# jacarvalho/mpd-public

Measured on AMD Instinct MI355X. Metric: denoising-steps/s, higher is better.
Workload: dtype f32; 1 GPU; cfg2: EnvDense2D-RobotPointMass shape, 100 trajectories (1 context(s)) x H=64 x D=4, T=100 (+5) reverse steps, unguided, U-Net dim_mults (1, 2, 4, 8), one plan = one bench step; parallelism=single, denoising_steps_per_plan=105

## Files before the change

### include/mpdx.h

```cpp
#ifndef MPDX_H
#define MPDX_H

#include <stddef.h>
#include <stdint.h>

#ifdef __cplusplus
extern "C" {
#endif

#define MPDX_E_INVALID   (-1)
#define MPDX_E_NOTFOUND  (-2)
#define MPDX_E_STATE     (-3)
#define MPDX_E_DEVICE    (-4)

#define MPDX_MAX_LEVELS 8

typedef struct mpdx_unet mpdx_unet;

typedef struct mpdx_unet_cfg {
    int32_t state_dim;
    int32_t n_support_points;
    int32_t unet_input_dim;
    int32_t n_levels;
    int32_t dim_mults[MPDX_MAX_LEVELS];
    int32_t time_emb_dim;
    int32_t self_attention;
} mpdx_unet_cfg;

const char* mpdx_last_error(void);
int mpdx_version(void);

int    mpdx_unet_create(const mpdx_unet_cfg* cfg, mpdx_unet** out);
void   mpdx_unet_destroy(mpdx_unet* u);
int    mpdx_unet_set_plan_join(mpdx_unet* u, int on);
int    mpdx_unet_plan_joined(const mpdx_unet* u);
int    mpdx_unet_set_level_split(mpdx_unet* u, int on);
int    mpdx_unet_plan_split(const mpdx_unet* u);
int    mpdx_level_split_block(int B, int block, int32_t* trajectory, int32_t* role);
int    mpdx_unet_set_inner_run(mpdx_unet* u, int on);
int    mpdx_unet_set_inner_run_parts(mpdx_unet* u, int parts);
int    mpdx_unet_set_inner_run_width(mpdx_unet* u, int width);
int    mpdx_inner_run_block(int B, int width, int cus, int block, int32_t* cluster, int32_t* tile, int32_t* counter_lines);
int    mpdx_unet_inner_runs(const mpdx_unet* u);
int    mpdx_unet_inner_run_layers(const mpdx_unet* u);
int    mpdx_unet_status(const mpdx_unet* u);
int    mpdx_unet_set_status(mpdx_unet* u, unsigned word);
int    mpdx_unet_num_params(const mpdx_unet* u);
int    mpdx_unet_param_info(const mpdx_unet* u, int idx, const char** name, int32_t shape[3], int32_t* ndim);
size_t mpdx_unet_packed_floats(const mpdx_unet* u);
size_t mpdx_unet_timetab_floats(const mpdx_unet* u, int T);
size_t mpdx_unet_workspace_floats(const mpdx_unet* u, int B);
int    mpdx_unet_pack_param(mpdx_unet* u, const char* name, const float* src_dev, size_t n_floats,
                            float* packed_dev, void* stream);
int    mpdx_unet_build_timetab(mpdx_unet* u, const float* packed_dev, const float* freqs16_dev, int T,
                               float* timetab_dev, void* stream);

int mpdx_unet_forward(mpdx_unet* u, const float* packed_dev, const float* timetab_dev, int T,
                      const float* x, int t, float* eps, int B, float* ws, void* stream);

typedef struct mpdx_step_coefs {
    float sqrt_recip_alphas_cumprod;
    float sqrt_recipm1_alphas_cumprod;
    float posterior_mean_coef1;
    float posterior_mean_coef2;
    float noise_scale;
    float noise_std_extra;
    int32_t predict_epsilon;
    int32_t clip_denoised;
    float ddim_k1;
    float ddim_k2;
    float guide_scale;
} mpdx_step_coefs;

int mpdx_ddpm_step(mpdx_unet* u, const float* packed_dev, const float* timetab_dev, int T,
                   float* x_io, const float* noise, const float* hard_start, const float* hard_goal,
                   const mpdx_step_coefs* coefs, int t, int mean_only, float* chain_out,
                   uint32_t* absmax_out, int n_per_ctx, int B, float* ws, void* stream);

int mpdx_add_noise(float* x_io, const float* noise, const float* hard_start, const float* hard_goal,
                   float noise_scale, float noise_std_extra, float* chain_out, int B, int H, int D, void* stream);

int mpdx_hard_conds(float* x_io, float* chain_out, int n, const int32_t* horizon_idx, const float* const* values, int B, int H, int D, void* stream);

int mpdx_q_sample(const float* x_start, const float* noise, const long long* t_dev, const float* sqrt_alphas_cumprod_dev,
                  const float* sqrt_one_minus_alphas_cumprod_dev, const float* hard_start, const float* hard_goal, float* out, int B, int H,
                  int D, int T, void* stream);
int mpdx_weighted_loss(const float* pred, const float* targ, const float* weights_hd, const float* hard_start, const float* hard_goal,
                       int l1, float* out1, int B, int H, int D, void* stream);

size_t mpdx_train_flat_floats(mpdx_unet* u);
size_t mpdx_train_dgrad_pack_floats(mpdx_unet* u);
size_t mpdx_train_workspace_floats(mpdx_unet* u, int B);
int    mpdx_train_param_offset(mpdx_unet* u, int idx, size_t* off, size_t* n);
int    mpdx_train_pack(mpdx_unet* u, const float* flat, float* packed, float* packedT, void* stream);
int    mpdx_train_loss_backward(mpdx_unet* u, const float* flat, const float* packed, const float* packedT, float* grads_flat,
                                const float* x_start, const float* noise, const long long* t_dev, const float* sqrt_alphas_cumprod_dev,
                                const float* sqrt_one_minus_alphas_cumprod_dev, const float* freqs16, const float* hard_start,
                                const float* hard_goal, const float* weights_hd, int T, int B, int predict_epsilon, int l1, float loss_scale,
                                float* loss_out, float* ws, void* stream);
int    mpdx_adam_step(float* params, const float* grads, float* exp_avg, float* exp_avg_sq, size_t n, float lr, float beta1, float beta2,
                      float eps, int step, float max_norm, float* scratch, void* stream);
int    mpdx_train_draw(mpdx_unet* u, unsigned long long seed, const int* step_counter_dev);
int    mpdx_ema_update(float* ema, const float* params, size_t n, float beta, void* stream);

int mpdx_randn(float* out, size_t n, uint64_t seed, uint64_t offset, void* stream);

#define MPDX_MAX_FIELDS 4
#define MPDX_FIELD_OBJECTS   0
#define MPDX_FIELD_WORKSPACE 1
#define MPDX_FIELD_SELF      2
#define MPDX_FIELD_GRID      3
#define MPDX_ROBOT_POINTMASS 0
#define MPDX_ROBOT_PANDA     1
#define MPDX_ROBOT_CHAIN     2

typedef struct mpdx_field {
    int32_t kind;
    float   weight;
    int32_t sphere_off, n_spheres;
    int32_t box_off, n_boxes;
    float   ws_min[3], ws_max[3];
    union { int32_t grid_sdf_off;
            int32_t track_len; };
    union { int32_t grid_grad_off;
            int32_t track_off; };
    int32_t n[3];
    float   origin[3];
    float   cell;
    int32_t mode;
} mpdx_field;
#define MPDX_GRID_LINEAR  0
#define MPDX_GRID_NEAREST 1

typedef struct mpdx_guide_params {
    int32_t robot;
    int32_t q_dim;
    int32_t ws_dim;
    int32_t interpolate;
    int32_t n_interp;
    int32_t clip_grad;
    float   max_grad_norm;
    float   mins[16], maxs[16];
    float   cutoff_margin;
    float   link_margin;
    int32_t n_fields;
    mpdx_field fields[MPDX_MAX_FIELDS];
    int32_t use_gp;
    float   gp_weight;
    float   dt;
    float   sigma_gp;
    const float* prims;
    int32_t n_prim_floats;
    int32_t clip_rule;
    float   max_grad_value;
    int32_t gp_half_factor;
    int32_t identity_normalizer;
    const float* grids;
    int32_t n_grid_floats;
    int32_t n_scenes;
    int32_t scene_stride;
    const int32_t* scene_of_ctx;
    int32_t scene_n_per_ctx;
    const float* chain;
    int32_t n_chain_floats;
    int32_t tool_frame;
    float   tool_axis[3];
    float   tool_world[3];
    float   tool_cos_min;
    float   tool_weight;
} mpdx_guide_params;
#define MPDX_ROBOT_CHAIN_MAX_JOINTS    8
#define MPDX_ROBOT_CHAIN_MAX_SPHERES   16
#define MPDX_ROBOT_CHAIN_MAX_PAIRS     24
#define MPDX_ROBOT_CHAIN_HEADER_FLOATS 4
#define MPDX_ROBOT_CHAIN_JOINT_FLOATS  16
#define MPDX_ROBOT_CHAIN_SPHERE_FLOATS 8
#define MPDX_ROBOT_CHAIN_REVOLUTE      0
#define MPDX_ROBOT_CHAIN_PRISMATIC     1
#define MPDX_SCENE_HEADER_WORDS 8
#define MPDX_SCENE_MAX_STAGED_FLOATS 12288

int mpdx_guide_step(const mpdx_guide_params* gp, float* x, float* grad_out, const float* hard_start, const float* hard_goal,
                    const uint32_t* absmax_in, uint32_t* absmax_out, int n_per_ctx, int B, int H, int D, void* stream);
int mpdx_guide_step_scaled(const mpdx_guide_params* gp, float* x, float* grad_out, const float* hard_start, const float* hard_goal,
                           const uint32_t* absmax_in, uint32_t* absmax_out, int n_per_ctx, int B, int H, int D, float guide_scale,
                           void* stream);
int mpdx_guide_time(const mpdx_guide_params* gp, float* x, float* grad_out, const uint32_t* absmax_in, int n_per_ctx, int B, int H, int D,
                    int reps, void* stream, float* ms_avg);
int mpdx_guide_trace(const mpdx_guide_params* gp, float* x, const uint32_t* absmax_in, int B, int H, int D, void* stream,
                     long long* stamps128);
int mpdx_guide_variant(const mpdx_guide_params* gp, int B, int H, int D);
int mpdx_absmax(const float* x, uint32_t* absmax_out, int n_per_ctx, int B, int H, int D, void* stream);

int mpdx_traj_metrics(const mpdx_guide_params* gp, const float* x_unnormalised, float* out4, int n_check, int B, int H, int D,
                      void* stream);
int mpdx_traj_metrics_mask(const mpdx_guide_params* gp, const float* x_unnormalised, float* out4, uint8_t* mask, int n_check, int B,
                           int H, int D, void* stream);

int mpdx_traj_tool_metrics(const mpdx_guide_params* gp, const float* x_unnormalised, float* out2, uint8_t* mask, int n_check, int B, int H, int D,
                           void* stream);

int mpdx_sdf_grid_bake(const mpdx_guide_params* gp, int field, float* sdf_out, float* grad_out, const int n[3], const float origin[3], float cell,
                       void* stream);

size_t mpdx_sdf_grid_edt_ws_bytes(const int n[3]);
int mpdx_sdf_grid_from_occupancy(const uint8_t* occ, float* sdf_out, float* grad_out, int32_t* d2_out, const int n[3], float cell, float inflate, void* ws,
                                 size_t ws_bytes, void* stream);
int mpdx_occupancy_from_points(const float* points, int n_points, uint8_t* occ, const int n[3], const float origin[3], float cell, void* stream);

#define MPDX_MESH_SIGN_WINDING 0
#define MPDX_MESH_SIGN_NONE    1
int mpdx_sdf_grid_from_mesh(const float* vertices, int n_vertices, const int32_t* faces, int n_faces, float* sdf_out, float* grad_out ,
                            float* wind_out , const int n[3], const float origin[3], float cell, float inflate,
                            int sign_mode, void* stream);

#define MPDX_TSDF_MAX_CAMS     8
#define MPDX_TSDF_MAX_SPHERES 64
typedef struct mpdx_depth_camera {
    const float* depth;
    int32_t width, height;
    float fx, fy, cx, cy;
    float cam_from_world[12];
    float world_from_cam[12];
    float min_depth, max_depth;
} mpdx_depth_camera;
int mpdx_tsdf_integrate(const mpdx_depth_camera* cams, int n_cams, const float* spheres , int n_spheres,
                        float* tsdf, float* weight, uint8_t* occ, const int n[3], const float origin[3], float cell, float trunc, float max_weight,
                        void* stream);

typedef struct mpdx_gpmp_opts {
    float   sigma_obs;
    float   lambda_up, lambda_down, lambda_min, lambda_max;
    float   step;
    int32_t adaptive;
} mpdx_gpmp_opts;
int mpdx_gpmp_step(const mpdx_guide_params* gp, const mpdx_gpmp_opts* opts, float* x, float* delta, float* state, int B, int H, int D,
                   int solve, void* stream);

typedef struct mpdx_rrt_opts {
    float    q_lo[8], q_hi[8];
    float    step;
    int32_t  max_nodes, max_iters, max_connect_steps, n_edge_checks;
    uint64_t seed;
} mpdx_rrt_opts;
int mpdx_rrt_connect(const mpdx_guide_params* gp, const mpdx_rrt_opts* opts, const float* start, const float* goal, float* nodes,
                     int32_t* parent, int32_t* count, int32_t* link, int32_t* iters, int n, void* stream);

int mpdx_rrt_paths(const mpdx_guide_params* gp, const float* start, const float* goal, const float* nodes, const int32_t* parent, const int32_t* link,
                   float* trajs_out, int32_t* path_len, int n, int max_nodes, int H, float dt, int n_edge_checks, int rounds, void* stream);

typedef struct mpdx_ik_opts {
    int32_t  frame;
    float    offset[3];
    float    q_lo[8], q_hi[8];
    float    rot_weight;
    float    pos_tol, rot_tol;
    float    lambda_init, lambda_up, lambda_down, lambda_min, lambda_max;
    int32_t  adaptive;
    int32_t  max_iters;
    uint64_t seed;
} mpdx_ik_opts;
int mpdx_ik_solve(const mpdx_guide_params* gp, const mpdx_ik_opts* opts, const float* target, const float* q_init, float* q_out, float* err_out,
                  int32_t* status, int n, int restarts, void* stream);

int mpdx_plan(mpdx_unet* u, const float* packed_dev, const float* timetab_dev, int T, const mpdx_step_coefs* coefs,
              int n_without_noise, float* x, const float* noise, const float* hard_start, const float* hard_goal,
              float* chain, int B, float* ws, const mpdx_guide_params* guide, int n_guide_steps, int t_start_guide,
              uint32_t* guide_flags, int n_per_ctx, uint64_t rng_seed, uint64_t rng_offset, void* stream);

int mpdx_unet_profile(mpdx_unet* u, const float* packed_dev, const float* timetab_dev, int T, const float* x, int t,
                      int B, float* ws, void* stream, int cap, float* ms_out, double* flops_out,
                      const char** names_out, int* n_out);
int mpdx_layer_trace(mpdx_unet* u, const float* packed_dev, const float* timetab_dev, const float* x, int layer, int B, float* ws,
                     void* stream, long long* stamps32);
int mpdx_fused_trace(mpdx_unet* u, const float* packed_dev, const float* timetab_dev, const float* x, int seg, int B,
                     float* ws, void* stream, long long* stamps_out, int cap, int* n_out, int* nops_out);
int mpdx_unet_time_units(mpdx_unet* u, const float* packed_dev, const float* timetab_dev, int T, const float* x, int t, int B,
                         float* ws, void* stream, int unit_first, int unit_last, int reps, float* ms_avg);
int mpdx_unet_time_without(mpdx_unet* u, const float* packed_dev, const float* timetab_dev, int T, const float* x, int t, int B,
                           float* ws, void* stream, unsigned long long skip_mask, int reps, float* ms_avg);
int mpdx_unet_unit_layer(const mpdx_unet* u, int B, int i);
int mpdx_unet_fused_program(const mpdx_unet* u, int seg);
double mpdx_unet_unit_bytes(const mpdx_unet* u, int B, int i);
int mpdx_unet_unit_is_pair(const mpdx_unet* u, int B, int i);
int mpdx_bench_layer(mpdx_unet* u, const float* packed_dev, const float* timetab_dev, const float* x, int layer, int B,
                     float* ws, void* stream, int reps, int dbg, float* ms_per_launch);
int mpdx_unet_layer_tile(const mpdx_unet* u, int i, int B, char* buf, size_t buflen);
int mpdx_attention_block(float* x, const float* to_qkv_w, const float* to_out_w, const float* to_out_b, const float* norm_g, const float* norm_b,
                         int B, int L, int Lv, int C, void* stream);

#ifdef __cplusplus
}
#endif
#endif
```

### mpd_public_amd/_lib.py

```python
from __future__ import annotations

import ctypes as C
from pathlib import Path

import os as _os

_LIB_PATH = Path(_os.environ["MPDX_LIB"]) if _os.environ.get("MPDX_LIB") else Path(__file__).resolve().parent / "libmpdx.so"
_lib = None

MAX_LEVELS = 8


class UnetCfg(C.Structure):
    _fields_ = [("state_dim", C.c_int32), ("n_support_points", C.c_int32), ("unet_input_dim", C.c_int32),
                ("n_levels", C.c_int32), ("dim_mults", C.c_int32 * MAX_LEVELS), ("time_emb_dim", C.c_int32),
                ("self_attention", C.c_int32)]


class StepCoefs(C.Structure):
    _fields_ = [("sqrt_recip_alphas_cumprod", C.c_float), ("sqrt_recipm1_alphas_cumprod", C.c_float),
                ("posterior_mean_coef1", C.c_float), ("posterior_mean_coef2", C.c_float),
                ("noise_scale", C.c_float), ("noise_std_extra", C.c_float),
                ("predict_epsilon", C.c_int32), ("clip_denoised", C.c_int32), ("ddim_k1", C.c_float), ("ddim_k2", C.c_float),
                ("guide_scale", C.c_float)]


MAX_FIELDS = 4
SCENE_HEADER_WORDS = 2 * MAX_FIELDS
SCENE_MAX_STAGED_FLOATS = 12 * 1024
FIELD_OBJECTS, FIELD_WORKSPACE, FIELD_SELF, FIELD_GRID = 0, 1, 2, 3
GRID_LINEAR, GRID_NEAREST = 0, 1
MESH_SIGN_WINDING, MESH_SIGN_NONE = 0, 1
ROBOT_POINTMASS, ROBOT_PANDA, ROBOT_CHAIN = 0, 1, 2
ROBOT_CHAIN_MAX_JOINTS, ROBOT_CHAIN_MAX_SPHERES, ROBOT_CHAIN_MAX_PAIRS = 8, 16, 24
ROBOT_CHAIN_HEADER_FLOATS, ROBOT_CHAIN_JOINT_FLOATS, ROBOT_CHAIN_SPHERE_FLOATS = 4, 16, 8
ROBOT_CHAIN_REVOLUTE, ROBOT_CHAIN_PRISMATIC = 0, 1


class _FieldWord0(C.Union):
    _fields_ = [("grid_sdf_off", C.c_int32), ("track_len", C.c_int32)]


class _FieldWord1(C.Union):
    _fields_ = [("grid_grad_off", C.c_int32), ("track_off", C.c_int32)]


class Field(C.Structure):
    _anonymous_ = ("_word0", "_word1")
    _fields_ = [("kind", C.c_int32), ("weight", C.c_float), ("sphere_off", C.c_int32), ("n_spheres", C.c_int32),
                ("box_off", C.c_int32), ("n_boxes", C.c_int32), ("ws_min", C.c_float * 3), ("ws_max", C.c_float * 3),
                ("_word0", _FieldWord0), ("_word1", _FieldWord1), ("n", C.c_int32 * 3), ("origin", C.c_float * 3),
                ("cell", C.c_float), ("mode", C.c_int32)]


class GuideParams(C.Structure):
    _fields_ = [("robot", C.c_int32), ("q_dim", C.c_int32), ("ws_dim", C.c_int32), ("interpolate", C.c_int32),
                ("n_interp", C.c_int32), ("clip_grad", C.c_int32), ("max_grad_norm", C.c_float),
                ("mins", C.c_float * 16), ("maxs", C.c_float * 16), ("cutoff_margin", C.c_float), ("link_margin", C.c_float),
                ("n_fields", C.c_int32), ("fields", Field * MAX_FIELDS), ("use_gp", C.c_int32), ("gp_weight", C.c_float),
                ("dt", C.c_float), ("sigma_gp", C.c_float), ("prims", C.c_void_p), ("n_prim_floats", C.c_int32),
                ("clip_rule", C.c_int32), ("max_grad_value", C.c_float), ("gp_half_factor", C.c_int32),
                ("identity_normalizer", C.c_int32), ("grids", C.c_void_p), ("n_grid_floats", C.c_int32),
                ("n_scenes", C.c_int32), ("scene_stride", C.c_int32), ("scene_of_ctx", C.c_void_p), ("scene_n_per_ctx", C.c_int32),
                ("chain", C.c_void_p), ("n_chain_floats", C.c_int32),
                ("tool_frame", C.c_int32), ("tool_axis", C.c_float * 3), ("tool_world", C.c_float * 3), ("tool_cos_min", C.c_float),
                ("tool_weight", C.c_float)]


class GpmpOpts(C.Structure):
    _fields_ = [("sigma_obs", C.c_float), ("lambda_up", C.c_float), ("lambda_down", C.c_float), ("lambda_min", C.c_float),
                ("lambda_max", C.c_float), ("step", C.c_float), ("adaptive", C.c_int32)]


class RrtOpts(C.Structure):
    _fields_ = [("q_lo", C.c_float * 8), ("q_hi", C.c_float * 8), ("step", C.c_float), ("max_nodes", C.c_int32), ("max_iters", C.c_int32),
                ("max_connect_steps", C.c_int32), ("n_edge_checks", C.c_int32), ("seed", C.c_uint64)]


class IkOpts(C.Structure):
    _fields_ = [("frame", C.c_int32), ("offset", C.c_float * 3), ("q_lo", C.c_float * 8), ("q_hi", C.c_float * 8), ("rot_weight", C.c_float),
                ("pos_tol", C.c_float), ("rot_tol", C.c_float), ("lambda_init", C.c_float), ("lambda_up", C.c_float), ("lambda_down", C.c_float),
                ("lambda_min", C.c_float), ("lambda_max", C.c_float), ("adaptive", C.c_int32), ("max_iters", C.c_int32), ("seed", C.c_uint64)]


TSDF_MAX_CAMS, TSDF_MAX_SPHERES = 8, 64


class DepthCamera(C.Structure):
    _fields_ = [("depth", C.c_void_p), ("width", C.c_int32), ("height", C.c_int32), ("fx", C.c_float), ("fy", C.c_float), ("cx", C.c_float),
                ("cy", C.c_float), ("cam_from_world", C.c_float * 12), ("world_from_cam", C.c_float * 12), ("min_depth", C.c_float),
                ("max_depth", C.c_float)]


_vp, _sz, _i, _f = C.c_void_p, C.c_size_t, C.c_int, C.c_float
SIGNATURES = {
    "mpdx_last_error": (C.c_char_p, []),
    "mpdx_version": (_i, []),
    "mpdx_unet_create": (_i, [C.POINTER(UnetCfg), C.POINTER(_vp)]),
    "mpdx_unet_destroy": (None, [_vp]),
    "mpdx_unet_set_plan_join": (_i, [_vp, _i]),
    "mpdx_unet_plan_joined": (_i, [_vp]),
    "mpdx_unet_set_level_split": (_i, [_vp, _i]),
    "mpdx_unet_plan_split": (_i, [_vp]),
    "mpdx_level_split_block": (_i, [_i, _i, _vp, _vp]),
    "mpdx_unet_set_inner_run": (_i, [_vp, _i]),
    "mpdx_unet_set_inner_run_parts": (_i, [_vp, _i]),
    "mpdx_unet_set_inner_run_width": (_i, [_vp, _i]),
    "mpdx_inner_run_block": (_i, [_i, _i, _i, _i, _vp, _vp, _vp]),
    "mpdx_unet_inner_runs": (_i, [_vp]),
    "mpdx_unet_inner_run_layers": (_i, [_vp]),
    "mpdx_unet_status": (_i, [_vp]),
    "mpdx_unet_set_status": (_i, [_vp, C.c_uint]),
    "mpdx_unet_num_params": (_i, [_vp]),
    "mpdx_unet_param_info": (_i, [_vp, _i, C.POINTER(C.c_char_p), C.POINTER(C.c_int32 * 3), C.POINTER(C.c_int32)]),
    "mpdx_unet_packed_floats": (_sz, [_vp]),
    "mpdx_unet_timetab_floats": (_sz, [_vp, _i]),
    "mpdx_unet_workspace_floats": (_sz, [_vp, _i]),
    "mpdx_unet_pack_param": (_i, [_vp, C.c_char_p, _vp, _sz, _vp, _vp]),
    "mpdx_unet_build_timetab": (_i, [_vp, _vp, _vp, _i, _vp, _vp]),
    "mpdx_unet_forward": (_i, [_vp, _vp, _vp, _i, _vp, _i, _vp, _i, _vp, _vp]),
    "mpdx_ddpm_step": (_i, [_vp, _vp, _vp, _i, _vp, _vp, _vp, _vp, C.POINTER(StepCoefs), _i, _i, _vp, _vp, _i, _i, _vp, _vp]),
    "mpdx_add_noise": (_i, [_vp, _vp, _vp, _vp, _f, _f, _vp, _i, _i, _i, _vp]),
    "mpdx_hard_conds": (_i, [_vp, _vp, _i, C.POINTER(C.c_int32), C.POINTER(_vp), _i, _i, _i, _vp]),
    "mpdx_q_sample": (_i, [_vp, _vp, _vp, _vp, _vp, _vp, _vp, _vp, _i, _i, _i, _i, _vp]),
    "mpdx_weighted_loss": (_i, [_vp, _vp, _vp, _vp, _vp, _i, _vp, _i, _i, _i, _vp]),
    "mpdx_plan": (_i, [_vp, _vp, _vp, _i, C.POINTER(StepCoefs), _i, _vp, _vp, _vp, _vp, _vp, _i, _vp,
                        C.POINTER(GuideParams), _i, _i, _vp, _i, C.c_uint64, C.c_uint64, _vp]),
    "mpdx_guide_step": (_i, [C.POINTER(GuideParams), _vp, _vp, _vp, _vp, _vp, _vp, _i, _i, _i, _i, _vp]),
    "mpdx_guide_step_scaled": (_i, [C.POINTER(GuideParams), _vp, _vp, _vp, _vp, _vp, _vp, _i, _i, _i, _i, _f, _vp]),
    "mpdx_guide_time": (_i, [C.POINTER(GuideParams), _vp, _vp, _vp, _i, _i, _i, _i, _i, _vp, C.POINTER(C.c_float)]),
    "mpdx_traj_metrics": (_i, [C.POINTER(GuideParams), _vp, _vp, _i, _i, _i, _i, _vp]),
    "mpdx_traj_metrics_mask": (_i, [C.POINTER(GuideParams), _vp, _vp, _vp, _i, _i, _i, _i, _vp]),
    "mpdx_traj_tool_metrics": (_i, [C.POINTER(GuideParams), _vp, _vp, _vp, _i, _i, _i, _i, _vp]),
    "mpdx_guide_trace": (_i, [C.POINTER(GuideParams), _vp, _vp, _i, _i, _i, _vp, C.POINTER(C.c_longlong)]),
    "mpdx_guide_variant": (_i, [C.POINTER(GuideParams), _i, _i, _i]),
    "mpdx_absmax": (_i, [_vp, _vp, _i, _i, _i, _i, _vp]),
    "mpdx_sdf_grid_bake": (_i, [C.POINTER(GuideParams), _i, _vp, _vp, C.POINTER(C.c_int * 3), C.POINTER(C.c_float * 3), _f, _vp]),
    "mpdx_sdf_grid_edt_ws_bytes": (_sz, [C.POINTER(C.c_int * 3)]),
    "mpdx_sdf_grid_from_occupancy": (_i, [_vp, _vp, _vp, _vp, C.POINTER(C.c_int * 3), _f, _f, _vp, _sz, _vp]),
    "mpdx_occupancy_from_points": (_i, [_vp, _i, _vp, C.POINTER(C.c_int * 3), C.POINTER(C.c_float * 3), _f, _vp]),
    "mpdx_sdf_grid_from_mesh": (_i, [_vp, _i, _vp, _i, _vp, _vp, _vp, C.POINTER(C.c_int * 3), C.POINTER(C.c_float * 3), _f, _f, _i, _vp]),
    "mpdx_tsdf_integrate": (_i, [_vp, _i, _vp, _i, _vp, _vp, _vp, C.POINTER(C.c_int * 3), C.POINTER(C.c_float * 3), _f, _f, _f, _vp]),
    "mpdx_unet_profile": (_i, [_vp, _vp, _vp, _i, _vp, _i, _i, _vp, _vp, _i, C.POINTER(C.c_float), C.POINTER(C.c_double),
                                C.POINTER(C.c_char_p), C.POINTER(C.c_int)]),
    "mpdx_layer_trace": (_i, [_vp, _vp, _vp, _vp, _i, _i, _vp, _vp, C.POINTER(C.c_longlong)]),
    "mpdx_fused_trace": (_i, [_vp, _vp, _vp, _vp, _i, _i, _vp, _vp, C.POINTER(C.c_longlong), _i, C.POINTER(C.c_int), C.POINTER(C.c_int)]),
    "mpdx_unet_time_units": (_i, [_vp, _vp, _vp, _i, _vp, _i, _i, _vp, _vp, _i, _i, _i, C.POINTER(C.c_float)]),
    "mpdx_unet_time_without": (_i, [_vp, _vp, _vp, _i, _vp, _i, _i, _vp, _vp, C.c_uint64, _i, C.POINTER(C.c_float)]),
    "mpdx_unet_unit_layer": (_i, [_vp, _i, _i]),
    "mpdx_unet_unit_is_pair": (_i, [_vp, _i, _i]),
    "mpdx_unet_unit_bytes": (C.c_double, [_vp, _i, _i]),
    "mpdx_unet_fused_program": (_i, [_vp, _i]),
    "mpdx_bench_layer": (_i, [_vp, _vp, _vp, _vp, _i, _i, _vp, _vp, _i, _i, C.POINTER(C.c_float)]),
    "mpdx_unet_layer_tile": (_i, [_vp, _i, _i, C.c_char_p, _sz]),
    "mpdx_attention_block": (_i, [_vp, _vp, _vp, _vp, _vp, _vp, _i, _i, _i, _i, _vp]),
    "mpdx_randn": (_i, [_vp, _sz, C.c_uint64, C.c_uint64, _vp]),
    "mpdx_train_flat_floats": (_sz, [_vp]),
    "mpdx_train_dgrad_pack_floats": (_sz, [_vp]),
    "mpdx_train_workspace_floats": (_sz, [_vp, _i]),
    "mpdx_train_param_offset": (_i, [_vp, _i, C.POINTER(_sz), C.POINTER(_sz)]),
    "mpdx_train_pack": (_i, [_vp, _vp, _vp, _vp, _vp]),
    "mpdx_train_loss_backward": (_i, [_vp, _vp, _vp, _vp, _vp, _vp, _vp, _vp, _vp, _vp, _vp, _vp, _vp, _vp, _i, _i, _i, _i, _f, _vp, _vp, _vp]),
    "mpdx_adam_step": (_i, [_vp, _vp, _vp, _vp, _sz, _f, _f, _f, _f, _i, _f, _vp, _vp]),
    "mpdx_train_draw": (_i, [_vp, C.c_uint64, _vp]),
    "mpdx_ema_update": (_i, [_vp, _vp, _sz, _f, _vp]),
    "mpdx_gpmp_step": (_i, [C.POINTER(GuideParams), C.POINTER(GpmpOpts), _vp, _vp, _vp, _i, _i, _i, _i, _vp]),
    "mpdx_rrt_paths": (_i, [C.POINTER(GuideParams), _vp, _vp, _vp, _vp, _vp, _vp, _vp, _i, _i, _i, _f, _i, _i, _vp]),
    "mpdx_rrt_connect": (_i, [C.POINTER(GuideParams), C.POINTER(RrtOpts), _vp, _vp, _vp, _vp, _vp, _vp, _vp, _i, _vp]),
    "mpdx_ik_solve": (_i, [C.POINTER(GuideParams), C.POINTER(IkOpts), _vp, _vp, _vp, _vp, _vp, _i, _i, _vp]),
}


def lib_path() -> Path:
    return _LIB_PATH


class LibraryUnavailable(RuntimeError):
    """libmpdx.so is missing or cannot be loaded on this host (every compute entry point raises it; nothing falls back)"""


def load():
    global _lib
    if _lib is not None:
        return _lib
    if not _LIB_PATH.exists():
        raise LibraryUnavailable(f"{_LIB_PATH} is missing - build it with `python -m mpd_public_amd.build` (hipcc, gfx950). "
                           "mpd_public_amd has no CPU fallback.")
    try:
        lib = C.CDLL(str(_LIB_PATH))
    except OSError as e:
        raise LibraryUnavailable(f"cannot load {_LIB_PATH}: {e}") from e
    for name, (res, args) in SIGNATURES.items():
        try:
            fn = getattr(lib, name)
        except AttributeError as e:
            raise LibraryUnavailable(f"{_LIB_PATH} does not export {name}; rebuild it") from e
        fn.restype, fn.argtypes = res, args
    _lib = lib
    return lib


def check(rc: int, what: str = "") -> None:
    if rc != 0:
        msg = load().mpdx_last_error()
        raise RuntimeError(f"libmpdx {what} failed (code {rc}): {msg.decode() if msg else '?'}")


def ptr(t) -> int:
    if t is None:
        return None
    return t.data_ptr()


def current_stream() -> int:
    import torch
    return torch.cuda.current_stream().cuda_stream
```

### mpd_public_amd/csrc/conv_block.hpp

```cpp
#pragma once
#include <hip/hip_runtime.h>
#include <stdint.h>

#include <type_traits>

#if defined(MPDX_LOOP_ABLATION) && !defined(MPDX_DEV_HOOKS)
#define MPDX_DEV_HOOKS 1
#endif
#ifdef MPDX_DEV_HOOKS
#define MPDX_TRACE_PTR(p) (p)
#define MPDX_DBG(a, bits) ((a).dbg & (bits))
#else
#define MPDX_TRACE_PTR(p) ((long long*)nullptr)
#define MPDX_DBG(a, bits) (0)
#endif

namespace mpdx {

typedef float f32x4 __attribute__((ext_vector_type(4)));
typedef float f32x2 __attribute__((ext_vector_type(2)));

enum : int { CONV_S1 = 0, CONV_DOWN = 1, CONV_UPT = 2 };
enum : int { EPI_BIAS = 0, EPI_GN_MISH = 1, EPI_GN_MISH_GEN = 2, EPI_GN_BWD = 3 };

struct ConvArgs {
    const float* src1;
    const float* src2;
    const float* wp;
    const float* bias;
    const float* gamma;
    const float* beta;
    const float* tbias;
    const float* res;
    float* dst;
    int c1, c2;
    int B, L_in, L_out, C_out;
    int cin_pad;
    int rs;
    int gs;
    int n_tiles_n;
    int lg_c4n, lg_Lin, lg_Lout, lg_gs;
    int dbg;
    long long* trace;
    int tb_stride;
    float* pre;
    float* dst2;
    int c_split, accum;
    float* bw_pg; float* bw_pb; float* bw_pbias; float* bw_dT; float* bw_gres;
    int bw_dT_stride;
    int bw_gres_store;
    int Lv_out;
    int stuff, decim;
};

template <int OFF, int END>
__device__ __forceinline__ void warm_kernarg_lines(unsigned long long kp, int& t) {
    if constexpr (OFF < END) {
        asm volatile("s_load_dword %0, %1, %2" : "+s"(t) : "s"(kp), "n"(OFF));
        warm_kernarg_lines<OFF + 64, END>(kp, t);
    }
}
template <int BYTES>
__device__ __forceinline__ void warm_kernarg() {
    const unsigned long long kp = (unsigned long long)__builtin_amdgcn_kernarg_segment_ptr();
    int t = 0;
    warm_kernarg_lines<0, BYTES>(kp, t);
    asm volatile("s_waitcnt lgkmcnt(0)" : "+s"(t));
}

__device__ __forceinline__ float wave_sum(float v) {
    v += __builtin_bit_cast(float, __builtin_amdgcn_update_dpp(0, __builtin_bit_cast(int, v), 0xB1, 0xF, 0xF, true));
    v += __builtin_bit_cast(float, __builtin_amdgcn_update_dpp(0, __builtin_bit_cast(int, v), 0x4E, 0xF, 0xF, true));
    v += __builtin_bit_cast(float, __builtin_amdgcn_update_dpp(0, __builtin_bit_cast(int, v), 0x141, 0xF, 0xF, true));
    v += __builtin_bit_cast(float, __builtin_amdgcn_update_dpp(0, __builtin_bit_cast(int, v), 0x140, 0xF, 0xF, true));
    v += __builtin_bit_cast(float, __builtin_amdgcn_update_dpp(0, __builtin_bit_cast(int, v), 0x142, 0xA, 0xF, false));
    v += __builtin_bit_cast(float, __builtin_amdgcn_update_dpp(0, __builtin_bit_cast(int, v), 0x143, 0xC, 0xF, false));
    return __builtin_bit_cast(float, __builtin_amdgcn_readlane(__builtin_bit_cast(int, v), 63));
}

__device__ __forceinline__ float mish(float x) {
    const float e = __builtin_amdgcn_exp2f(x * 1.4426950408889634f);
    const float n = e * (e + 2.0f);
    const float r = x * (n * __builtin_amdgcn_rcpf(n + 2.0f));
    return x > 20.0f ? x : r;
}

__device__ __forceinline__ float mish_nosel(float x) {
    const float e = __builtin_amdgcn_exp2f(fminf(x * 1.4426950408889634f, 30.0f));
    const float n = e * (e + 2.0f);
    return x * (n * __builtin_amdgcn_rcpf(n + 2.0f));
}

__device__ __forceinline__ float mish_grad(float v) {
    const float e = __expf(fminf(v, 20.0f));
    const float n = (1.0f + e) * (1.0f + e);
    const float th = (n - 1.0f) / (n + 1.0f);
    const float sg = e / (1.0f + e);
    return th + v * (1.0f - th * th) * sg;
}

__device__ __forceinline__ float gn_rstd(float var) { return __builtin_amdgcn_rsqf(var + 1e-5f); }

struct NoiseRng {
    unsigned long long seed;
    unsigned long long offset;
    unsigned long long elem0;
    int on;
};
__device__ __forceinline__ void philox_round(uint32_t& c0, uint32_t& c1, uint32_t& c2, uint32_t& c3, uint32_t k0, uint32_t k1) {
    const uint64_t p0 = (uint64_t)0xD2511F53u * c0, p1 = (uint64_t)0xCD9E8D57u * c2;
    const uint32_t n0 = (uint32_t)(p1 >> 32) ^ c1 ^ k0, n1 = (uint32_t)p1;
    const uint32_t n2 = (uint32_t)(p0 >> 32) ^ c3 ^ k1, n3 = (uint32_t)p0;
    c0 = n0; c1 = n1; c2 = n2; c3 = n3;
}
__device__ __forceinline__ float philox_radius(uint32_t k) {
    const float u = ((float)k + 0.5f) * (1.0f / 16777216.0f);
    const float v = ((float)(16777216u - k) - 0.5f) * (1.0f / 16777216.0f);
    return sqrtf(k >= 16777216u - 1024u ? 2.0f * v + v * v : -2.0f * logf(u));
}
__device__ __forceinline__ void philox_normal4(uint64_t seed, uint64_t ctr, float (&z)[4]) {
    uint32_t c0 = (uint32_t)ctr, c1 = (uint32_t)(ctr >> 32), c2 = 0x243F6A88u, c3 = 0x85A308D3u;
    uint32_t k0 = (uint32_t)seed, k1 = (uint32_t)(seed >> 32);
#pragma unroll
    for (int r = 0; r < 10; ++r) {
        philox_round(c0, c1, c2, c3, k0, k1);
        k0 += 0x9E3779B9u; k1 += 0xBB67AE85u;
    }
    const float u1 = ((float)(c1 >> 8) + 0.5f) * (1.0f / 16777216.0f), u3 = ((float)(c3 >> 8) + 0.5f) * (1.0f / 16777216.0f);
    const float r0 = philox_radius(c0 >> 8), r1 = philox_radius(c2 >> 8);
    float s0, cs0, s1, cs1;
    sincosf(6.28318530717958647692f * u1, &s0, &cs0);
    sincosf(6.28318530717958647692f * u3, &s1, &cs1);
    z[0] = r0 * cs0; z[1] = r0 * s0; z[2] = r1 * cs1; z[3] = r1 * s1;
}
__device__ __forceinline__ void philox_uniform4(uint64_t seed, uint64_t ctr, float (&u)[4]) {
    uint32_t c0 = (uint32_t)ctr, c1 = (uint32_t)(ctr >> 32), c2 = 0x243F6A88u, c3 = 0x85A308D3u;
    uint32_t k0 = (uint32_t)seed, k1 = (uint32_t)(seed >> 32);
#pragma unroll
    for (int r = 0; r < 10; ++r) {
        philox_round(c0, c1, c2, c3, k0, k1);
        k0 += 0x9E3779B9u; k1 += 0xBB67AE85u;
    }
    u[0] = ((float)(c0 >> 8) + 0.5f) * (1.0f / 16777216.0f); u[1] = ((float)(c1 >> 8) + 0.5f) * (1.0f / 16777216.0f);
    u[2] = ((float)(c2 >> 8) + 0.5f) * (1.0f / 16777216.0f); u[3] = ((float)(c3 >> 8) + 0.5f) * (1.0f / 16777216.0f);
}
__device__ __forceinline__ float philox_normal_at(uint64_t seed, uint64_t offset, uint64_t i) {
    float z[4];
    philox_normal4(seed, offset + (i >> 2), z);
    const int c = (int)(i & 3);
    return c == 0 ? z[0] : c == 1 ? z[1] : c == 2 ? z[2] : z[3];
}

template <int MODE, int KS>
struct ConvGeom {
    static constexpr int PAD = (MODE == CONV_S1) ? KS / 2 : 1;
    static constexpr int NTAP = (MODE == CONV_UPT) ? 2 : KS;
    static constexpr int NSLOT = (MODE == CONV_UPT) ? 4 : KS;
};

__host__ __device__ inline int upt_slot_to_k(int slot) { return slot == 0 ? 1 : slot == 1 ? 3 : slot == 2 ? 2 : 0; }

struct GeoAny { static constexpr int L = 0, NC16 = 0, RSPAD = 0; };
template <int NC16_> struct GeoL8 { static constexpr int L = 8, NC16 = NC16_, RSPAD = 8; };
template <int NC16_> struct GeoUp8 { static constexpr int L = 8, NC16 = NC16_, RSPAD = 4; };
constexpr int geo_ilog2(int v) { return v <= 1 ? 0 : 1 + geo_ilog2(v >> 1); }

struct RunCtx {
    unsigned* counter = nullptr;
    unsigned target = 0;
    int wait = 0;
    long long budget = 0;
    int tiled = 0;
};
__device__ __forceinline__ int run_tiled_off(int pos, int c) { return ((pos >> 3) << 10) + ((c >> 4) << 7) + ((pos & 7) << 4) + (c & 15); }
constexpr unsigned kRunPoison = 0x10000000u;
constexpr unsigned kRunPoisonSeen = 0x08000000u;

typedef unsigned u32x4 __attribute__((ext_vector_type(4)));

template <int MODE, int KS, int EPI, int MT, int NT, int WN, int WK, class GEO = GeoAny, int TBRES = -1, bool RUN = false>
__device__ __forceinline__ bool conv_block_body(const ConvArgs& a, const int block_id, const RunCtx rc = RunCtx()) {
    using G = ConvGeom<MODE, KS>;
    constexpr bool GK = GEO::L > 0;
    static_assert(!GK || MODE == CONV_S1 || MODE == CONV_UPT, "compile-time geometry: stride-1 and transposed convolutions on 8 input positions");
    constexpr int NWAVE = WN * WK, NTHR = 64 * NWAVE;
    constexpr int MS = MT / 16, NSUB = NT / 16, NSW = NSUB / WN;
    constexpr int PAD = G::PAD, NTAP = G::NTAP, NSLOT = G::NSLOT;
    constexpr int MTP = MT + 4;
    constexpr int MTP4 = MTP / 4;
    static_assert(NSUB % WN == 0, "N split");
    static_assert(MODE != CONV_UPT || (NSW % 2 == 0), "transposed conv pairs even/odd sub-tiles");

    extern __shared__ __attribute__((aligned(16))) float smem[];

    const int tid = threadIdx.x, lane = tid & 63;
    if constexpr (GK) __builtin_assume(tid < NTHR);
    const int wave = __builtin_amdgcn_readfirstlane(tid >> 6);
    const int wn = wave % WN, wk = wave / WN;
    int tr_i = 0;
#define CB_STAMP() do { if (MPDX_TRACE_PTR(a.trace) && tid == 0 && (block_id == 0 || block_id == (int)gridDim.x - 1)) a.trace[(block_id ? 16 : 0) + tr_i] = (long long)__builtin_readcyclecounter(); ++tr_i; } while (0)
    const int n_mt = a.C_out / MT;
    const int mt = block_id % n_mt, nt = block_id / n_mt;
    constexpr int GLO = (MODE == CONV_UPT) ? 2 * GEO::L : GEO::L;
    const int L_in = GK ? GEO::L : a.L_in, L_out = GK ? GLO : a.L_out;
    const int lg_Lin = GK ? geo_ilog2(GEO::L) : a.lg_Lin, lg_Lout = GK ? geo_ilog2(GLO) : a.lg_Lout, lg_c4n = GK ? geo_ilog2(GEO::NC16 * 4) : a.lg_c4n;
    const int spt = NT >> lg_Lout;
    const int s0 = nt * spt;
    const int LP = L_in + 2 * PAD;
    const int RS4 = GK ? (GEO::NC16 * 16 + GEO::RSPAD) / 4 : a.rs >> 2;
    f32x4* const smem4 = (f32x4*)smem;
    const int cin = GK ? GEO::NC16 * 16 : a.c1 + a.c2;
    const int c4n = GK ? GEO::NC16 * 4 : a.cin_pad >> 2;

    CB_STAMP();
    constexpr int NCLS = (MODE == CONV_UPT) ? 2 : 1;
#ifndef MPDX_PF
#define MPDX_PF 2
#endif
    constexpr int PF = MPDX_PF;
    const int nc16 = GK ? GEO::NC16 : a.cin_pad >> 4;
    const int ngroups = nc16 * NTAP;
    const __amdgpu_buffer_rsrc_t wrs = __builtin_amdgcn_make_buffer_rsrc((void*)a.wp, 0, 0x7fffffff, 0x00020000);
    const int wlane = lane * 16;
    const int wtile = (mt * MS) * nc16 * NSLOT * 1024;
    f32x4 af[PF][MS][NCLS];
    auto load_a = [&](int g, f32x4 (&dst)[MS][NCLS]) {
        const int c16 = g / NTAP, ts = g - c16 * NTAP;
#pragma unroll
        for (int m = 0; m < MS; ++m)
#pragma unroll
            for (int p = 0; p < NCLS; ++p) {
                const int slot = (MODE == CONV_UPT) ? (p * 2 + ts) : ts;
                dst[m][p] = __builtin_bit_cast(f32x4, __builtin_amdgcn_raw_buffer_load_b128(wrs, wlane, wtile + ((m * nc16 + c16) * NSLOT + slot) * 1024, 0));
            }
    };
    const int niter = (ngroups + WK - 1) / WK;
    auto ring_g = [&](int it) { const int g = wk + it * WK; return g < ngroups ? g : ngroups - 1; };
    auto ring_init = [&]() {
#pragma unroll
        for (int u = 0; u < PF; ++u) load_a(ring_g(u), af[u]);
    };
#ifdef MPDX_RING_FIRST
    ring_init();
#endif
    f32x4 run_bi = {0.f, 0.f, 0.f, 0.f}, run_ga = run_bi, run_be = run_bi, run_tb = run_bi;
    f32x2 run_bi2 = {0.f, 0.f}, run_ga2 = run_bi2, run_be2 = run_bi2, run_tb2 = run_bi2;
    constexpr bool RUN_UP = RUN && MODE == CONV_UPT;
    if constexpr (RUN) {
        static_assert(GK && TBRES < 0 && WN == 1 && ((MODE == CONV_S1 && EPI == EPI_GN_MISH && (MT == 32 || MT == 16)) || (MODE == CONV_UPT && EPI == EPI_BIAS)),
                      "a run layer: stride-1 GroupNorm block or transposed conv + bias, compile-time geometry");
#ifndef MPDX_RING_FIRST
        ring_init();
#endif
        if constexpr (RUN_UP) {
            static_assert(NTHR % (MT / 4) == 0 && NT * (MT / 4) <= NTHR, "bias epilogue: one element per thread");
            run_bi = *(const f32x4*)(a.bias + mt * MT + (tid & (MT / 4 - 1)) * 4);
        } else if constexpr (MT == 32) {
        const int co = mt * MT + ((lane * 4) & (MT - 1));
        run_bi = *(const f32x4*)(a.bias + co);
        run_ga = *(const f32x4*)(a.gamma + co); run_be = *(const f32x4*)(a.beta + co);
        run_tb = *(const f32x4*)((a.tbias ? a.tbias : a.bias) + co);
        } else {
            const int co = mt * MT + ((lane * 2) & (MT - 1));
            run_bi2 = *(const f32x2*)(a.bias + co);
            run_ga2 = *(const f32x2*)(a.gamma + co); run_be2 = *(const f32x2*)(a.beta + co);
            run_tb2 = *(const f32x2*)((a.tbias ? a.tbias : a.bias) + co);
        }
        {
            constexpr int P2 = 2 * PAD;
            const int htot = (spt * P2) << lg_c4n;
            for (int idx = tid; idx < htot; idx += NTHR) {
                const int hr = idx >> lg_c4n, c4 = idx & (c4n - 1);
                const int s = hr / P2, k = hr - s * P2;
                const int lp = (k < PAD) ? k : (L_in + k);
                smem4[(s * LP + lp) * RS4 + c4] = (f32x4){0.f, 0.f, 0.f, 0.f};
            }
        }
        CB_STAMP();
        if (rc.wait) {
            constexpr int STAGE_FL = (GEO::NC16 * 16 + GEO::RSPAD) * (NT / GLO) * (GEO::L + 2 * PAD), RED_FL = WK * NT * MTP;
            int* const flag = (int*)(smem + (STAGE_FL > RED_FL ? STAGE_FL : RED_FL));
            if (wave == 0) {
                const long long t0 = (long long)__builtin_amdgcn_s_memtime();
                int ok;
                for (;;) {
                    const unsigned v = __hip_atomic_load(rc.counter, __ATOMIC_RELAXED, __HIP_MEMORY_SCOPE_AGENT);
                    const int d = (int)(v - rc.target);
                    if (d >= 0) { ok = (unsigned)d < kRunPoisonSeen; break; }
                    if ((long long)__builtin_amdgcn_s_memtime() - t0 > rc.budget) { ok = 0; break; }
                    __builtin_amdgcn_s_sleep(1);
                }
                if (lane == 0) *flag = ok;
            }
            __syncthreads();
            if (!*flag) return false;
        }
        CB_STAMP();
    }

    if (!MPDX_DBG(a, 1)) {
        const int total = (spt << lg_Lin) << lg_c4n;
        const bool vec_ok = GK ? true : ((a.c1 & 3) == 0) && ((a.c2 & 3) == 0);
        constexpr int SB = 4;
        auto stage_pass = [&](int base, auto vec, auto first) {
            constexpr bool VEC = decltype(vec)::value;
            constexpr bool FIRST = decltype(first)::value;
            f32x4 v[SB];
            int dsto[SB], cc[SB];
            bool ok[SB];
            size_t pos[SB];
#pragma unroll
            for (int u = 0; u < SB; ++u) {
                const int idx = base + u * NTHR;
                const bool in = idx < total;
                const int idc = in ? idx : 0;
                const int rowi = idc >> lg_c4n, c = (idc & (c4n - 1)) << 2;
                const int s = rowi >> lg_Lin, li = rowi & (L_in - 1);
                const int b = s0 + s;
                dsto[u] = in ? (s * LP + li + PAD) * RS4 + (c >> 2) : -1;
                ok[u] = in && b < a.B && c < cin;
                cc[u] = c < cin ? c : 0;
                pos[u] = (size_t)(b < a.B ? b : a.B - 1) * L_in + li;
                if (a.stuff) { ok[u] = ok[u] && !(li & 1); pos[u] = (size_t)(b < a.B ? b : a.B - 1) * (L_in >> 1) + (li >> 1); }
            }
#pragma unroll
            for (int u = 0; u < SB; ++u) {
                if constexpr (RUN) {
                    const __amdgpu_buffer_rsrc_t srs = __builtin_amdgcn_make_buffer_rsrc((void*)a.src1, 0, 0x7fffffff, 0x00020000);
                    if constexpr (GEO::NC16 == 8) {
                        const int fo = (rc.tiled & 1) ? run_tiled_off((int)pos[u], cc[u]) : (int)(pos[u] * (GEO::NC16 * 16) + cc[u]);
                        v[u] = __builtin_bit_cast(f32x4, __builtin_amdgcn_raw_buffer_load_b128(srs, fo * 4, 0, 16));
                    } else
                    v[u] = __builtin_bit_cast(f32x4, __builtin_amdgcn_raw_buffer_load_b128(srs, (int)(pos[u] * (GEO::NC16 * 16) + cc[u]) * 4, 0, 16));
                } else if constexpr (VEC) {
                    const float* src = (cc[u] < a.c1) ? a.src1 + pos[u] * a.c1 + cc[u] : a.src2 + pos[u] * a.c2 + (cc[u] - a.c1);
                    v[u] = *(const f32x4*)src;
                } else {
#pragma unroll
                    for (int e = 0; e < 4; ++e) {
                        const int ce = cc[u] + e;
                        const float* src = (ce < a.c1) ? a.src1 + pos[u] * a.c1 + ce : (ce < cin) ? a.src2 + pos[u] * a.c2 + (ce - a.c1) : a.src1 + pos[u] * a.c1;
                        v[u][e] = *src;
                    }
                }
            }
#ifndef MPDX_RING_FIRST
            if constexpr (FIRST && !RUN) ring_init();
#endif
#pragma unroll
            for (int u = 0; u < SB; ++u) {
                if constexpr (!VEC) {
#pragma unroll
                    for (int e = 0; e < 4; ++e) v[u][e] = (cc[u] + e < cin) ? v[u][e] : 0.f;
                }
                if (dsto[u] >= 0) smem4[dsto[u]] = ok[u] ? v[u] : (f32x4){0.f, 0.f, 0.f, 0.f};
            }
        };
        if (vec_ok) {
            stage_pass(tid, std::true_type{}, std::true_type{});
            for (int base = tid + NTHR * SB; base < total; base += NTHR * SB) stage_pass(base, std::true_type{}, std::false_type{});
        } else {
            stage_pass(tid, std::false_type{}, std::true_type{});
            for (int base = tid + NTHR * SB; base < total; base += NTHR * SB) stage_pass(base, std::false_type{}, std::false_type{});
        }
        if (PAD > 0 && !RUN) {
            constexpr int P2 = PAD > 0 ? 2 * PAD : 1;
            const int htot = (spt * P2) << lg_c4n;
            for (int idx = tid; idx < htot; idx += NTHR) {
                const int hr = idx >> lg_c4n, c4 = idx & (c4n - 1);
                const int s = hr / P2, k = hr - s * P2;
                const int lp = (k < PAD) ? k : (L_in + k);
                smem4[(s * LP + lp) * RS4 + c4] = (f32x4){0.f, 0.f, 0.f, 0.f};
            }
        }
    }
#ifndef MPDX_RING_FIRST
    if (!RUN && MPDX_DBG(a, 1)) ring_init();
#endif
    CB_STAMP();
    __syncthreads();
    CB_STAMP();

    const int j = lane & 15, q = lane >> 4;
    int boff[NSW];
    int npos[NSW];
#pragma unroll
    for (int i = 0; i < NSW; ++i) {
        const int ns = wn * NSW + i;
        if (MODE == CONV_UPT) {
            const int gm = (ns >> 1) * 16 + j;
            const int s = gm >> lg_Lin, m = gm & (L_in - 1);
            boff[i] = (s * LP + m + PAD) * RS4 + q;
            npos[i] = s * L_out + 2 * m + (ns & 1);
        } else {
            const int n = ns * 16 + j;
            const int s = n >> lg_Lout, l = n & (L_out - 1);
            const int r0 = (MODE == CONV_DOWN) ? 2 * l : l;
            boff[i] = (s * LP + r0) * RS4 + q;
            npos[i] = n;
        }
    }

    f32x4 acc[MS][NSW];
#pragma unroll
    for (int m = 0; m < MS; ++m)
#pragma unroll
        for (int i = 0; i < NSW; ++i) acc[m][i] = (f32x4){0.f, 0.f, 0.f, 0.f};

    auto kgroup = [&](const int g, f32x4 (&afu)[MS][NCLS]) {
        const int c16 = g / NTAP, ts = g - c16 * NTAP;
#pragma unroll
        for (int i = 0; i < NSW; ++i) {
            const int p = (MODE == CONV_UPT) ? (i & 1) : 0;
            const int roff = (MODE == CONV_UPT) ? ((ts == 0) ? 0 : (p == 0 ? -1 : 1)) : ts;
#ifdef MPDX_LOOP_ABLATION
            const f32x4 bf = (a.dbg & 32) ? (f32x4){1.f, 2.f, 3.f, 4.f} : smem4[boff[i] + roff * RS4 + c16 * 4];
#else
            const f32x4 bf = smem4[boff[i] + roff * RS4 + c16 * 4];
#endif
#pragma unroll
            for (int e = 0; e < 4; ++e)
#pragma unroll
                for (int m = 0; m < MS; ++m)
                    acc[m][i] = __builtin_amdgcn_mfma_f32_16x16x4f32(afu[m][p][e], bf[e], acc[m][i], 0, 0, 0);
        }
    };
    if constexpr (GK) {
        constexpr int NGR = GEO::NC16 * NTAP;
        constexpr int NIT = (NGR + WK - 1) / WK;
        static_assert(NGR % WK == 0, "GeoL8: the k-groups split evenly over the K-split waves");
        if (!MPDX_DBG(a, 2)) {
#pragma unroll
            for (int it = 0; it < NIT; ++it) {
                kgroup(wk + it * WK, af[it % PF]);
                if (it + PF < NIT) load_a(wk + (it + PF) * WK, af[it % PF]);
            }
        }
    } else
    for (int it0 = 0; it0 < niter && !MPDX_DBG(a, 2); it0 += PF) {
#pragma unroll
        for (int u = 0; u < PF; ++u) {
            const int g = wk + (it0 + u) * WK;
            if (g < ngroups) kgroup(g, af[u]);
#ifdef MPDX_LOOP_ABLATION
            if (!(a.dbg & 8)) load_a(ring_g(it0 + u + PF), af[u]);
#else
            load_a(ring_g(it0 + u + PF), af[u]);
#endif
        }
    }

    CB_STAMP();
    __syncthreads();
    CB_STAMP();
    float* red = smem;
#pragma unroll
    for (int m = 0; m < MS; ++m)
#pragma unroll
        for (int i = 0; i < NSW; ++i)
            smem4[(wk * NT + npos[i]) * MTP4 + m * 4 + q] = acc[m][i];
    __syncthreads();
    CB_STAMP();

    if (MPDX_DBG(a, 4)) {
        if (tid == 0 && red[0] == 123.456f) a.dst[0] = red[1];
        return true;
    }
    if constexpr (EPI == EPI_GN_MISH_GEN) {
        const int gs = a.gs;
        const int lg_gpt = (MT == 32 ? 5 : 4) - a.lg_gs;
        const int gpt = 1 << lg_gpt;
        const int nreg = spt << lg_gpt;
        const int re = gs << a.lg_Lout;
        const int Lv = (a.Lv_out > 0 && a.Lv_out < L_out) ? a.Lv_out : L_out;
        const float inv_re = 1.0f / (float)(gs * Lv);
        auto region = [&](auto w_, auto nch_, int s, int gl, int b) {
            constexpr int W = decltype(w_)::value, NCH = decltype(nch_)::value;
            float v[NCH][W], tb[NCH][W], rsd[NCH][W], ga[NCH][W], be[NCH][W];
            size_t o[NCH];
            bool ok[NCH];
            float sum = 0.f;
#pragma unroll
            for (int k = 0; k < NCH; ++k) {
                const int e0 = (k * 64 + lane) * W;
                const int l = e0 >> a.lg_gs, c = gl * gs + (e0 & (gs - 1));
                const int n = s * L_out + l, co = mt * MT + c;
                ok[k] = l < Lv;
                o[k] = ((size_t)(b < a.B ? b : 0) * L_out + l) * a.C_out + co;
#pragma unroll
                for (int e = 0; e < W; ++e) {
                    ga[k][e] = a.gamma[co + e]; be[k][e] = a.beta[co + e];
                    tb[k][e] = a.tbias ? a.tbias[(size_t)(b < a.B ? b : 0) * a.tb_stride + co + e] : 0.f;
                    rsd[k][e] = a.res ? a.res[o[k] + e] : 0.f;
                    float x = red[(size_t)n * MTP + c + e];
#pragma unroll
                    for (int kk = 1; kk < WK; ++kk) x += red[((size_t)(kk * NT + n)) * MTP + c + e];
                    x += a.bias[co + e];
                    v[k][e] = x;
                    if (a.pre && b < a.B) a.pre[o[k] + e] = x;
                }
                float p = v[k][0];
#pragma unroll
                for (int e = 1; e < W; ++e) p += v[k][e];
                sum += ok[k] ? p : 0.f;
            }
            const float mean = wave_sum(sum) * inv_re;
            float sq = 0.f;
#pragma unroll
            for (int k = 0; k < NCH; ++k) {
                float p = 0.f;
#pragma unroll
                for (int e = 0; e < W; ++e) { v[k][e] -= mean; p += v[k][e] * v[k][e]; }
                sq += ok[k] ? p : 0.f;
            }
            const float var = wave_sum(sq) * inv_re;
            const float rstd = gn_rstd(var);
#pragma unroll
            for (int k = 0; k < NCH; ++k) {
#pragma unroll
                for (int e = 0; e < W; ++e) {
                    float y = mish_nosel(v[k][e] * rstd * ga[k][e] + be[k][e]);
                    y += tb[k][e];
                    y += rsd[k][e];
                    if (b < a.B) a.dst[o[k] + e] = ok[k] ? y : 0.f;
                }
            }
        };
        for (int r = wave; r < nreg; r += NWAVE) {
            const int s = r >> lg_gpt, gl = r & (gpt - 1);
            const int b = s0 + s;
            using I1 = std::integral_constant<int, 1>; using I2 = std::integral_constant<int, 2>; using I4 = std::integral_constant<int, 4>;
            using I8 = std::integral_constant<int, 8>;
            switch (re) {
                case 64: region(I1{}, I1{}, s, gl, b); break;
                case 128: region(I2{}, I1{}, s, gl, b); break;
                case 256: region(I4{}, I1{}, s, gl, b); break;
                case 512: region(I4{}, I2{}, s, gl, b); break;
                case 1024: region(I4{}, I4{}, s, gl, b); break;
                default: region(I4{}, I8{}, s, gl, b); break;
            }
        }
    } else
    if constexpr (EPI == EPI_GN_BWD) {
        const int gs = a.gs;
        const int lg_gpt = (MT == 32 ? 5 : 4) - a.lg_gs;
        const int gpt = 1 << lg_gpt;
        const int nreg = spt << lg_gpt;
        const int re = gs << a.lg_Lout;
        auto region = [&](auto epl_, int s, int gl, int b) {
            constexpr int EPL = decltype(epl_)::value;
            const float inv_n = 1.0f / (float)(64 * EPL);
            const int e0 = lane * EPL;
            const int l = e0 >> a.lg_gs, c = gl * gs + (e0 & (gs - 1));
            const int n = s * L_out + l, co = mt * MT + c;
            const int bb = b < a.B ? b : 0;
            const size_t o = ((size_t)bb * L_out + l) * a.C_out + co;
            float u[EPL], gy[EPL], ga[EPL], be[EPL];
#pragma unroll
            for (int e = 0; e < EPL; ++e) { u[e] = a.res[o + e]; ga[e] = a.gamma[co + e]; be[e] = a.beta[co + e]; }
#pragma unroll
            for (int e = 0; e < EPL; ++e) {
                float v = red[(size_t)n * MTP + c + e];
#pragma unroll
                for (int k = 1; k < WK; ++k) v += red[((size_t)(k * NT + n)) * MTP + c + e];
                gy[e] = v + a.bias[co + e];
            }
            if (a.accum & 1) {
#pragma unroll
                for (int e = 0; e < EPL; ++e) gy[e] += a.dst[o + e];
            }
            if (a.bw_gres && b < a.B) {
#pragma unroll
                for (int e = 0; e < EPL; ++e) a.bw_gres[o + e] = a.bw_gres_store ? gy[e] : a.bw_gres[o + e] + gy[e];
            }
            float sm = 0.f;
#pragma unroll
            for (int e = 0; e < EPL; ++e) sm += u[e];
            const float mean = wave_sum(sm) * inv_n;
            float q = 0.f;
#pragma unroll
            for (int e = 0; e < EPL; ++e) { u[e] -= mean; q += u[e] * u[e]; }
            const float var = wave_sum(q) * inv_n;
            const float rstd = 1.0f / sqrtf(var + 1e-5f);
            float vh[EPL], gm[EPL], dvh[EPL];
            float s1 = 0.f, s2 = 0.f;
#pragma unroll
            for (int e = 0; e < EPL; ++e) {
                vh[e] = u[e] * rstd;
                gm[e] = gy[e] * mish_grad(vh[e] * ga[e] + be[e]);
                dvh[e] = gm[e] * ga[e];
                s1 += dvh[e];
                s2 += dvh[e] * vh[e];
            }
            s1 = wave_sum(s1) * inv_n;
            s2 = wave_sum(s2) * inv_n;
            float du[EPL];
#pragma unroll
            for (int e = 0; e < EPL; ++e) {
                du[e] = rstd * (dvh[e] - s1 - vh[e] * s2);
                if (b < a.B) a.dst[o + e] = du[e];
            }
            float r[4 * EPL];
#pragma unroll
            for (int e = 0; e < EPL; ++e) { r[e] = gm[e] * vh[e]; r[EPL + e] = gm[e]; r[2 * EPL + e] = du[e]; r[3 * EPL + e] = gy[e]; }
            for (int off = gs / EPL; off < 64; off <<= 1) {
#pragma unroll
                for (int k = 0; k < 4 * EPL; ++k) r[k] += __shfl_xor(r[k], off, 64);
            }
            if (l == 0 && b < a.B) {
                const size_t po = (size_t)b * a.C_out + co;
#pragma unroll
                for (int e = 0; e < EPL; ++e) {
                    a.bw_pg[po + e] = r[e];
                    a.bw_pb[po + e] = r[EPL + e];
                    a.bw_pbias[po + e] = r[2 * EPL + e];
                    if (a.bw_dT) a.bw_dT[(size_t)b * a.bw_dT_stride + co + e] = r[3 * EPL + e];
                }
            }
        };
        for (int r = wave; r < nreg; r += NWAVE) {
            const int s = r >> lg_gpt, gl = r & (gpt - 1);
            if (re == 256) region(std::integral_constant<int, 4>{}, s, gl, s0 + s);
            else region(std::integral_constant<int, 2>{}, s, gl, s0 + s);
        }
    } else
    if (EPI == EPI_GN_MISH) {
        const int gs = a.gs;
        const int lg_gpt = (MT == 32 ? 5 : 4) - a.lg_gs;
        const int gpt = 1 << lg_gpt;
        const int nreg = spt << lg_gpt;
        const int re = gs << lg_Lout;
        const bool has_tb = TBRES < 0 ? a.tbias != nullptr : TBRES == 1, has_res = TBRES < 0 ? a.res != nullptr : TBRES == 2;
        const float inv_re = (re == 256) ? (1.0f / 256.0f) : (1.0f / 128.0f);
        for (int r = wave; r < nreg; r += NWAVE) {
            const int s = r >> lg_gpt, gl = r & (gpt - 1);
            const int b = s0 + s;
            if constexpr (RUN && MT == 16) {
                const int e0 = lane * 2;
                const int l = e0 >> a.lg_gs, c = gl * gs + (e0 & (gs - 1));
                const int n = s * L_out + l, co = mt * MT + c;
                const int bb = b < a.B ? b : 0;
                const int o = (bb * L_out + l) * a.C_out + co;
                const int ot = run_tiled_off(bb * 8 + l, co);
                const int o_res = (rc.tiled & 2) ? ot : o, o_dst = (rc.tiled & 4) ? ot : o;
                const __amdgpu_buffer_rsrc_t rrs = __builtin_amdgcn_make_buffer_rsrc((void*)(a.res ? a.res : a.src1), 0, 0x7fffffff, 0x00020000);
                f32x2 rs2;
                rs2[0] = __builtin_bit_cast(float, __builtin_amdgcn_raw_buffer_load_b32(rrs, (a.res ? o_res : 0) * 4, 0, 16));
                rs2[1] = __builtin_bit_cast(float, __builtin_amdgcn_raw_buffer_load_b32(rrs, (a.res ? o_res : 0) * 4, __builtin_amdgcn_readfirstlane(4), 16));
                const f32x2 ex = has_tb ? run_tb2 : rs2;
                f32x2 v = *(const f32x2*)(red + (size_t)n * MTP + c);
#pragma unroll
                for (int k = 1; k < WK; ++k) v += *(const f32x2*)(red + ((size_t)(k * NT + n)) * MTP + c);
                v += run_bi2;
                const float mean = wave_sum(v[0] + v[1]) * inv_re;
                const f32x2 d = v - mean;
                const float var = wave_sum(d[0] * d[0] + d[1] * d[1]) * inv_re;
                const float rstd = gn_rstd(var);
                f32x2 y;
#pragma unroll
                for (int e = 0; e < 2; ++e) y[e] = mish_nosel(d[e] * rstd * run_ga2[e] + run_be2[e]);
                y += ex;
                if (b < a.B) {
                    typedef unsigned u32x2 __attribute__((ext_vector_type(2)));
                    const __amdgpu_buffer_rsrc_t drs = __builtin_amdgcn_make_buffer_rsrc((void*)a.dst, 0, 0x7fffffff, 0x00020000);
                    __builtin_amdgcn_raw_buffer_store_b64(__builtin_bit_cast(u32x2, y), drs, o_dst * 4, 0, 16);
                }
            } else
            if constexpr (RUN) {
                const int e0 = lane * 4;
                const int l = e0 >> a.lg_gs, c = gl * gs + (e0 & (gs - 1));
                const int n = s * L_out + l, co = mt * MT + c;
                const size_t o = ((size_t)(b < a.B ? b : 0) * L_out + l) * a.C_out + co;
                const __amdgpu_buffer_rsrc_t rrs = __builtin_amdgcn_make_buffer_rsrc((void*)(a.res ? a.res : a.src1), 0, 0x7fffffff, 0x00020000);
                const f32x4 rs4 = __builtin_bit_cast(f32x4, __builtin_amdgcn_raw_buffer_load_b128(rrs, (int)o * 4, 0, 16));
                const f32x4 ex = has_tb ? run_tb : rs4;
                const int ri = n * MTP4 + (c >> 2);
                f32x4 v = smem4[ri];
#pragma unroll
                for (int k = 1; k < WK; ++k) v += smem4[ri + k * NT * MTP4];
                v += run_bi;
                const float mean = wave_sum((v[0] + v[1]) + (v[2] + v[3])) * inv_re;
                const f32x4 d = v - mean;
                const float var = wave_sum((d[0] * d[0] + d[1] * d[1]) + (d[2] * d[2] + d[3] * d[3])) * inv_re;
                const float rstd = gn_rstd(var);
                f32x4 y;
#pragma unroll
                for (int e = 0; e < 4; ++e) y[e] = mish_nosel(d[e] * rstd * run_ga[e] + run_be[e]);
                y += ex;
                if (b < a.B) {
                    const __amdgpu_buffer_rsrc_t drs = __builtin_amdgcn_make_buffer_rsrc((void*)a.dst, 0, 0x7fffffff, 0x00020000);
                    __builtin_amdgcn_raw_buffer_store_b128(__builtin_bit_cast(u32x4, y), drs, (int)o * 4, 0, 16);
                }
            } else
            if (re == 256) {
                const int e0 = lane * 4;
                const int l = e0 >> a.lg_gs, c = gl * gs + (e0 & (gs - 1));
                const int n = s * L_out + l, co = mt * MT + c;
                const size_t o = ((size_t)(b < a.B ? b : 0) * L_out + l) * a.C_out + co;
                const f32x4 bi = *(const f32x4*)(a.bias + co);
                const f32x4 ga = *(const f32x4*)(a.gamma + co), be = *(const f32x4*)(a.beta + co);
                f32x4 tb = {0.f, 0.f, 0.f, 0.f}, rs4 = {0.f, 0.f, 0.f, 0.f};
                if (has_tb) tb = *(const f32x4*)(a.tbias + (size_t)(b < a.B ? b : 0) * a.tb_stride + co);
                if (has_res) rs4 = *(const f32x4*)(a.res + o);
                const int ri = n * MTP4 + (c >> 2);
                f32x4 v = smem4[ri];
#pragma unroll
                for (int k = 1; k < WK; ++k) v += smem4[ri + k * NT * MTP4];
                v += bi;
                if (a.pre && b < a.B) *(f32x4*)(a.pre + o) = v;
                const float mean = wave_sum((v[0] + v[1]) + (v[2] + v[3])) * inv_re;
                const f32x4 d = v - mean;
                const float var = wave_sum((d[0] * d[0] + d[1] * d[1]) + (d[2] * d[2] + d[3] * d[3])) * inv_re;
                const float rstd = gn_rstd(var);
                f32x4 y;
#pragma unroll
                for (int e = 0; e < 4; ++e) y[e] = mish_nosel(d[e] * rstd * ga[e] + be[e]);
                if (TBRES < 0 || TBRES == 1) y += tb;
                if (TBRES < 0 || TBRES == 2) y += rs4;
                if (b < a.B) *(f32x4*)(a.dst + o) = y;
            } else {
                const int e0 = lane * 2;
                const int l = e0 >> a.lg_gs, c = gl * gs + (e0 & (gs - 1));
                const int n = s * L_out + l, co = mt * MT + c;
                const size_t o = ((size_t)(b < a.B ? b : 0) * L_out + l) * a.C_out + co;
                const f32x2 bi = *(const f32x2*)(a.bias + co);
                const f32x2 ga = *(const f32x2*)(a.gamma + co), be = *(const f32x2*)(a.beta + co);
                f32x2 tb = {0.f, 0.f}, rs2 = {0.f, 0.f};
                if (has_tb) tb = *(const f32x2*)(a.tbias + (size_t)(b < a.B ? b : 0) * a.tb_stride + co);
                if (has_res) rs2 = *(const f32x2*)(a.res + o);
                f32x2 v = *(const f32x2*)(red + (size_t)n * MTP + c);
#pragma unroll
                for (int k = 1; k < WK; ++k) v += *(const f32x2*)(red + ((size_t)(k * NT + n)) * MTP + c);
                v += bi;
                if (a.pre && b < a.B) *(f32x2*)(a.pre + o) = v;
                const float mean = wave_sum(v[0] + v[1]) * inv_re;
                const f32x2 d = v - mean;
                const float var = wave_sum(d[0] * d[0] + d[1] * d[1]) * inv_re;
                const float rstd = gn_rstd(var);
                f32x2 y;
#pragma unroll
                for (int e = 0; e < 2; ++e) y[e] = mish_nosel(d[e] * rstd * ga[e] + be[e]);
                if (TBRES < 0 || TBRES == 1) y += tb;
                if (TBRES < 0 || TBRES == 2) y += rs2;
                if (b < a.B) *(f32x2*)(a.dst + o) = y;
            }
        }
    } else {
        constexpr int M4 = MT / 4;
        for (int idx = tid; idx < NT * M4; idx += NTHR) {
            const int n = idx / M4, c = (idx - n * M4) * 4;
            const int s = n >> lg_Lout, l = n & (L_out - 1), b = s0 + s;
            const int co = mt * MT + c;
            const int ri = n * MTP4 + (c >> 2);
            f32x4 v = smem4[ri];
#pragma unroll
            for (int k = 1; k < WK; ++k) v += smem4[ri + k * NT * MTP4];
            if constexpr (RUN_UP) {
                v += run_bi;
                if (b < a.B) *(f32x4*)(a.dst + ((size_t)b * L_out + l) * a.C_out + co) = v;
                continue;
            }
            v += *(const f32x4*)(a.bias + co);
            float* d = a.dst;
            int ld = a.C_out, cc = co;
            if (a.c_split > 0) {
                if (co >= a.c_split) { d = a.dst2; cc = co - a.c_split; ld = a.C_out - a.c_split; }
                else ld = a.c_split;
            }
            if (a.decim && (l & 1)) continue;
            if (b < a.B && d) {
                f32x4* q = a.decim ? (f32x4*)(d + ((size_t)b * (L_out >> 1) + (l >> 1)) * ld + cc) : (f32x4*)(d + ((size_t)b * L_out + l) * ld + cc);
                if (a.accum & (d == a.dst2 ? 2 : 1)) v += *q;
                if (a.Lv_out > 0 && l >= a.Lv_out) v = (f32x4){0.f, 0.f, 0.f, 0.f};
                *q = v;
            }
        }
    }
    CB_STAMP();
    if constexpr (RUN) {
        asm volatile("s_waitcnt vmcnt(0)" ::: "memory");
        __syncthreads();
        if (tid == 0) __hip_atomic_fetch_add(rc.counter, 1u, __ATOMIC_RELAXED, __HIP_MEMORY_SCOPE_AGENT);
        CB_STAMP();
    }
#undef CB_STAMP
    return true;
}

template <int MODE, int KS, int EPI, int MT, int NT, int WN, int WK, class GEO = GeoAny, int TBRES = -1>
__global__ __launch_bounds__(64 * WN * WK) void conv_block_kernel(const ConvArgs a) {
    conv_block_body<MODE, KS, EPI, MT, NT, WN, WK, GEO, TBRES>(a, blockIdx.x);
}

template <int MT, int NT, class GEO = GeoAny>
__global__ __launch_bounds__(512) void conv_pair_kernel(const ConvArgs a1, const ConvArgs a2, const int n_first) {
    if ((int)blockIdx.x < n_first) conv_block_body<CONV_S1, 5, EPI_GN_MISH, MT, NT, 1, 8, GEO, (GEO::L > 0 ? 1 : -1)>(a1, blockIdx.x);
    else conv_block_body<CONV_S1, 1, EPI_BIAS, MT, NT, 1, 8, GEO>(a2, blockIdx.x - n_first);
}

template <int MODE, int KS, int MT, int NT, int WK>
inline size_t conv_block_lds_bytes(int L_in, int L_out, int rs) {
    using G = ConvGeom<MODE, KS>;
    const size_t stage = (size_t)(NT / L_out) * (L_in + 2 * G::PAD) * rs * sizeof(float);
    const size_t red = (size_t)WK * NT * (MT + 4) * sizeof(float);
    return stage > red ? stage : red;
}

}
```

### mpd_public_amd/csrc/host.hpp

```cpp
#pragma once
#include <hip/hip_runtime.h>

#include <algorithm>
#include <cmath>
#include <cstdarg>
#include <cstdio>
#include <cstdlib>
#include <cstring>
#include <mutex>
#include <set>
#include <string>
#include <unordered_map>
#include <vector>

#include "../../include/mpdx.h"
#include "conv_block.hpp"
#include "conv_ws.hpp"
#include "fused_level.hpp"
#include "switches.hpp"
#include "train_types.hpp"

namespace mpdx {

int fail(int code, const char* fmt, ...);
#define HIP_TRY(expr)                                                                                 \
    do {                                                                                              \
        hipError_t e_ = (expr);                                                                       \
        if (e_ != hipSuccess) return ::mpdx::fail((int)e_, "%s: %s (%s:%d)", #expr, hipGetErrorString(e_), __FILE__, __LINE__); \
    } while (0)
int raise_lds_limit(const void* kern);
int dev_hooks_missing(const char* fn);
inline bool finite_f(float v) { return fabsf(v) < 3.0e38f; }

struct FinalArgs {
    const float* h;
    const float* w;
    const float* bias;
    const float* x_in;
    const float* noise;
    const float* hs;
    const float* hg;
    float* out;
    float* chain;
    uint32_t* absmax;
    int B, H, D, C;
    int Hc;
    int mode;
    int n_per_ctx;
    mpdx_step_coefs k;
    NoiseRng rng;
};

enum ParamKind { PK_VEC = 0, PK_CONV = 1, PK_CONVT = 2 };

struct Param {
    std::string name;
    int32_t shape[3] = {0, 0, 0};
    int32_t ndim = 0;
    size_t n = 0;
    size_t off = 0;
    size_t foff = 0;
    size_t pn = 0;
    int kind = PK_VEC;
    int cout = 0, cin = 0, ksz = 0, cin_pad = 0, nslot = 0;
    bool done = false;
};

enum { SRC_X = -1, SRC_NONE = -2 };

struct Layer {
    int mode = CONV_S1, ks = 5, epi = EPI_GN_MISH;
    int c1 = 0, c2 = 0, cout = 0, L_in = 0, L_out = 0, gs = 0;
    int Lv_out = 0;
    int src1 = SRC_NONE, src2 = SRC_NONE, dst = 0, res = SRC_NONE;
    int w = -1, b = -1, gamma = -1, beta = -1;
    int tb_off = -1;
    int cin_pad = 0, rs = 0;
    bool attn = false;
    int w2 = -1, b2 = -1;
    bool pin_nt = false;
    std::string name;
};

}

struct mpdx_unet {
    mpdx_unet_cfg cfg;
    std::vector<mpdx::Param> params;
    std::unordered_map<std::string, int> pidx;
    std::vector<mpdx::Layer> layers;
    size_t packed_floats = 0;
    size_t slot_floats = 0;
    int n_slots = 0;
    int tt_row = 0;
    std::vector<int> tt_w, tt_b, tt_cout, tt_off;
    int final_slot = 0;
    int n_done = 0;
    int Hc = 0, xpad_slot = -1;
    bool masked() const { return Hc != cfg.n_support_points; }
    int plan_join = 1;
    enum RunPart { kRunSeven = 1, kRunTail = 2 };
    int inner_run = kRunSeven | kRunTail;
    int inner_run_width = 0;
    int plan_joined = 0, inner_runs = 0;
    int inner_run_layers = 0;
    struct InnerRunState {
        int capacity = -1;
        int seven_wgs[2] = {0, 0}, tail_wgs[2] = {0, 0};
        long long budget = 0;
        unsigned* counters = nullptr;
        struct Counters {
            unsigned* p = nullptr;
            unsigned base = 0;
            int live = 1 << 30;
            bool rezero = false;
        } ctr[2];
        unsigned *status = nullptr, *status_dev = nullptr;
        unsigned status_host = 0;
        unsigned status_word() const { return status ? __atomic_load_n(status, __ATOMIC_RELAXED) : status_host; }
    } run;
    int level_split = -1;
    int plan_split = 0;
    struct LevelSplitState {
        int capacity = -1;
        int wgs = 0;
        float* xch = nullptr;
        unsigned* counters = nullptr;
        unsigned base = 0;
        int live = 1 << 30;
        bool rezero = false;
    } split;
    struct CopyJob { size_t src, dst; int n0, ss0, ds0, n1, ss1, ds1, n_inner; };
    struct Fused {
        int first = 0, count = 0;
        bool has_final = false;
        int in1 = 0, in2 = 0;
        int in3 = mpdx::SRC_NONE;
        int gout_slot[3] = {-1, -1, -1};
        size_t lds_bytes = 0;
        mpdx::FusedArgs tmpl;
        int program = -1;
        std::vector<CopyJob> jobs;
        std::vector<int> op_layer;
        int in3_consumer = -1;
    };
    std::vector<Fused> fused;
    void* jobs_dev = nullptr;
    int n_jobs = 0;
    const float* streams_for = nullptr;
    int pack_version = 0, streams_version = -1;
    enum UnitKind { kProgram, kLayer, kPair, kInnerRun, kTailRun };
    struct Unit { UnitKind kind; int fused; int layer; int count; int width = 0; };
    std::vector<int> owner;
    struct TrainLayer {
        int src1_l = -2, src2_l = -2, res_l = -2;
        bool need_dgrad = false;
        size_t dgrad_woff = 0;
        mpdx::Layer dg;
    };
    bool train_ready = false;
    size_t flat_floats = 0, packedT_floats = 0;
    std::vector<TrainLayer> tl;
    std::vector<mpdx::PackDesc> pack_descs_host;
    void* pack_descs_dev = nullptr;
    void* pack_chunks_dev = nullptr;
    size_t n_pack_chunks = 0;
};

namespace mpdx {

int pick_row_stride(int cin_pad, int mode, int L_in, int L_out, int LP);
void choose_tile(const Layer& l, int B, int& MT, int& NT);
bool layer_ksplit(const Layer& l);
int check_ready(const mpdx_unet* u);
unsigned fused_mask(int B);
bool fused_save_variant(const mpdx_unet::Fused& f);
int ensure_fused_streams(mpdx_unet* u, const float* packed, hipStream_t st);
int claim_fused_stream_jobs(mpdx_unet* u, const float* packed, const void** jobs, int* n);
int launch_final_step(const FinalArgs& fa, hipStream_t st);
int launch_conv_layer(const Layer& l, ConvArgs& a, int B, hipStream_t st);
bool pair_tile(const Layer& l1, const Layer& l2, int B, int& MT, int& NT);
int launch_conv_pair(int MT, int NT, const ConvArgs& a1, const ConvArgs& a2, const Layer& l1, const Layer& l2, hipStream_t st);
template <int N> struct RunArgs;
bool inner_run_width_ok(int width);
int inner_run_clusters(int B, int width);
int inner_run_grid(int B, int width);
void inner_run_slot(int block, int* cluster, int* tile);
int inner_run_workgroups_per_cu(int width);
int tail_run_workgroups_per_cu(int width);
int launch_inner_run(const RunArgs<7>& ra, int B, int width, hipStream_t st);
int launch_tail_run(const RunArgs<4>& ra, int B, int width, hipStream_t st);
struct AttnArgs;
const char* attn_unsupported(int C, int L);
int launch_attention(const Layer& l, AttnArgs& a, int B, hipStream_t st);
int launch_weight_stationary(int variant, const Layer& l, ConvArgs& a, const ConvArgs& a2, int B, hipStream_t st);
int launch_fused_args(const mpdx_unet::Fused& f, const FusedArgs& a, int B, hipStream_t st, bool save = false);
int launch_fused_train(const mpdx_unet::Fused& f, const FusedArgs& a, int B, hipStream_t st);
int launch_fused_join(const FusedJoinArgs& ja, int B, hipStream_t st);
size_t fused_join_lds_bytes();
int launch_fused_join_split(const FusedJoinArgs& ja, const FusedSplitArgs& sa, int B, hipStream_t st);
int fused_join_split_workgroups_per_cu();
struct NoiseRng;
int launch_guide(const mpdx_guide_params* gp, float* x, float* grad_out, const float* hs, const float* hg, const uint32_t* amax_in,
                 uint32_t* amax_out, int n_per_ctx, int B, int H, int D, hipStream_t st, const float* noise = nullptr, float noise_scale = 0.f,
                 float noise_extra = 0.f, float* chain = nullptr, float guide_scale = 1.0f, const NoiseRng* rng = nullptr);
const char* chain_params_problem(const mpdx_guide_params& gp);
const char* tool_params_problem(const mpdx_guide_params& gp);
struct ChainInfo;
int guide_block_problem(const mpdx_guide_params* gp, int D, ChainInfo* chain_info, int H);

}
```

### mpd_public_amd/csrc/inner_run.hpp

```cpp
#pragma once
#include "conv_block.hpp"

namespace mpdx {

constexpr int kInnerRunLayers = 7;
constexpr int kTailRunLayers = 4;
constexpr int kInnerRunCounterStride = 32;
constexpr int kRunWide = 32, kRunNarrow = 16;

struct RunSlot { int c, m; };
constexpr int run_clusters(int B, int width) { return (B + width / 8 - 1) / (width / 8); }
constexpr int run_grid(int nc, bool same_xcd) { return same_xcd ? ((nc + 7) / 8) * 64 : nc * 8; }
constexpr int run_block(int c, int m, bool same_xcd) { return same_xcd ? (c & 7) + 8 * (m + 8 * (c >> 3)) : 8 * c + m; }
__host__ __device__ constexpr RunSlot run_slot(int block, bool same_xcd) {
    return same_xcd ? RunSlot{((block >> 6) << 3) + (block & 7), (block >> 3) & 7} : RunSlot{block >> 3, block & 7};
}
constexpr bool run_map_ok(int width) {
    for (int B = 1; B <= 128; ++B) {
        const int nc = run_clusters(B, width), grid = run_grid(nc, true);
        int live = 0;
        for (int b = 0; b < grid; ++b) {
            const RunSlot s = run_slot(b, true);
            if (s.m < 0 || s.m > 7 || s.c < 0) return false;
            if (s.c >= nc) continue;
            if (run_block(s.c, s.m, true) != b || (b & 7) != (s.c & 7)) return false;
            ++live;
        }
        if (live != 8 * nc || grid % 64 || grid < 8 * nc) return false;
    }
    return true;
}
static_assert(run_map_ok(kRunWide) && run_map_ok(kRunNarrow), "block <-> (cluster, channel tile): a bijection on the live blocks, one XCD per cluster");

template <int N>
struct RunArgs {
    ConvArgs layer[N];
    unsigned* counters;
    unsigned* status;
    long long budget;
    unsigned base;
    int n_layers;
    int nc;
};
typedef RunArgs<kInnerRunLayers> InnerRunArgs;
typedef RunArgs<kTailRunLayers> TailRunArgs;

constexpr size_t run_max(size_t a, size_t b) { return a > b ? a : b; }

template <int NT>
struct RunSeqSeven {
    typedef InnerRunArgs Args;
    static constexpr int kWidth = NT, kSpt = NT / 8;
    static constexpr int kLayers = kInnerRunLayers;
    static constexpr bool kUp = false;
    static constexpr int kLastL = 8, kLastMT = 32, kLastC = 256;
    static __device__ __forceinline__ bool gn(const ConvArgs& a, int id, const RunCtx& rc) { return conv_block_body<CONV_S1, 5, EPI_GN_MISH, 32, NT, 1, 8, GeoL8<16>, -1, true>(a, id, rc); }
    static __device__ __forceinline__ bool up(const ConvArgs&, int, const RunCtx&) { return true; }
    static __device__ __forceinline__ int tiled(int) { return 0; }
    static size_t lds() { return conv_block_lds_bytes<CONV_S1, 5, 32, NT, 8>(8, 8, 256 + 8) + 16; }
};
template <int NT>
struct RunSeqTail {
    typedef TailRunArgs Args;
    static constexpr int kWidth = NT, kSpt = NT / 8;
    static constexpr int kLayers = kTailRunLayers;
    static constexpr bool kUp = true;
    static constexpr int kLastL = 16, kLastMT = 16, kLastC = 128;
    static __device__ __forceinline__ bool gn(const ConvArgs& a, int id, const RunCtx& rc) { return conv_block_body<CONV_S1, 5, EPI_GN_MISH, 16, NT, 1, 8, GeoL8<8>, -1, true>(a, id, rc); }
    static __device__ __forceinline__ bool up(const ConvArgs& a, int id, const RunCtx& rc) { return conv_block_body<CONV_UPT, 4, EPI_BIAS, 16, 2 * NT, 1, 8, GeoUp8<8>, -1, true>(a, id, rc); }
    static __device__ __forceinline__ int tiled(int i) { return i >= 3 ? 1 : ((i > 0 ? 1 : 0) | (i == 2 ? 2 : 0) | 4); }
    static size_t lds() { return run_max(conv_block_lds_bytes<CONV_S1, 5, 16, NT, 8>(8, 8, 128 + 8), conv_block_lds_bytes<CONV_UPT, 4, 16, 2 * NT, 8>(8, 16, 128 + 4)) + 16; }
};

template <class SEQ>
__device__ __forceinline__ void run_give_up(const typename SEQ::Args& ra, const RunCtx& rc, const int c, const int m, const int i) {
    const int tid = threadIdx.x;
    if (tid == 0) {
        __hip_atomic_fetch_or(ra.status, 1u | ((unsigned)i << 8), __ATOMIC_RELAXED, __HIP_MEMORY_SCOPE_SYSTEM);
        __hip_atomic_store(rc.counter, rc.target + kRunPoison, __ATOMIC_RELAXED, __HIP_MEMORY_SCOPE_AGENT);
    }
    const ConvArgs& last = ra.layer[ra.n_layers - 1];
    constexpr int L = SEQ::kLastL, MT = SEQ::kLastMT;
    for (int e = tid; e < SEQ::kSpt * L * MT; e += 512) {
        const int b = c * SEQ::kSpt + (e >> geo_ilog2(L * MT)), l = (e >> geo_ilog2(MT)) & (L - 1), ch = m * MT + (e & (MT - 1));
        if (b < last.B) last.dst[((size_t)b * L + l) * SEQ::kLastC + ch] = __builtin_nanf("");
    }
}

template <class SEQ, bool SAME_XCD>
__global__ __launch_bounds__(512) void inner_run_kernel(const typename SEQ::Args ra) {
    const RunSlot slot = run_slot((int)blockIdx.x, SAME_XCD);
    const int c = slot.c, m = slot.m;
    if constexpr (SAME_XCD) {
        if (c >= ra.nc) return;
    }
    warm_kernarg<sizeof(typename SEQ::Args)>();
    RunCtx rc;
    rc.counter = ra.counters + (size_t)c * kInnerRunCounterStride;
    rc.budget = ra.budget;
    const int n_gn = SEQ::kUp ? ra.n_layers - 1 : ra.n_layers;
#pragma nounroll
    for (int i = 0; i < n_gn; ++i) {
        rc.wait = i > 0;
        rc.target = ra.base + 8u * (unsigned)i;
        rc.tiled = SEQ::tiled(i);
        if (SEQ::gn(ra.layer[i], c * 8 + m, rc)) continue;
        run_give_up<SEQ>(ra, rc, c, m, i);
        return;
    }
    if constexpr (SEQ::kUp) {
        rc.wait = n_gn > 0;
        rc.target = ra.base + 8u * (unsigned)n_gn;
        rc.tiled = SEQ::tiled(n_gn);
        if (!SEQ::up(ra.layer[n_gn], c * 8 + m, rc)) run_give_up<SEQ>(ra, rc, c, m, n_gn);
    }
}

}
```

### mpd_public_amd/csrc/k_inner_run.hip

```cpp
#include "host.hpp"
#include "inner_run.hpp"

namespace mpdx {

#ifndef MPDX_INNER_RUN_SAME_XCD
#define MPDX_INNER_RUN_SAME_XCD 1
#endif
static constexpr bool kSameXcd = MPDX_INNER_RUN_SAME_XCD != 0;

bool inner_run_width_ok(int width) { return width == kRunWide || width == kRunNarrow; }
int inner_run_clusters(int B, int width) { return inner_run_width_ok(width) ? run_clusters(B, width) : 0; }
int inner_run_grid(int B, int width) { return run_grid(inner_run_clusters(B, width), kSameXcd); }
void inner_run_slot(int block, int* cluster, int* tile) { const RunSlot s = run_slot(block, kSameXcd); *cluster = s.c; *tile = s.m; }

template <class SEQ>
static int workgroups_per_cu() {
    int n = 0;
    if (hipOccupancyMaxActiveBlocksPerMultiprocessor(&n, (const void*)inner_run_kernel<SEQ, kSameXcd>, 512, SEQ::lds()) != hipSuccess) {
        (void)hipGetLastError();
        return 0;
    }
    return n;
}
int inner_run_workgroups_per_cu(int width) {
    return width == kRunWide ? workgroups_per_cu<RunSeqSeven<kRunWide>>() : width == kRunNarrow ? workgroups_per_cu<RunSeqSeven<kRunNarrow>>() : 0;
}
int tail_run_workgroups_per_cu(int width) {
    return width == kRunWide ? workgroups_per_cu<RunSeqTail<kRunWide>>() : width == kRunNarrow ? workgroups_per_cu<RunSeqTail<kRunNarrow>>() : 0;
}

template <class SEQ>
static int launch_run(const typename SEQ::Args& ra, int B, hipStream_t st, const char* what) {
    if (ra.n_layers != SEQ::kLayers || ra.nc != run_clusters(B, SEQ::kWidth))
        return fail(MPDX_E_INVALID, "%s: %d layers, %d clusters for B=%d at width %d", what, ra.n_layers, ra.nc, B, SEQ::kWidth);
    hipLaunchKernelGGL((inner_run_kernel<SEQ, kSameXcd>), dim3(run_grid(ra.nc, kSameXcd)), dim3(512), SEQ::lds(), st, ra);
    return 0;
}
int launch_inner_run(const InnerRunArgs& ra, int B, int width, hipStream_t st) {
    if (width == kRunNarrow) return launch_run<RunSeqSeven<kRunNarrow>>(ra, B, st, "inner run");
    if (width == kRunWide) return launch_run<RunSeqSeven<kRunWide>>(ra, B, st, "inner run");
    return fail(MPDX_E_INVALID, "inner run: width %d", width);
}
int launch_tail_run(const TailRunArgs& ra, int B, int width, hipStream_t st) {
    if (width == kRunNarrow) return launch_run<RunSeqTail<kRunNarrow>>(ra, B, st, "tail run");
    if (width == kRunWide) return launch_run<RunSeqTail<kRunWide>>(ra, B, st, "tail run");
    return fail(MPDX_E_INVALID, "tail run: width %d", width);
}

}
```

### mpd_public_amd/csrc/mpdx.hip

```cpp
#include "host.hpp"
#include "attn.hpp"
#include "inner_run.hpp"
#include "loss.hpp"
#include "scene_table.hpp"
#include "motion.hpp"

namespace mpdx {

static thread_local char g_err[512] = "";
int fail(int code, const char* fmt, ...) {
    va_list ap;
    va_start(ap, fmt);
    vsnprintf(g_err, sizeof(g_err), fmt, ap);
    va_end(ap);
    return code;
}

int raise_lds_limit(const void* kern) {
    static std::mutex mu;
    static std::set<std::pair<int, const void*>> done;
    int dev = 0;
    HIP_TRY(hipGetDevice(&dev));
    std::lock_guard<std::mutex> lock(mu);
    if (done.count({dev, kern})) return 0;
    HIP_TRY(hipFuncSetAttribute(kern, hipFuncAttributeMaxDynamicSharedMemorySize, 160 * 1024));
    done.insert({dev, kern});
    return 0;
}

static long long* g_conv_trace = nullptr;


struct TimeTabArgs {
    const float* packed;
    const float* freqs;
    float* tab;
    int w1, b1, w2, b2;
    int row;
    int nblk;
    int woff[40], boff[40], cout[40], toff[40];
};

__global__ __launch_bounds__(128) void timetab_kernel(const TimeTabArgs a) {
    __shared__ float emb[32], h1[128], te[32];
    const int t = blockIdx.x, tid = threadIdx.x;
    if (tid < 16) {
        const float arg = (float)t * a.freqs[tid];
        emb[tid] = sinf(arg);
        emb[tid + 16] = cosf(arg);
    }
    __syncthreads();
    {
        const float* w = a.packed + a.w1 + tid * 32;
        float s = a.packed[a.b1 + tid];
        for (int k = 0; k < 32; ++k) s = fmaf(w[k], emb[k], s);
        h1[tid] = mish(s);
    }
    __syncthreads();
    if (tid < 32) {
        const float* w = a.packed + a.w2 + tid * 128;
        float s = a.packed[a.b2 + tid];
        for (int k = 0; k < 128; ++k) s = fmaf(w[k], h1[k], s);
        te[tid] = mish(s);
    }
    __syncthreads();
    for (int blk = 0; blk < a.nblk; ++blk) {
        for (int c = tid; c < a.cout[blk]; c += 128) {
            const float* w = a.packed + a.woff[blk] + c * 32;
            float s = a.packed[a.boff[blk] + c];
            for (int k = 0; k < 32; ++k) s = fmaf(w[k], te[k], s);
            a.tab[(size_t)t * a.row + a.toff[blk] + c] = s;
        }
    }
}


__global__ __launch_bounds__(256) void final_step_kernel(const FinalArgs a) {
    extern __shared__ __attribute__((aligned(16))) float sm[];
    float* w = sm;
    float* bs = sm + a.D * a.C;
    for (int i = threadIdx.x; i < a.D * a.C; i += blockDim.x) w[i] = a.w[i];
    for (int i = threadIdx.x; i < a.D; i += blockDim.x) bs[i] = a.bias[i];
    __syncthreads();
    const int p = blockIdx.x * blockDim.x + threadIdx.x;
    const bool live = p < a.B * a.H;
    const int b = live ? p / a.H : 0, l = live ? p - b * a.H : 0;
    float vmax = 0.f;
    if (live) {
        const float* hp = a.h + ((size_t)b * (a.Hc > 0 ? a.Hc : a.H) + l) * a.C;
        for (int d = 0; d < a.D; ++d) {
            float s = bs[d];
            for (int c = 0; c < a.C; c += 4) {
                const f32x4 hv = *(const f32x4*)(hp + c);
                const f32x4 wv = *(const f32x4*)(w + d * a.C + c);
                s = fmaf(hv[0], wv[0], s); s = fmaf(hv[1], wv[1], s);
                s = fmaf(hv[2], wv[2], s); s = fmaf(hv[3], wv[3], s);
            }
            const size_t o = (size_t)p * a.D + d;
            float r;
            if (a.mode == 0) {
                r = s;
            } else {
                const float xv = a.x_in[o];
                float x0;
                if (a.k.predict_epsilon)
                    x0 = __fsub_rn(__fmul_rn(a.k.sqrt_recip_alphas_cumprod, xv), __fmul_rn(a.k.sqrt_recipm1_alphas_cumprod, s));
                else
                    x0 = s;
                if (a.mode == 3) {
                    const float pn = a.k.predict_epsilon
                                         ? s
                                         : __fdiv_rn(__fsub_rn(__fmul_rn(a.k.sqrt_recip_alphas_cumprod, xv), s), a.k.sqrt_recipm1_alphas_cumprod);
                    r = __fadd_rn(__fmul_rn(x0, a.k.ddim_k1), __fmul_rn(a.k.ddim_k2, pn));
                    if (a.hs && l == 0) r = a.hs[(size_t)b * a.D + d];
                    if (a.hg && l == a.H - 1) r = a.hg[(size_t)b * a.D + d];
                } else {
                    if (a.k.clip_denoised) x0 = fminf(fmaxf(x0, -1.0f), 1.0f);
                    r = __fadd_rn(__fmul_rn(a.k.posterior_mean_coef1, x0), __fmul_rn(a.k.posterior_mean_coef2, xv));
                    if (a.mode == 1) {
                        if (a.rng.on) r = __fadd_rn(r, __fmul_rn(__fmul_rn(a.k.noise_scale, philox_normal_at(a.rng.seed, a.rng.offset, a.rng.elem0 + o)), a.k.noise_std_extra));
                        else if (a.noise) r = __fadd_rn(r, __fmul_rn(__fmul_rn(a.k.noise_scale, a.noise[o]), a.k.noise_std_extra));
                        if (a.hs && l == 0) r = a.hs[(size_t)b * a.D + d];
                        if (a.hg && l == a.H - 1) r = a.hg[(size_t)b * a.D + d];
                    }
                }
            }
            a.out[o] = r;
            if (a.chain) a.chain[o] = r;
            vmax = fmaxf(vmax, fabsf(r));
        }
    }
    if (a.absmax) {
        const int ctx = b / a.n_per_ctx;
        const int ctx0 = __builtin_amdgcn_readfirstlane(ctx);
        if (__all(ctx == ctx0)) {
            float m = vmax;
#pragma unroll
            for (int s = 32; s >= 1; s >>= 1) m = fmaxf(m, __shfl_xor(m, s, 64));
            if ((threadIdx.x & 63) == 0) atomicMax(a.absmax + ctx0, __float_as_uint(m));
        } else if (live) {
            atomicMax(a.absmax + ctx, __float_as_uint(vmax));
        }
    }
}

__global__ __launch_bounds__(256) void add_noise_kernel(float* x, const float* noise, const float* hs, const float* hg,
                                                         float scale, float extra, float* chain, int B, int H, int D) {
    const size_t n = (size_t)B * H * D;
    for (size_t i = (size_t)blockIdx.x * blockDim.x + threadIdx.x; i < n; i += (size_t)gridDim.x * blockDim.x) {
        const int d = i % D;
        const size_t p = i / D;
        const int l = p % H;
        const size_t b = p / H;
        float r = x[i];
        if (noise) r = __fadd_rn(r, __fmul_rn(__fmul_rn(scale, noise[i]), extra));
        if (hs && l == 0) r = hs[b * D + d];
        if (hg && l == H - 1) r = hg[b * D + d];
        x[i] = r;
        if (chain) chain[i] = r;
    }
}

constexpr int kMaxHardConds = 16;
struct HardCondArgs { int idx[kMaxHardConds]; const float* vals[kMaxHardConds]; int n; };
__global__ __launch_bounds__(256) void hard_conds_kernel(float* x, float* chain, const HardCondArgs a, int B, int H, int D) {
    const size_t per = (size_t)B * D;
    for (size_t i = (size_t)blockIdx.x * blockDim.x + threadIdx.x; i < per; i += (size_t)gridDim.x * blockDim.x) {
        const size_t b = i / D;
        const int d = (int)(i - b * D);
        for (int k = 0; k < a.n; ++k) {
            const float v = a.vals[k][i];
            const size_t o = (b * H + a.idx[k]) * D + d;
            x[o] = v;
            if (chain) chain[o] = v;
        }
    }
}

__global__ __launch_bounds__(256) void q_sample_kernel(const float* x0, const float* noise, const long long* t, const float* sqrt_ac,
                                                        const float* sqrt_1mac, const float* hs, const float* hg, float* out, int B, int H,
                                                        int D, int T) {
    const size_t n = (size_t)B * H * D;
    for (size_t i = (size_t)blockIdx.x * blockDim.x + threadIdx.x; i < n; i += (size_t)gridDim.x * blockDim.x) {
        const int d = i % D;
        const size_t p = i / D;
        const int l = p % H;
        const size_t b = p / H;
        long long tb = t[b];
        tb = tb < 0 ? 0 : (tb >= T ? T - 1 : tb);
        float r = __fadd_rn(__fmul_rn(sqrt_ac[tb], x0[i]), __fmul_rn(sqrt_1mac[tb], noise[i]));
        if (hs && l == 0) r = hs[b * D + d];
        if (hg && l == H - 1) r = hg[b * D + d];
        out[i] = r;
    }
}

__global__ __launch_bounds__(1024) void weighted_loss_kernel(const float* pred, const float* targ, const float* weights, const float* hs,
                                                             const float* hg, int l1, float* out, int B, int H, int D) {
    __shared__ double part[16];
    weighted_loss_body(pred, targ, weights, hs, hg, l1, out, B, H, D, part);
}

__global__ __launch_bounds__(256) void randn_kernel(float* out, size_t n, uint64_t seed, uint64_t offset) {
    const size_t nquad = (n + 3) / 4;
    for (size_t qd = (size_t)blockIdx.x * blockDim.x + threadIdx.x; qd < nquad; qd += (size_t)gridDim.x * blockDim.x) {
        float z[4];
        philox_normal4(seed, qd + offset, z);
        const size_t base = qd * 4;
#pragma unroll
        for (int e = 0; e < 4; ++e)
            if (base + e < n) out[base + e] = z[e];
    }
}

__global__ __launch_bounds__(256) void pad_input_kernel(const float* __restrict__ x, float* __restrict__ xc, int B, int H, int Hc, int D) {
    const size_t n = (size_t)B * Hc * D;
    for (size_t i = (size_t)blockIdx.x * blockDim.x + threadIdx.x; i < n; i += (size_t)gridDim.x * blockDim.x) {
        const int d = (int)(i % D);
        const size_t p = i / D;
        const int l = (int)(p % Hc);
        const size_t b = p / Hc;
        xc[i] = l < H ? x[(b * H + l) * D + d] : 0.f;
    }
}

__global__ void copy_kernel(const float* __restrict__ src, float* __restrict__ dst, size_t n) {
    for (size_t i = (size_t)blockIdx.x * blockDim.x + threadIdx.x; i < n; i += (size_t)gridDim.x * blockDim.x) dst[i] = src[i];
}

__global__ void pack_conv_weights_kernel(const float* __restrict__ src, float* __restrict__ dst, int C_out, int C_in,
                                         int ksz, int cin_pad, int nslot, int transposed) {
    const int nc16 = cin_pad >> 4;
    const size_t total = (size_t)(C_out >> 4) * nc16 * nslot * 256;
    for (size_t i = (size_t)blockIdx.x * blockDim.x + threadIdx.x; i < total; i += (size_t)gridDim.x * blockDim.x) {
        const int e = i & 3, lane = (i >> 2) & 63;
        size_t r = i >> 8;
        const int slot = r % nslot; r /= nslot;
        const int c16 = r % nc16; const int m16 = r / nc16;
        const int co = m16 * 16 + (lane & 15);
        const int ci = c16 * 16 + (lane >> 4) * 4 + e;
        float v = 0.f;
        if (ci < C_in) {
            if (transposed) v = src[((size_t)ci * C_out + co) * ksz + upt_slot_to_k(slot)];
            else v = src[((size_t)co * C_in + ci) * ksz + slot];
        }
        dst[i] = v;
    }
}


static int gn_groups(int c) {
    if (c < 8) return 1;
    for (int g = 8; g < 18; ++g)
        if (c % g == 0) return g;
    return 1;
}

static int pad_cin(int c) {
    int p = (c + 15) / 16 * 16;
    while (p & (p - 1)) p += 16;
    return p;
}

static int add_param(mpdx_unet* u, const std::string& name, std::initializer_list<int> shape, int kind = PK_VEC) {
    Param p;
    p.name = name;
    p.ndim = (int)shape.size();
    p.n = 1;
    int i = 0;
    for (int s : shape) { p.shape[i++] = s; p.n *= (size_t)s; }
    p.kind = kind;
    if (kind == PK_CONV) {
        p.cout = p.shape[0]; p.cin = p.shape[1]; p.ksz = p.shape[2];
        p.nslot = p.ksz;
    } else if (kind == PK_CONVT) {
        p.cin = p.shape[0]; p.cout = p.shape[1]; p.ksz = p.shape[2];
        p.nslot = 4;
    }
    if (kind != PK_VEC) {
        p.cin_pad = pad_cin(p.cin);
        p.pn = (size_t)(p.cout / 16) * (p.cin_pad / 16) * p.nslot * 256;
    } else {
        p.pn = (p.n + 3) / 4 * 4;
    }
    p.off = u->packed_floats;
    u->packed_floats += p.pn;
    u->pidx[name] = (int)u->params.size();
    u->params.push_back(p);
    return (int)u->params.size() - 1;
}

int pick_row_stride(int cin_pad, int mode, int L_in, int L_out, int LP) {
    static const int groups[4][16] = {{0, 1, 2, 3, 12, 13, 14, 15, 20, 21, 22, 23, 24, 25, 26, 27},
                                      {4, 5, 6, 7, 8, 9, 10, 11, 16, 17, 18, 19, 28, 29, 30, 31},
                                      {32, 33, 34, 35, 44, 45, 46, 47, 52, 53, 54, 55, 56, 57, 58, 59},
                                      {36, 37, 38, 39, 40, 41, 42, 43, 48, 49, 50, 51, 60, 61, 62, 63}};
    int best_rs = cin_pad, best = 1 << 30;
    for (int pad = 0; pad <= 64; pad += 4) {
        const int rs = cin_pad + pad;
        int score = 0;
        for (int g = 0; g < 4; ++g) {
            int cnt[16] = {0};
            int worst = 0;
            for (int i = 0; i < 16; ++i) {
                const int lane = groups[g][i], j = lane & 15, q = lane >> 4;
                int row;
                if (mode == CONV_UPT) { const int s = j / L_in, m = j % L_in; row = s * LP + m; }
                else { const int s = j / L_out, l = j % L_out; row = s * LP + (mode == CONV_DOWN ? 2 * l : l); }
                const int slot16 = ((row * rs + q * 4) & 63) >> 2;
                worst = std::max(worst, ++cnt[slot16]);
            }
            score += worst;
        }
        if (score < best) { best = score; best_rs = rs; }
        if (best == 4) break;
    }
    return best_rs;
}

static void build_model(mpdx_unet* u) {
    const mpdx_unet_cfg& c = u->cfg;
    const int nl = c.n_levels, D = c.state_dim, te = c.time_emb_dim;
    const int Hv = c.n_support_points;
    int H = 1;
    while (H < Hv) H <<= 1;
    u->Hc = H;
    std::vector<int> dims(nl + 1);
    dims[0] = D;
    for (int i = 0; i < nl; ++i) dims[i + 1] = c.unet_input_dim * c.dim_mults[i];

    add_param(u, "time_mlp.encoder.1.weight", {128, 32});
    add_param(u, "time_mlp.encoder.1.bias", {128});
    add_param(u, "time_mlp.encoder.3.weight", {te, 128});
    add_param(u, "time_mlp.encoder.3.bias", {te});

    const int P0 = 0, P1 = 1, HB = 2, RB = 3, S0 = 4;
    u->n_slots = S0 + nl;
    auto other = [&](int s) { return s == P0 ? P1 : P0; };
    size_t slot = 0;

    auto conv_layer = [&](const std::string& wname, const std::string& bname, int mode, int ks, int epi, int src1, int c1,
                          int src2, int c2, int cout, int L_in, int L_out, int dst) -> Layer& {
        Layer l;
        l.name = wname; l.mode = mode; l.ks = ks; l.epi = epi;
        l.src1 = src1; l.c1 = c1; l.src2 = src2; l.c2 = c2; l.cout = cout; l.L_in = L_in; l.L_out = L_out; l.dst = dst;
        l.Lv_out = (H != Hv) ? (int)((long)L_out * Hv / H) : 0;
        l.pin_nt = c.self_attention != 0;
        if (mode == CONV_UPT) l.w = add_param(u, wname, {c1 + c2, cout, ks}, PK_CONVT);
        else l.w = add_param(u, wname, {cout, c1 + c2, ks}, PK_CONV);
        l.b = add_param(u, bname, {cout});
        l.cin_pad = pad_cin(c1 + c2);
        const int pad = (mode == CONV_S1) ? ks / 2 : 1;
        l.rs = pick_row_stride(l.cin_pad, mode, L_in, L_out, L_in + 2 * pad);
        slot = std::max(slot, (size_t)cout * L_out);
        u->layers.push_back(l);
        return u->layers.back();
    };
    auto cblock = [&](const std::string& p, int src1, int c1, int src2, int c2, int cout, int L, int dst) -> Layer& {
        Layer& l = conv_layer(p + ".block.0.weight", p + ".block.0.bias", CONV_S1, 5, EPI_GN_MISH, src1, c1, src2, c2, cout, L, L, dst);
        const int idx = (int)u->layers.size() - 1;
        const int ga = add_param(u, p + ".block.2.weight", {cout});
        const int be = add_param(u, p + ".block.2.bias", {cout});
        Layer& ll = u->layers[idx];
        ll.gamma = ga; ll.beta = be;
        ll.gs = cout / gn_groups(cout);
        (void)l;
        return ll;
    };
    auto rtb = [&](const std::string& p, int src1, int c1, int src2, int c2, int cout, int L, int dst) {
        {
            Layer& b0 = cblock(p + ".blocks.0", src1, c1, src2, c2, cout, L, HB);
            b0.tb_off = u->tt_row;
        }
        const int i1 = (int)u->layers.size();
        cblock(p + ".blocks.1", HB, cout, SRC_NONE, 0, cout, L, dst);
        const int tw = add_param(u, p + ".cond_mlp.1.weight", {cout, te});
        const int tbp = add_param(u, p + ".cond_mlp.1.bias", {cout});
        u->tt_w.push_back(tw); u->tt_b.push_back(tbp); u->tt_cout.push_back(cout); u->tt_off.push_back(u->tt_row);
        u->tt_row += cout;
        int res = src1;
        if (c1 + c2 != cout) {
            Layer keep = u->layers[i1];
            u->layers.pop_back();
            conv_layer(p + ".residual_conv.weight", p + ".residual_conv.bias", CONV_S1, 1, EPI_BIAS, src1, c1, src2, c2, cout, L, L, RB);
            u->layers.push_back(keep);
            res = RB;
        }
        u->layers.back().res = res;
    };

    auto attention = [&](const std::string& p, int slot_id, int C, int Lc) {
        if (!c.self_attention) return;
        Layer l;
        l.name = p + ".fn.fn.to_qkv.weight"; l.attn = true; l.mode = CONV_S1; l.ks = 0; l.epi = EPI_BIAS;
        l.src1 = slot_id; l.dst = slot_id; l.c1 = C; l.cout = C; l.L_in = Lc; l.L_out = Lc;
        l.Lv_out = (H != Hv) ? (int)((long)Lc * Hv / H) : 0;
        l.w = add_param(u, p + ".fn.fn.to_qkv.weight", {3 * kAttnHid, C, 1}, PK_CONV);
        l.w2 = add_param(u, p + ".fn.fn.to_out.weight", {C, kAttnHid, 1}, PK_CONV);
        l.b2 = add_param(u, p + ".fn.fn.to_out.bias", {C});
        l.gamma = add_param(u, p + ".fn.norm.g", {1, C, 1});
        l.beta = add_param(u, p + ".fn.norm.b", {1, C, 1});
        l.cin_pad = pad_cin(C);
        l.rs = pick_row_stride(l.cin_pad, CONV_S1, Lc, Lc, Lc);
        u->layers.push_back(l);
    };

    int L = H, cur = SRC_X, curC = D;
    for (int i = 0; i < nl; ++i) {
        const int co = dims[i + 1];
        const std::string p = "downs." + std::to_string(i);
        const int a = other(cur);
        rtb(p + ".0", cur, curC, SRC_NONE, 0, co, L, a);
        rtb(p + ".1", a, co, SRC_NONE, 0, co, L, S0 + i);
        attention(p + ".2", S0 + i, co, L);
        cur = S0 + i; curC = co;
        if (i < nl - 1) {
            conv_layer(p + ".4.conv.weight", p + ".4.conv.bias", CONV_DOWN, 3, EPI_BIAS, cur, co, SRC_NONE, 0, co, L, L / 2, P0);
            cur = P0; L /= 2;
        }
    }
    rtb("mid_block1", cur, curC, SRC_NONE, 0, curC, L, P0);
    attention("mid_attn", P0, curC, L);
    rtb("mid_block2", P0, curC, SRC_NONE, 0, curC, L, P1);
    cur = P1;
    for (int j = 0; j < nl - 1; ++j) {
        const int lv = nl - 1 - j;
        const int dout = dims[lv + 1], din = dims[lv];
        const std::string p = "ups." + std::to_string(j);
        const int a = other(cur);
        rtb(p + ".0", cur, dout, S0 + lv, dout, din, L, a);
        const int b = other(a);
        rtb(p + ".1", a, din, SRC_NONE, 0, din, L, b);
        attention(p + ".2", b, din, L);
        const int d = other(b);
        conv_layer(p + ".4.conv.weight", p + ".4.conv.bias", CONV_UPT, 4, EPI_BIAS, b, din, SRC_NONE, 0, din, L, 2 * L, d);
        cur = d; L *= 2; curC = din;
    }
    cblock("final_conv.0", cur, curC, SRC_NONE, 0, c.unet_input_dim, L, HB);
    u->final_slot = HB;
    add_param(u, "final_conv.1.weight", {D, c.unet_input_dim, 1});
    add_param(u, "final_conv.1.bias", {D});
    u->slot_floats = std::max(slot, (size_t)c.unet_input_dim * H);
    if (H != Hv) u->xpad_slot = u->n_slots++;
}

}

#include "fused_build.hpp"

namespace mpdx {

void choose_tile(const Layer& l, int B, int& MT, int& NT) {
    const int min_mt = (l.epi == EPI_GN_MISH && l.gs > 16) ? 32 : 16;
    const int min_nt = std::max(l.mode == CONV_UPT ? 32 : 16, l.L_out);
    const long npos = (long)B * l.L_out;
    if (const char* ov = sw::tile()) {
        int mt = 0, nt = 0;
        if (sscanf(ov, "%dx%d", &mt, &nt) == 2 && mt >= min_mt && nt >= min_nt && l.cout % mt == 0 && nt % l.L_out == 0) { MT = mt; NT = nt; return; }
    }
    if (min_nt > 64) {
        NT = min_nt;
        MT = (min_mt <= 16 && l.cout % 16 == 0) ? 16 : 32;
        return;
    }
    const int target = std::max(1, sw::target_wgs());
    auto wgs = [&](int mt, int nt) { return (long)(l.cout / mt) * ((npos + nt - 1) / nt); };
    const int pad = (l.mode == CONV_S1) ? l.ks / 2 : 1;
    auto lds = [&](int mt, int nt) {
        const size_t stage = (size_t)(nt / l.L_out) * (l.L_in + 2 * pad) * l.rs * sizeof(float);
        const size_t red = (size_t)8 * nt * (mt + 4) * sizeof(float);
        return std::max(stage, red);
    };
    const int mts[2] = {32, 16}, nts[3] = {64, 32, 16};
    if (l.pin_nt && !layer_ksplit(l)) {
        NT = min_nt;
        for (int mt : mts)
            if (mt >= min_mt && l.cout % mt == 0 && lds(mt, NT) <= (size_t)sw::lds_cap_kb() * 1024 && wgs(mt, NT) >= target) { MT = mt; return; }
        MT = (min_mt <= 16 && l.cout % 16 == 0) ? 16 : 32;
        return;
    }
    const size_t cap = (size_t)sw::lds_cap_kb() * 1024;
    for (int nt : nts)
        for (int mt : mts) {
            if (mt < min_mt || nt < min_nt || l.cout % mt || lds(mt, nt) > cap) continue;
            if (wgs(mt, nt) >= target) { MT = mt; NT = nt; return; }
        }
    MT = (min_mt <= 16 && l.cout % 16 == 0) ? 16 : 32;
    NT = min_nt;
}

static int layer_ntap(const Layer& l) { return l.mode == CONV_UPT ? 2 : l.ks; }
bool layer_ksplit(const Layer& l) {
    if (!(l.mode == CONV_S1 && l.ks == 5 && l.epi == EPI_GN_MISH)) return true;
    if (const int forced = sw::ksplit(); forced >= 0) return forced != 0;
    return (l.cin_pad / 16) * layer_ntap(l) >= 16;
}
static double layer_flops(const Layer& l, int B) {
    if (l.attn) return (double)B * l.L_out * (1024.0 * l.cout + 16384.0);
    return 2.0 * l.cout * (double)B * l.L_out * (l.c1 + l.c2) * layer_ntap(l);
}


static int make_conv_args(const mpdx_unet* u, const Layer& l, const float* packed, const float* tt_row, const float* x, float* ws, int B,
                          int dbg, ConvArgs& a) {
    const size_t slot = u->slot_floats * (size_t)B;
    auto src = [&](int s) -> const float* { return s == SRC_X ? x : (s == SRC_NONE ? nullptr : ws + slot * s); };
    memset(&a, 0, sizeof(a));
    a.src1 = src(l.src1); a.src2 = src(l.src2);
    a.c1 = l.c1; a.c2 = l.c2;
    a.wp = packed + u->params[l.w].off;
    a.bias = packed + u->params[l.b].off;
    a.gamma = l.gamma >= 0 ? packed + u->params[l.gamma].off : nullptr;
    a.beta = l.beta >= 0 ? packed + u->params[l.beta].off : nullptr;
    a.tbias = (l.tb_off >= 0 && tt_row) ? tt_row + l.tb_off : nullptr;
    a.res = src(l.res);
    a.dst = ws + slot * l.dst;
    a.B = B; a.L_in = l.L_in; a.L_out = l.L_out; a.C_out = l.cout;
    a.cin_pad = l.cin_pad; a.rs = l.rs; a.gs = l.gs; a.dbg = dbg;
    a.Lv_out = l.Lv_out;
    a.trace = g_conv_trace;
    auto lg2 = [](int v) { int k = 0; while ((1 << k) < v) ++k; return k; };
    a.lg_c4n = lg2(l.cin_pad / 4); a.lg_Lin = lg2(l.L_in); a.lg_Lout = lg2(l.L_out); a.lg_gs = l.gs > 0 ? lg2(l.gs) : 0;
    if ((1 << a.lg_c4n) != l.cin_pad / 4 || (1 << a.lg_Lin) != l.L_in || (1 << a.lg_Lout) != l.L_out || (l.gs > 0 && (1 << a.lg_gs) != l.gs))
        return fail(MPDX_E_INVALID, "layer %s: channel/length/group sizes must be powers of two", l.name.c_str());
    return 0;
}

static int weight_stationary_variant(const Layer& l, const Layer* l2, const ConvArgs& a, int B, int dbg) {
    const int ws_env = sw::ws();
    const int wsn_min_b = sw::wsn_min_b(), wsp_min_b = sw::wsp_min_b();
    const bool wsn_on = sw::wsn() && ws_env != 0 && B >= wsn_min_b;
    const bool wsp_on = ws_env != 0 && B >= wsp_min_b && sw::wsp();
    if (l.mode == CONV_UPT && l.ks == 4 && l.epi == EPI_BIAS && !l2 && l.L_in == 8 && l.L_out == 16 && !l.Lv_out && l.c1 == 128 && l.c2 == 0 &&
        l.cin_pad == 128 && l.cout == 128 && !dbg && !a.pre && !a.accum && !a.dst2 && wsn_on && (long)B * 8 >= 16L * kWsGroups * 8)
        return 5;
    if (!(l.mode == CONV_S1 && l.ks == 5 && l.epi == EPI_GN_MISH && l.L_out == 8 && l.L_in == 8) || l.Lv_out) return 0;
    if (dbg || a.pre || (l.c1 & 3) || (l.c2 & 3) || l.cin_pad != l.c1 + l.c2) return 0;
    if ((long)B * l.L_out < 16L * kWsGroups * 8) return 0;
    if (ws_env == 0 || (l2 && ws_env == 2)) return 0;
    if (l2) {
        if (!(l2->mode == CONV_S1 && l2->ks == 1 && l2->epi == EPI_BIAS && l2->cout == l.cout && l2->L_out == 8 && l2->c1 == l.c1 && l2->c2 == l.c2)) return 0;
        if (l.cout == 128 && l.gs == 16 && l.cin_pad == 512) return 3;
        if (l.cout == 256 && l.gs == 32 && l.cin_pad == 128 && l.c2 == 0 && wsp_on && !a.res)
            return 6;
        return 0;
    }
    if (l.cout == 256 && l.gs == 32 && l.cin_pad == 256) return 1;
    if (l.cout == 128 && l.gs == 16 && l.cin_pad == 128 && l.c2 == 0 && wsn_on) return 4;
    return 0;
}


static int run_layer(const mpdx_unet* u, const Layer& l, const float* packed, const float* tt_row, const float* x,
                     float* ws, int B, hipStream_t st, int dbg = 0) {
    if (l.attn) {
        AttnArgs aa;
        memset(&aa, 0, sizeof(aa));
        aa.x = ws + u->slot_floats * (size_t)B * l.dst;
        aa.wqkv = packed + u->params[l.w].off; aa.wout = packed + u->params[l.w2].off; aa.bout = packed + u->params[l.b2].off;
        aa.g = packed + u->params[l.gamma].off; aa.b = packed + u->params[l.beta].off;
        return launch_attention(l, aa, B, st);
    }
    ConvArgs a;
    if (int rc = make_conv_args(u, l, packed, tt_row, x, ws, B, dbg, a)) return rc;
    if (const int v = weight_stationary_variant(l, nullptr, a, B, dbg)) return launch_weight_stationary(v, l, a, a, B, st);
    return launch_conv_layer(l, a, B, st);
}

bool pair_tile(const Layer& l1, const Layer& l2, int B, int& MT, int& NT) {
    if (!sw::pair()) return false;
    if (!(l1.mode == CONV_S1 && l1.ks == 5 && l1.epi == EPI_GN_MISH && l2.mode == CONV_S1 && l2.ks == 1 && l2.epi == EPI_BIAS)) return false;
    if ((l1.gs * l1.L_out != 128 && l1.gs * l1.L_out != 256) || l1.Lv_out) return false;
    if (l1.src1 != l2.src1 || l1.src2 != l2.src2 || l1.cout != l2.cout || l1.L_out != l2.L_out || !layer_ksplit(l1)) return false;
    choose_tile(l1, B, MT, NT);
    if (l1.cout % MT) MT = 16;
    if (l1.cout % MT || NT % l1.L_out) return false;
    const size_t lds = std::max({(size_t)(NT / l1.L_out) * (l1.L_in + 4) * l1.rs * sizeof(float), (size_t)(NT / l2.L_out) * l2.L_in * l2.rs * sizeof(float),
                                 (size_t)8 * NT * (MT + 4) * sizeof(float)});
    return lds <= 160 * 1024;
}

static int run_pair(const mpdx_unet* u, const Layer& l1, const Layer& l2, const float* packed, const float* tt_row, const float* x, float* ws,
                    int B, hipStream_t st) {
    int MT, NT;
    if (!pair_tile(l1, l2, B, MT, NT)) return fail(MPDX_E_STATE, "layers %s / %s do not pair", l1.name.c_str(), l2.name.c_str());
    ConvArgs a1, a2;
    if (int rc = make_conv_args(u, l1, packed, tt_row, x, ws, B, 0, a1)) return rc;
    if (int rc = make_conv_args(u, l2, packed, tt_row, x, ws, B, 0, a2)) return rc;
    if (const int v = weight_stationary_variant(l1, &l2, a1, B, 0)) return launch_weight_stationary(v, l1, a1, a2, B, st);
    a1.n_tiles_n = a2.n_tiles_n = (int)(((long)B * l1.L_out + NT - 1) / NT);
    return launch_conv_pair(MT, NT, a1, a2, l1, l2, st) == 1 ? 0 : fail(MPDX_E_INVALID, "pair launch failed (tile %dx%d)", MT, NT);
}

int check_ready(const mpdx_unet* u) {
    if (u->n_done != (int)u->params.size())
        return fail(MPDX_E_STATE, "%d of %zu parameters packed; call mpdx_unet_pack_param for every state-dict tensor first",
                    u->n_done, u->params.size());
    return 0;
}

unsigned fused_mask(int B) {
    (void)B;
    return sw::fused() ? sw::fused_mask() : 0u;
}
static std::vector<mpdx_unet::Unit> current_units(const mpdx_unet* u, int B, bool* final_in_fused) {
    std::vector<mpdx_unet::Unit> out;
    const unsigned m = fused_mask(B);
    bool fin = false;
    const int nlay = (int)u->layers.size();
    auto fused_on = [&](int i) { const int o = u->owner[i]; return o >= 0 && ((m >> o) & 1u); };
    for (int i = 0; i < nlay; ++i) {
        const int o = u->owner[i];
        if (fused_on(i)) {
            if (i == u->fused[o].first) { out.push_back({mpdx_unet::kProgram, o, i, u->fused[o].count}); fin |= u->fused[o].has_final; }
            continue;
        }
        int MT, NT;
        if (i + 1 < nlay && !fused_on(i + 1) && pair_tile(u->layers[i], u->layers[i + 1], B, MT, NT)) {
            out.push_back({mpdx_unet::kPair, -1, i, 2});
            ++i;
            continue;
        }
        out.push_back({mpdx_unet::kLayer, -1, i, 1});
    }
    if (final_in_fused) *final_in_fused = fin;
    return out;
}

static int run_final(mpdx_unet* u, const float* packed, FinalArgs& fa, int B, float* ws, hipStream_t st) {
    const mpdx_unet_cfg& c = u->cfg;
    fa.h = ws + u->slot_floats * (size_t)B * u->final_slot;
    fa.w = packed + u->params[u->pidx.at("final_conv.1.weight")].off;
    fa.bias = packed + u->params[u->pidx.at("final_conv.1.bias")].off;
    fa.B = B; fa.H = c.n_support_points; fa.D = c.state_dim; fa.C = c.unet_input_dim;
    fa.Hc = u->Hc;
    return launch_final_step(fa, st);
}
int launch_final_step(const FinalArgs& fa, hipStream_t st) {
    const int n = fa.B * fa.H;
    const size_t lds = (size_t)(fa.D * fa.C + fa.D) * sizeof(float);
    hipLaunchKernelGGL(final_step_kernel, dim3((n + 255) / 256), dim3(256), lds, st, fa);
    return 0;
}

static long long* g_fused_trace = nullptr;
static int g_fused_trace_seg = -1;

__global__ __launch_bounds__(256) void restream_all_kernel(float* __restrict__ packed, const CopyJobDev* __restrict__ jobs) {
    restream_job(packed, jobs[blockIdx.y], blockIdx.x * 256u + threadIdx.x, gridDim.x * 256u);
}

static int ensure_stream_jobs(mpdx_unet* u) {
    if (!u->jobs_dev) {
        std::vector<CopyJobDev> all;
        for (const auto& f : u->fused)
            for (const auto& j : f.jobs) all.push_back({(unsigned long long)j.src, (unsigned long long)j.dst, j.n0, j.ss0, j.ds0, j.n1, j.ss1, j.ds1, j.n_inner});
        u->n_jobs = (int)all.size();
        if (u->n_jobs) {
            HIP_TRY(hipMalloc(&u->jobs_dev, all.size() * sizeof(CopyJobDev)));
            HIP_TRY(hipMemcpy(u->jobs_dev, all.data(), all.size() * sizeof(CopyJobDev), hipMemcpyHostToDevice));
        }
    }
    return 0;
}
int ensure_fused_streams(mpdx_unet* u, const float* packed, hipStream_t st) {
    if (u->streams_for == packed && u->streams_version == u->pack_version) return 0;
    if (int rc = ensure_stream_jobs(u)) return rc;
    if (u->n_jobs)
        hipLaunchKernelGGL(restream_all_kernel, dim3(64, (unsigned)u->n_jobs), dim3(256), 0, st, const_cast<float*>(packed), (const CopyJobDev*)u->jobs_dev);
    HIP_TRY(hipGetLastError());
    u->streams_for = packed; u->streams_version = u->pack_version;
    return 0;
}
int claim_fused_stream_jobs(mpdx_unet* u, const float* packed, const void** jobs, int* n) {
    *jobs = nullptr; *n = 0;
    if (u->streams_for == packed && u->streams_version == u->pack_version) return 0;
    if (int rc = ensure_stream_jobs(u)) return rc;
    *jobs = u->jobs_dev; *n = u->n_jobs;
    u->streams_for = packed; u->streams_version = u->pack_version;
    return 0;
}

bool fused_save_variant(const mpdx_unet::Fused& f) { return f.program == 0 || f.program == 3 || f.program == 5 || f.program == 6 || f.program < 0; }
static int fill_fused_args(mpdx_unet* u, const mpdx_unet::Fused& f, const float* packed, const float* tt_row, const float* x, float* ws,
                           int B, const FinalArgs* fa, FusedArgs& a) {
    const size_t slot = u->slot_floats * (size_t)B;
    auto src = [&](int s) -> const float* { return s == SRC_X ? x : (s == SRC_NONE ? nullptr : ws + slot * s); };
    a = f.tmpl;
    a.packed = packed; a.tt_row = tt_row;
    a.gsrc1 = src(f.in1); a.gsrc2 = src(f.in2);
    a.gsrc3 = f.in3 != SRC_NONE ? src(f.in3) : a.gsrc1;
    for (int k = 0; k < 3; ++k) a.gout[k] = f.gout_slot[k] >= 0 ? ws + slot * f.gout_slot[k] : nullptr;
    a.B = B;
    a.trace = (g_fused_trace && (g_fused_trace_seg < 0 || g_fused_trace_seg == (int)(&f - &u->fused[0]))) ? g_fused_trace : nullptr;
    if (f.has_final) {
        if (!fa) return fail(MPDX_E_STATE, "fused final segment needs the step arguments");
        a.x_in = fa->x_in; a.noise = fa->noise; a.hs = fa->hs; a.hg = fa->hg; a.out = fa->out; a.chain = fa->chain;
        a.absmax = fa->absmax; a.fmode = fa->mode; a.n_per_ctx = fa->n_per_ctx > 0 ? fa->n_per_ctx : B; a.k = fa->k;
        a.rng = fa->rng;
    }
    return 0;
}
static int run_fused(mpdx_unet* u, const mpdx_unet::Fused& f, const float* packed, const float* tt_row, const float* x, float* ws,
                     int B, const FinalArgs* fa, hipStream_t st) {
    if (int rc = ensure_fused_streams(u, packed, st)) return rc;
    FusedArgs a;
    if (int rc = fill_fused_args(u, f, packed, tt_row, x, ws, B, fa, a)) return rc;
    return launch_fused_args(f, a, B, st);
}
static int run_index(int width) { return width == kRunNarrow ? 1 : 0; }
static int inner_run_resident(int cus, int width, int wgs_per_cu) { return cus * std::min(width == kRunNarrow ? 2 : 1, wgs_per_cu); }
static int inner_run_counter_lines(int cus, int width) { return inner_run_resident(cus, width, 2) / 8 + 8; }
static size_t inner_run_counter_bytes(int cus, int width) { return (size_t)inner_run_counter_lines(cus, width) * kInnerRunCounterStride * sizeof(unsigned); }
static int inner_run_create(mpdx_unet::InnerRunState& r, int cus) {
    if (r.capacity >= 0) return 0;
    r.capacity = 0;
    int dev = 0, khz = 0;
    if (cus <= 0 || hipGetDevice(&dev) != hipSuccess || hipDeviceGetAttribute(&khz, hipDeviceAttributeClockRate, dev) != hipSuccess)
        return (void)hipGetLastError(), 0;
    bool any = false;
    for (int width : {kRunWide, kRunNarrow}) {
        r.seven_wgs[run_index(width)] = inner_run_workgroups_per_cu(width);
        r.tail_wgs[run_index(width)] = tail_run_workgroups_per_cu(width);
        any = any || r.seven_wgs[run_index(width)] > 0 || r.tail_wgs[run_index(width)] > 0;
    }
    if (!any) return 0;
    const size_t bytes = inner_run_counter_bytes(cus, kRunWide) + inner_run_counter_bytes(cus, kRunNarrow);
    HIP_TRY(hipMalloc((void**)&r.counters, bytes));
    HIP_TRY(hipMemset(r.counters, 0, bytes));
    r.ctr[0].p = r.counters;
    r.ctr[1].p = r.counters + inner_run_counter_lines(cus, kRunWide) * kInnerRunCounterStride;
    HIP_TRY(hipHostMalloc((void**)&r.status, 64, hipHostMallocMapped));
    *r.status = r.status_host;
    HIP_TRY(hipHostGetDevicePointer((void**)&r.status_dev, r.status, 0));
    r.budget = 4LL * (khz > 0 ? khz : 2400000);
    r.capacity = cus;
    return 0;
}
static int inner_run_begin(mpdx_unet::InnerRunState& r, int width, int nc, int n_layers, hipStream_t st, unsigned** counters_out, unsigned* base_out) {
    mpdx_unet::InnerRunState::Counters& k = r.ctr[run_index(width)];
    if (nc > inner_run_counter_lines(r.capacity, width)) return fail(MPDX_E_STATE, "run of width %d: %d clusters, %d counter lines", width, nc, inner_run_counter_lines(r.capacity, width));
    if (k.rezero || nc > k.live) {
        HIP_TRY(hipMemsetAsync(k.p, 0, inner_run_counter_bytes(r.capacity, width), st));
        k.base = 0; k.rezero = false;
    }
    k.live = nc;
    *counters_out = k.p;
    *base_out = k.base;
    k.base += 8u * (unsigned)n_layers;
    return 0;
}
static void inner_run_free(mpdx_unet::InnerRunState& r) {
    if (r.counters) (void)hipFree(r.counters);
    if (r.status) (void)hipHostFree(r.status);
}
static int handle_status_error(const mpdx_unet* u, const char* fn) {
    const unsigned w = u->run.status_word();
    if (!w) return 0;
    return fail(MPDX_E_DEVICE, "%s: a workgroup of an inner-level run or of the paired joined launch gave up its wait (status 0x%x: layer %u of the run, or down op %u of the paired launch); the outputs of that plan hold NaN. "
                "mpdx_unet_set_status(u, 0) clears the word", fn, w, w >> 8, w >> 8);
}
static int level_split_create(mpdx_unet* u, int cus) {
    mpdx_unet::LevelSplitState& s = u->split;
    if (s.capacity >= 0) return 0;
    s.capacity = 0;
    if (int rc = inner_run_create(u->run, cus)) return rc;
    if (u->run.capacity <= 0 || !u->run.status_dev) return 0;
    s.wgs = fused_join_split_workgroups_per_cu();
    if (s.wgs < 1) return 0;
    HIP_TRY(hipMalloc((void**)&s.xch, (size_t)kSplitMaxB * kSplitTrajFloats * sizeof(float)));
    HIP_TRY(hipMalloc((void**)&s.counters, (size_t)kSplitMaxB * kInnerRunCounterStride * sizeof(unsigned)));
    HIP_TRY(hipMemset(s.counters, 0, (size_t)kSplitMaxB * kInnerRunCounterStride * sizeof(unsigned)));
    s.capacity = cus;
    return 0;
}
static void level_split_free(mpdx_unet::LevelSplitState& s) {
    if (s.xch) (void)hipFree(s.xch);
    if (s.counters) (void)hipFree(s.counters);
}
static int level_split_begin(mpdx_unet::LevelSplitState& s, int B, hipStream_t st, unsigned* base_out) {
    if (B > kSplitMaxB) return fail(MPDX_E_STATE, "paired joined launch of %d trajectories (at most %d)", B, kSplitMaxB);
    if (s.rezero || B > s.live) {
        HIP_TRY(hipMemsetAsync(s.counters, 0, (size_t)kSplitMaxB * kInnerRunCounterStride * sizeof(unsigned), st));
        s.base = 0; s.rezero = false;
    }
    s.live = B;
    *base_out = s.base;
    s.base += kSplitAdvance;
    return 0;
}
static int run_fused_join(mpdx_unet* u, const mpdx_unet::Fused& up, const mpdx_unet::Fused& dn, const float* packed, const float* tt_row, const float* tt_next,
                          const float* x, float* ws, int B, const FinalArgs* fa, hipStream_t st, long long* trace = nullptr, bool split = false) {
    if (int rc = ensure_fused_streams(u, packed, st)) return rc;
    FusedJoinArgs ja;
    FusedArgs d;
    if (int rc = fill_fused_args(u, up, packed, tt_row, x, ws, B, fa, ja.up)) return rc;
    if (int rc = fill_fused_args(u, dn, packed, tt_next, x, ws, B, nullptr, d)) return rc;
    ja.up.trace = trace;
    ja.dn.packed = d.packed; ja.dn.tt_row = d.tt_row;
    for (int k = 0; k < 3; ++k) ja.dn.gout[k] = d.gout[k];
    ja.dn.gpar_off = d.gpar_off; ja.dn.tt_lo = d.tt_lo;
    for (int k = 0; k < kMaxFusedOps; ++k) ja.dn.sbase[k] = k < d.nops ? d.ops[k].sbase : 0;
    if (!split) return launch_fused_join(ja, B, st);
    FusedSplitArgs sa;
    memset(&sa, 0, sizeof(sa));
    if (int rc = level_split_begin(u->split, B, st, &sa.base)) return rc;
    sa.xch = u->split.xch; sa.counters = u->split.counters; sa.status = u->run.status_dev; sa.budget = u->run.budget; sa.nb8 = split_nb8(B);
    return launch_fused_join_split(ja, sa, B, st);
}

static long long* g_run_trace = nullptr;
static int g_run_trace_kind = -1;
constexpr int kRunTraceSlots = 32;
template <int N>
static int fill_run_args(mpdx_unet* u, int kind, int first, int width, const float* packed, const float* row, const float* x, float* ws, int B, hipStream_t st, RunArgs<N>& ra) {
    memset(&ra, 0, sizeof(ra));
    if (!inner_run_width_ok(width)) return fail(MPDX_E_STATE, "run unit of width %d", width);
    const int nc = inner_run_clusters(B, width);
    for (int k = 0; k < N; ++k) {
        if (int rc = make_conv_args(u, u->layers[first + k], packed, row, x, ws, B, 0, ra.layer[k])) return rc;
        ra.layer[k].n_tiles_n = nc;
        ra.layer[k].trace = g_run_trace && g_run_trace_kind == kind ? g_run_trace + k * kRunTraceSlots : nullptr;
    }
    ra.n_layers = N; ra.nc = nc;
    if (int rc = inner_run_begin(u->run, width, nc, N, st, &ra.counters, &ra.base)) return rc;
    ra.status = u->run.status_dev; ra.budget = u->run.budget;
    u->inner_run_layers += N;
    return 0;
}
static int run_inner_run(mpdx_unet* u, int first, int width, const float* packed, const float* row, const float* x, float* ws, int B, hipStream_t st) {
    InnerRunArgs ra;
    if (int rc = fill_run_args(u, mpdx_unet::kInnerRun, first, width, packed, row, x, ws, B, st, ra)) return rc;
    u->inner_runs++;
    return launch_inner_run(ra, B, width, st);
}
static int run_tail_run(mpdx_unet* u, int first, int spare, int width, const float* packed, const float* row, const float* x, float* ws, int B, hipStream_t st) {
    TailRunArgs ra;
    if (spare < 0 || spare >= u->n_slots) return fail(MPDX_E_STATE, "tail run without a spare slot");
    if (int rc = fill_run_args(u, mpdx_unet::kTailRun, first, width, packed, row, x, ws, B, st, ra)) return rc;
    float* const sp = ws + u->slot_floats * (size_t)B * spare;
    ra.layer[0].dst = sp; ra.layer[1].src1 = sp; ra.layer[2].res = sp;
    return launch_tail_run(ra, B, width, st);
}

static int run_unit(mpdx_unet* u, const mpdx_unet::Unit& un, const float* packed, const float* row, const float* x, float* ws, int B,
                    const FinalArgs* fa, hipStream_t st) {
    if (un.kind == mpdx_unet::kProgram) return run_fused(u, u->fused[un.fused], packed, row, x, ws, B, fa, st);
    if (un.kind == mpdx_unet::kPair) return run_pair(u, u->layers[un.layer], u->layers[un.layer + 1], packed, row, x, ws, B, st);
    if (un.kind == mpdx_unet::kInnerRun) return run_inner_run(u, un.layer, un.width, packed, row, x, ws, B, st);
    if (un.kind == mpdx_unet::kTailRun) return run_tail_run(u, un.layer, un.fused, un.width, packed, row, x, ws, B, st);
    return run_layer(u, u->layers[un.layer], packed, row, x, ws, B, st);
}
static double unit_flops(const mpdx_unet* u, const mpdx_unet::Unit& un, int B) {
    double fl = 0.0;
    for (int k = un.layer; k < un.layer + un.count; ++k) fl += layer_flops(u->layers[k], B);
    return fl;
}

static double layer_param_bytes(const mpdx_unet* u, const Layer& l) {
    if (l.attn) return 4.0 * ((double)u->params[l.w].n + (double)u->params[l.w2].n + 3.0 * l.cout);
    double n = (double)u->params[l.w].n + l.cout;
    if (l.gamma >= 0) n += 2.0 * l.cout;
    if (l.tb_off >= 0) n += l.cout;
    return 4.0 * n;
}
static double unit_bytes(const mpdx_unet* u, const mpdx_unet::Unit& un, int B) {
    auto act = [&](int L, int C) { return 4.0 * B * (double)L * C; };
    if (un.kind == mpdx_unet::kProgram) {
        const auto& f = u->fused[un.fused];
        const Layer& l0 = u->layers[f.first];
        double b = act(l0.L_in, l0.c1 + l0.c2);
        if (f.in3_consumer >= 0) b += act(u->layers[f.in3_consumer].L_in, u->layers[f.in3_consumer].c2);
        for (int k = f.first; k < f.first + f.count; ++k) b += layer_param_bytes(u, u->layers[k]);
        for (int k = 0; k < f.tmpl.nops; ++k)
            if (f.tmpl.ops[k].shape != kFusedShapeFinal && f.tmpl.ops[k].gdst >= 0) {
                const Layer& l = u->layers[f.op_layer[k]];
                b += act(l.L_out, l.cout);
            }
        if (f.has_final) b += 3.0 * act(u->cfg.n_support_points, u->cfg.state_dim);
        return b;
    }
    double b = 0.0;
    for (int k = un.layer; k < un.layer + un.count; ++k) {
        const Layer& l = u->layers[k];
        b += layer_param_bytes(u, l) + act(l.L_out, l.cout) + (l.res != SRC_NONE ? act(l.L_out, l.cout) : 0.0);
        if (k == un.layer || un.kind != mpdx_unet::kPair) b += act(l.L_in, l.c1 + l.c2);
    }
    return b;
}

enum PassEvent { kSkipUnit, kBeforeLaunch, kAfterLaunch };
static int no_hook(PassEvent, int) { return 0; }
template <class Hook>
static int walk_pass(mpdx_unet* u, const std::vector<mpdx_unet::Unit>& units, const float* packed, const float* row, const float* x, float* ws,
                     int B, FinalArgs& fa, hipStream_t st, Hook&& hook, bool first_done = false, const float* next_row = nullptr,
                     long long* join_trace = nullptr, bool split = false) {
    const int n = (int)units.size();
    bool final_done = false;
    for (int i = first_done ? 1 : 0; i < n; ++i) {
        const mpdx_unet::Unit& un = units[i];
        if (un.kind == mpdx_unet::kProgram) final_done |= u->fused[un.fused].has_final;
        if (hook(kSkipUnit, i)) continue;
        if (int rc = hook(kBeforeLaunch, i)) return rc;
        const int rc = next_row && i == n - 1 ? run_fused_join(u, u->fused[un.fused], u->fused[units[0].fused], packed, row, next_row, x, ws, B, &fa, st, join_trace, split)
                                              : run_unit(u, un, packed, row, x, ws, B, &fa, st);
        if (rc) return rc;
        if (int rc = hook(kAfterLaunch, i)) return rc;
    }
    if (final_done) return 0;
    if (int rc = hook(kBeforeLaunch, n)) return rc;
    if (int rc = run_final(u, packed, fa, B, ws, st)) return rc;
    return hook(kAfterLaunch, n);
}

static const float* padded_input(const mpdx_unet* u, const float* x, float* ws, int B, hipStream_t st) {
    if (!u->masked()) return x;
    float* xc = ws + u->slot_floats * (size_t)B * u->xpad_slot;
    const size_t nx = (size_t)B * u->Hc * u->cfg.state_dim;
    hipLaunchKernelGGL(pad_input_kernel, dim3((unsigned)std::min<size_t>((nx + 255) / 256, 2048)), dim3(256), 0, st, x, xc, B, u->cfg.n_support_points, u->Hc,
                       u->cfg.state_dim);
    return xc;
}
static int run_unet_and_final(mpdx_unet* u, const float* packed, const float* timetab, int T, const float* x, int t, int B,
                              float* ws, FinalArgs& fa, hipStream_t st) {
    if (int rc = check_ready(u)) return rc;
    if (t < 0 || t >= T) return fail(MPDX_E_INVALID, "timestep %d outside [0,%d)", t, T);
    if (B <= 0) return fail(MPDX_E_INVALID, "B must be positive");
    return walk_pass(u, current_units(u, B, nullptr), packed, timetab + (size_t)t * u->tt_row, padded_input(u, x, ws, B, st), ws, B, fa, st, no_hook);
}

static int inner_run_first(const mpdx_unet* u, const std::vector<mpdx_unet::Unit>& units) {
    auto fits = [&](const mpdx_unet::Unit& un) {
        if (un.kind != mpdx_unet::kLayer) return false;
        const Layer& l = u->layers[un.layer];
        if (l.attn || !(l.mode == CONV_S1 && l.ks == 5 && l.epi == EPI_GN_MISH) || l.Lv_out) return false;
        if (!(l.c1 == 256 && l.c2 == 0 && l.src2 == SRC_NONE && l.cout == 256 && l.L_in == 8 && l.L_out == 8 && l.gs == 32 && l.cin_pad == 256 && l.rs == 264)) return false;
        if ((l.tb_off >= 0) == (l.res != SRC_NONE)) return false;
        return layer_ksplit(l);
    };
    const int n = (int)units.size();
    for (int i = 0; i + kInnerRunLayers <= n; ++i) {
        int k = 0;
        while (k < kInnerRunLayers && fits(units[i + k])) ++k;
        if (k == kInnerRunLayers) return i;
    }
    return -1;
}
static int tail_run_first(const mpdx_unet* u, const std::vector<mpdx_unet::Unit>& units, int* spare) {
    *spare = -1;
    auto layer_of = [&](const mpdx_unet::Unit& un) -> const Layer* {
        if (un.kind != mpdx_unet::kLayer) return nullptr;
        const Layer& l = u->layers[un.layer];
        if (l.attn || l.Lv_out || !(l.c1 == 128 && l.c2 == 0 && l.src2 == SRC_NONE && l.cout == 128 && l.L_in == 8 && l.cin_pad == 128)) return nullptr;
        return &l;
    };
    auto fits_gn = [&](const mpdx_unet::Unit& un) {
        const Layer* l = layer_of(un);
        if (!l || !(l->mode == CONV_S1 && l->ks == 5 && l->epi == EPI_GN_MISH && l->L_out == 8 && l->gs == 16 && l->rs == 136)) return false;
        if ((l->tb_off >= 0) == (l->res != SRC_NONE)) return false;
        return layer_ksplit(*l);
    };
    auto fits_up = [&](const mpdx_unet::Unit& un) {
        const Layer* l = layer_of(un);
        return l && l->mode == CONV_UPT && l->ks == 4 && l->epi == EPI_BIAS && l->L_out == 16 && l->rs == 132 && l->res == SRC_NONE && l->tb_off < 0;
    };
    const int n = (int)units.size();
    for (int i = 0; i + kTailRunLayers <= n; ++i) {
        int k = 0;
        while (k < kTailRunLayers - 1 && fits_gn(units[i + k])) ++k;
        if (!(k == kTailRunLayers - 1 && fits_up(units[i + k]))) continue;
        const int f = units[i].layer;
        const Layer &l0 = u->layers[f], &l1 = u->layers[f + 1], &l2 = u->layers[f + 2], &l3 = u->layers[f + 3];
        if (units[i + 1].layer != f + 1 || units[i + 2].layer != f + 2 || units[i + 3].layer != f + 3) continue;
        if (!(l1.src1 == l0.dst && l2.src1 == l1.dst && l2.res == l0.dst && l3.src1 == l2.dst && l0.res != SRC_NONE && l1.res == SRC_NONE)) continue;
        std::vector<int> kept = {l0.dst, l1.dst, l2.dst};
        auto drop = [&](int s) { kept.erase(std::remove(kept.begin(), kept.end(), s), kept.end()); };
        auto held = [&](int s) { return std::find(kept.begin(), kept.end(), s) != kept.end(); };
        if (l0.dst == l1.dst || l1.dst == l2.dst || l0.dst == l2.dst) continue;
        drop(l3.dst);
        bool read_later = false;
        for (int j = f + kTailRunLayers; j < (int)u->layers.size() && !read_later; ++j) {
            const Layer& l = u->layers[j];
            read_later = held(l.src1) || held(l.src2) || held(l.res);
            drop(l.dst);
        }
        if (read_later || held(u->final_slot)) continue;
        auto named = [&](const Layer& l, int s) { return l.src1 == s || l.src2 == s || l.res == s || l.dst == s; };
        for (int s = 0; s < u->n_slots && *spare < 0; ++s) {
            if (s == u->xpad_slot || named(l0, s) || named(l1, s) || named(l2, s) || named(l3, s)) continue;
            bool dead = s != u->final_slot;
            for (int j = f + kTailRunLayers; j < (int)u->layers.size() && dead; ++j) {
                const Layer& l = u->layers[j];
                if (l.src1 == s || l.src2 == s || l.res == s) dead = false;
                else if (l.dst == s) break;
            }
            if (dead) *spare = s;
        }
        if (*spare < 0 || l3.dst == l1.dst || l3.dst == l2.dst || l3.dst == l0.src1 || l3.dst == l0.res) { *spare = -1; continue; }
        return i;
    }
    return -1;
}
static int device_cus() {
    int dev = 0, cus = 0;
    if (hipGetDevice(&dev) != hipSuccess || hipDeviceGetAttribute(&cus, hipDeviceAttributeMultiprocessorCount, dev) != hipSuccess) (void)hipGetLastError();
    return cus;
}
static int inner_run_auto_width(int B) { return (void)B, kRunNarrow; }
static int tail_run_auto_width(int B) { return B <= 64 ? kRunNarrow : kRunWide; }
static bool level_split_auto(int B) { return B <= kSplitMaxB; }
struct PlanSchedule {
    std::vector<mpdx_unet::Unit> units;
    bool run = false;
    bool join = false;
    bool split = false;
    int build(mpdx_unet* u, int B, bool with_run = true) {
        units = current_units(u, B, nullptr);
        const int cus = device_cus();
        if (with_run && u->inner_run && !u->masked() && !u->cfg.self_attention && u->cfg.n_levels == 4 && u->cfg.n_support_points == 64) {
            if (int rc = inner_run_create(u->run, cus)) return rc;
            const bool may = u->run.capacity > 0 && sw::geo() && !sw::debug();
            auto width_of = [&](const int (&wgs)[2], int automatic) {
                auto fits = [&](int w) { return may && inner_run_grid(B, w) <= inner_run_resident(u->run.capacity, w, wgs[run_index(w)]); };
                if (u->inner_run_width) return fits(u->inner_run_width) ? u->inner_run_width : 0;
                return fits(automatic) ? automatic : fits(kRunWide) ? kRunWide : 0;
            };
            const int sw7 = width_of(u->run.seven_wgs, inner_run_auto_width(B)), swt = width_of(u->run.tail_wgs, tail_run_auto_width(B));
            const int rf = sw7 && (u->inner_run & mpdx_unet::kRunSeven) ? inner_run_first(u, units) : -1;
            if (rf >= 0) {
                units[rf] = {mpdx_unet::kInnerRun, -1, units[rf].layer, kInnerRunLayers, sw7};
                units.erase(units.begin() + rf + 1, units.begin() + rf + kInnerRunLayers);
                run = true;
            }
            int spare = -1;
            const int tf = swt && (u->inner_run & mpdx_unet::kRunTail) ? tail_run_first(u, units, &spare) : -1;
            if (tf >= 0) {
                units[tf] = {mpdx_unet::kTailRun, spare, units[tf].layer, kTailRunLayers, swt};
                units.erase(units.begin() + tf + 1, units.begin() + tf + kTailRunLayers);
                run = true;
            }
        }
        if (!u->plan_join || u->masked() || units.size() < 2) return 0;
        const mpdx_unet::Unit &first = units.front(), &last = units.back();
        if (first.kind != mpdx_unet::kProgram || last.kind != mpdx_unet::kProgram || first.fused == last.fused) return 0;
        const mpdx_unet::Fused &dn = u->fused[first.fused], &up = u->fused[last.fused];
        join = dn.program == 5 && dn.in1 == SRC_X && dn.in2 == SRC_NONE && !dn.has_final && up.program == 3 && up.has_final && B <= cus;
        const bool want = u->level_split > 0 || (u->level_split < 0 && level_split_auto(B));
        if (join && want && u->cfg.state_dim <= 16 && split_grid(B) <= cus && B <= kSplitMaxB && sw::geo() && !sw::debug()) {
            if (int rc = level_split_create(u, cus)) return rc;
            split = u->split.capacity > 0 && split_grid(B) <= u->split.capacity * std::min(1, u->split.wgs);
        }
        return 0;
    }
};

int dev_hooks_missing(const char* fn) {
#ifdef MPDX_DEV_HOOKS
    return (void)fn, 0;
#endif
    return fail(MPDX_E_STATE, "%s needs a development build of libmpdx.so (MPDX_BUILD_DEFS=-DMPDX_DEV_HOOKS MPDX_BUILD_OUT=build_ab/libmpdx_dev.so python -m mpd_public_amd.build, then MPDX_LIB=build_ab/libmpdx_dev.so): "
                "the production kernels carry no trace / ablation hooks", fn);
}

}

using namespace mpdx;

#include "unet_measure.hpp"

extern "C" {

const char* mpdx_last_error(void) { return g_err; }
int mpdx_version(void) { return 1; }

int mpdx_unet_create(const mpdx_unet_cfg* cfg, mpdx_unet** out) {
    if (!cfg || !out) return fail(MPDX_E_INVALID, "null argument");
    if (cfg->n_levels < 2 || cfg->n_levels > MPDX_MAX_LEVELS) return fail(MPDX_E_INVALID, "n_levels %d unsupported", cfg->n_levels);
    if (cfg->state_dim < 1 || cfg->state_dim > 64) return fail(MPDX_E_INVALID, "state_dim %d unsupported", cfg->state_dim);
    if (cfg->time_emb_dim != 32) return fail(MPDX_E_INVALID, "time_emb_dim must be 32 (TimeEncoder(32, .), temporal_unet.py:66)");
    if (cfg->unet_input_dim % 16) return fail(MPDX_E_INVALID, "unet_input_dim must be a multiple of 16");
    if (cfg->self_attention != 0 && cfg->self_attention != 1) return fail(MPDX_E_INVALID, "self_attention must be 0 or 1");
    if (cfg->dim_mults[0] != 1) return fail(MPDX_E_INVALID, "dim_mults[0] must be 1: final_conv takes unet_input_dim channels (temporal_unet.py:113-116)");
    for (int i = 0; i < cfg->n_levels; ++i)
        if (cfg->dim_mults[i] < 1) return fail(MPDX_E_INVALID, "dim_mults[%d] = %d", i, cfg->dim_mults[i]);
    const int H = cfg->n_support_points;
    if (H < 16 || H > 128 || (H % (1 << (cfg->n_levels - 1))) || (H >> (cfg->n_levels - 1)) < 2)
        return fail(MPDX_E_INVALID, "n_support_points %d must be a multiple of 2^(levels-1) = %d in [16, 128] with >= 2 points at the coarsest level", H,
                    1 << (cfg->n_levels - 1));
    for (int lv = 1; lv < cfg->n_levels; ++lv)
        if (2 * cfg->dim_mults[lv] == cfg->dim_mults[lv - 1])
            return fail(MPDX_E_INVALID, "layer ups.%d.0: identity residual over a concatenation (dim_mults[%d] = %d is twice dim_mults[%d] = %d, so the block "
                        "has no residual_conv) unsupported", cfg->n_levels - 1 - lv, lv - 1, cfg->dim_mults[lv - 1], lv, cfg->dim_mults[lv]);
    mpdx_unet* u = new mpdx_unet();
    u->cfg = *cfg;
    build_model(u);
    for (const Layer& l : u->layers)
        if (l.epi == EPI_GN_MISH) {
            const int re = l.gs * l.L_out;
            if (re < 64 || re > 2048 || (re & (re - 1)) || l.gs < 4 || 32 % l.gs) {
                std::string nm = l.name;
                delete u;
                return fail(MPDX_E_INVALID, "layer %s: GroupNorm region of %d elements (group of %d) unsupported", nm.c_str(), re, l.gs);
            }
        }
    for (const Layer& l : u->layers)
        if (l.attn)
            if (const char* why = attn_unsupported(l.cout, l.L_out)) {
                const std::string nm = l.name;
                const int ch = l.cout, np = l.L_out;
                delete u;
                return fail(MPDX_E_INVALID, "self-attention block %s (%d channels on %d positions): %s", nm.c_str(), ch, np, why);
            }
    if ((int)u->tt_w.size() > 40) { delete u; return fail(MPDX_E_INVALID, "too many residual blocks"); }
    build_units(u);
    u->packed_floats += 64;
    *out = u;
    return 0;
}

int mpdx_unet_set_plan_join(mpdx_unet* u, int on) {
    if (!u) return fail(MPDX_E_INVALID, "null argument");
    u->plan_join = on ? 1 : 0;
    return 0;
}
int mpdx_unet_plan_joined(const mpdx_unet* u) { return u ? u->plan_joined : 0; }
int mpdx_unet_set_level_split(mpdx_unet* u, int on) {
    if (!u) return fail(MPDX_E_INVALID, "null argument");
    u->level_split = on < 0 ? -1 : on ? 1 : 0;
    return 0;
}
int mpdx_unet_plan_split(const mpdx_unet* u) { return u ? u->plan_split : 0; }
int mpdx_level_split_block(int B, int block, int32_t* trajectory, int32_t* role) {
    if (B <= 0 || B > kSplitMaxB) return fail(MPDX_E_INVALID, "mpdx_level_split_block: B=%d", B);
    const int grid = split_grid(B);
    if (block < 0 || block >= grid) return fail(MPDX_E_INVALID, "mpdx_level_split_block: block %d of %d", block, grid);
    const SplitSlot s = split_slot(block, split_nb8(B));
    if (trajectory) *trajectory = s.b < B ? s.b : -1;
    if (role) *role = s.role;
    return grid;
}

int mpdx_unet_set_inner_run(mpdx_unet* u, int on) {
    if (!u) return fail(MPDX_E_INVALID, "null argument");
    u->inner_run = on ? (mpdx_unet::kRunSeven | mpdx_unet::kRunTail) : 0;
    return 0;
}
int mpdx_unet_set_inner_run_parts(mpdx_unet* u, int parts) {
    if (!u) return fail(MPDX_E_INVALID, "null argument");
    if (parts & ~(mpdx_unet::kRunSeven | mpdx_unet::kRunTail)) return fail(MPDX_E_INVALID, "inner-run parts 0x%x: bit 0 the seven 256 -> 256 layers, bit 1 the tail of up level 0", parts);
    u->inner_run = parts;
    return 0;
}
int mpdx_unet_set_inner_run_width(mpdx_unet* u, int width) {
    if (!u) return fail(MPDX_E_INVALID, "null argument");
    if (width != 0 && !inner_run_width_ok(width)) return fail(MPDX_E_INVALID, "inner-run width %d: 0 (automatic), 16 or 32 positions per cluster", width);
    u->inner_run_width = width;
    return 0;
}
int mpdx_inner_run_block(int B, int width, int cus, int block, int32_t* cluster, int32_t* tile, int32_t* counter_lines) {
    if (B <= 0 || cus <= 0 || !inner_run_width_ok(width)) return fail(MPDX_E_INVALID, "mpdx_inner_run_block: B=%d width=%d cus=%d", B, width, cus);
    const int grid = inner_run_grid(B, width);
    if (block < 0 || block >= grid) return fail(MPDX_E_INVALID, "mpdx_inner_run_block: block %d of %d", block, grid);
    int c = 0, m = 0;
    inner_run_slot(block, &c, &m);
    if (cluster) *cluster = c < inner_run_clusters(B, width) ? c : -1;
    if (tile) *tile = m;
    if (counter_lines) *counter_lines = inner_run_counter_lines(cus, width);
    return grid;
}
int mpdx_unet_inner_runs(const mpdx_unet* u) { return u ? u->inner_runs : 0; }
int mpdx_unet_inner_run_layers(const mpdx_unet* u) { return u ? u->inner_run_layers : 0; }
int mpdx_unet_status(const mpdx_unet* u) {
    if (!u) return fail(MPDX_E_INVALID, "null argument");
    return handle_status_error(u, "mpdx_unet_status");
}
int mpdx_unet_set_status(mpdx_unet* u, unsigned word) {
    if (!u) return fail(MPDX_E_INVALID, "null argument");
    if (u->run.status) __atomic_store_n(u->run.status, word, __ATOMIC_RELAXED);
    u->run.status_host = word;
    if (!word && u->run.counters) u->run.ctr[0].rezero = u->run.ctr[1].rezero = true;
    if (!word) u->split.rezero = true;
    return 0;
}

void mpdx_unet_destroy(mpdx_unet* u) {
    if (u && u->pack_descs_dev) (void)hipFree(u->pack_descs_dev);
    if (u && u->pack_chunks_dev) (void)hipFree(u->pack_chunks_dev);
    if (u && u->jobs_dev) (void)hipFree(u->jobs_dev);
    if (u) inner_run_free(u->run);
    if (u) level_split_free(u->split);
    delete u;
}

int mpdx_unet_num_params(const mpdx_unet* u) { return u ? (int)u->params.size() : 0; }

int mpdx_unet_param_info(const mpdx_unet* u, int idx, const char** name, int32_t shape[3], int32_t* ndim) {
    if (!u || idx < 0 || idx >= (int)u->params.size()) return fail(MPDX_E_INVALID, "bad parameter index %d", idx);
    const Param& p = u->params[idx];
    if (name) *name = p.name.c_str();
    if (shape) { shape[0] = p.shape[0]; shape[1] = p.shape[1]; shape[2] = p.shape[2]; }
    if (ndim) *ndim = p.ndim;
    return 0;
}

size_t mpdx_unet_packed_floats(const mpdx_unet* u) { return u ? u->packed_floats : 0; }
size_t mpdx_unet_timetab_floats(const mpdx_unet* u, int T) { return u ? (size_t)T * u->tt_row : 0; }
size_t mpdx_unet_workspace_floats(const mpdx_unet* u, int B) { return u ? u->slot_floats * (size_t)B * u->n_slots : 0; }

int mpdx_unet_pack_param(mpdx_unet* u, const char* name, const float* src, size_t n, float* packed, void* stream) {
    if (!u || !name || !src || !packed) return fail(MPDX_E_INVALID, "null argument");
    auto it = u->pidx.find(name);
    if (it == u->pidx.end()) return fail(MPDX_E_NOTFOUND, "unexpected state-dict key '%s'", name);
    Param& p = u->params[it->second];
    if (n != p.n) return fail(MPDX_E_INVALID, "'%s': got %zu floats, expected %zu", name, n, p.n);
    hipStream_t st = (hipStream_t)stream;
    if (p.kind == PK_VEC) {
        hipLaunchKernelGGL(copy_kernel, dim3((unsigned)std::min<size_t>((p.n + 255) / 256, 1024)), dim3(256), 0, st, src, packed + p.off, p.n);
    } else {
        hipLaunchKernelGGL(pack_conv_weights_kernel, dim3((unsigned)std::min<size_t>((p.pn + 255) / 256, 2048)), dim3(256), 0, st, src,
                           packed + p.off, p.cout, p.cin, p.ksz, p.cin_pad, p.nslot, p.kind == PK_CONVT ? 1 : 0);
    }
    HIP_TRY(hipGetLastError());
    if (!p.done) { p.done = true; u->n_done++; }
    u->pack_version++;
    return 0;
}

int mpdx_unet_build_timetab(mpdx_unet* u, const float* packed, const float* freqs16, int T, float* timetab, void* stream) {
    if (!u || !packed || !freqs16 || !timetab || T <= 0) return fail(MPDX_E_INVALID, "bad argument");
    if (int rc = check_ready(u)) return rc;
    TimeTabArgs a;
    memset(&a, 0, sizeof(a));
    a.packed = packed; a.freqs = freqs16; a.tab = timetab;
    a.w1 = (int)u->params[u->pidx.at("time_mlp.encoder.1.weight")].off;
    a.b1 = (int)u->params[u->pidx.at("time_mlp.encoder.1.bias")].off;
    a.w2 = (int)u->params[u->pidx.at("time_mlp.encoder.3.weight")].off;
    a.b2 = (int)u->params[u->pidx.at("time_mlp.encoder.3.bias")].off;
    a.row = u->tt_row;
    a.nblk = (int)u->tt_w.size();
    for (int i = 0; i < a.nblk; ++i) {
        a.woff[i] = (int)u->params[u->tt_w[i]].off;
        a.boff[i] = (int)u->params[u->tt_b[i]].off;
        a.cout[i] = u->tt_cout[i];
        a.toff[i] = u->tt_off[i];
    }
    hipLaunchKernelGGL(timetab_kernel, dim3(T), dim3(128), 0, (hipStream_t)stream, a);
    HIP_TRY(hipGetLastError());
    return 0;
}

int mpdx_unet_forward(mpdx_unet* u, const float* packed, const float* timetab, int T, const float* x, int t, float* eps,
                      int B, float* ws, void* stream) {
    if (!u || !packed || !timetab || !x || !eps || !ws) return fail(MPDX_E_INVALID, "null argument");
    hipStream_t st = (hipStream_t)stream;
    FinalArgs fa;
    memset(&fa, 0, sizeof(fa));
    fa.out = eps; fa.mode = 0; fa.n_per_ctx = 1;
    if (int rc = run_unet_and_final(u, packed, timetab, T, x, t, B, ws, fa, st)) return rc;
    HIP_TRY(hipGetLastError());
    return 0;
}

int mpdx_ddpm_step(mpdx_unet* u, const float* packed, const float* timetab, int T, float* x_io, const float* noise,
                   const float* hard_start, const float* hard_goal, const mpdx_step_coefs* coefs, int t, int mean_only,
                   float* chain_out, uint32_t* absmax_out, int n_per_ctx, int B, float* ws, void* stream) {
    if (!u || !packed || !timetab || !x_io || !coefs || !ws) return fail(MPDX_E_INVALID, "null argument");
    hipStream_t st = (hipStream_t)stream;
    FinalArgs fa;
    memset(&fa, 0, sizeof(fa));
    fa.x_in = x_io; fa.out = x_io; fa.noise = noise; fa.hs = hard_start; fa.hg = hard_goal;
    fa.chain = chain_out; fa.absmax = absmax_out; fa.n_per_ctx = n_per_ctx > 0 ? n_per_ctx : B;
    fa.mode = mean_only == 2 ? 3 : (mean_only ? 2 : 1);
    fa.k = *coefs;
    if (int rc = run_unet_and_final(u, packed, timetab, T, x_io, t, B, ws, fa, st)) return rc;
    HIP_TRY(hipGetLastError());
    return 0;
}

int mpdx_add_noise(float* x_io, const float* noise, const float* hard_start, const float* hard_goal, float noise_scale,
                   float noise_std_extra, float* chain_out, int B, int H, int D, void* stream) {
    if (!x_io || B <= 0) return fail(MPDX_E_INVALID, "bad argument");
    const size_t n = (size_t)B * H * D;
    hipLaunchKernelGGL(add_noise_kernel, dim3((unsigned)std::min<size_t>((n + 255) / 256, 2048)), dim3(256), 0, (hipStream_t)stream,
                       x_io, noise, hard_start, hard_goal, noise_scale, noise_std_extra, chain_out, B, H, D);
    HIP_TRY(hipGetLastError());
    return 0;
}

int mpdx_hard_conds(float* x_io, float* chain_out, int n, const int32_t* horizon_idx, const float* const* values, int B, int H, int D, void* stream) {
    if (!x_io || B <= 0 || H <= 0 || D <= 0 || n < 0 || (n && (!horizon_idx || !values))) return fail(MPDX_E_INVALID, "bad argument");
    if (n > kMaxHardConds) return fail(MPDX_E_INVALID, "at most 16 hard conditions per call");
    if (n == 0) return 0;
    HardCondArgs a;
    memset(&a, 0, sizeof(a));
    a.n = n;
    for (int k = 0; k < n; ++k) {
        int t = horizon_idx[k];
        if (t < 0) t += H;
        if (t < 0 || t >= H) return fail(MPDX_E_INVALID, "hard condition index out of range for this horizon");
        if (!values[k]) return fail(MPDX_E_INVALID, "null hard condition table");
        a.idx[k] = t; a.vals[k] = values[k];
    }
    const size_t per = (size_t)B * D;
    hipLaunchKernelGGL(hard_conds_kernel, dim3((unsigned)std::min<size_t>((per + 255) / 256, 1024)), dim3(256), 0, (hipStream_t)stream, x_io, chain_out, a, B, H, D);
    HIP_TRY(hipGetLastError());
    return 0;
}

int mpdx_q_sample(const float* x_start, const float* noise, const long long* t_dev, const float* sqrt_alphas_cumprod_dev,
                  const float* sqrt_one_minus_alphas_cumprod_dev, const float* hard_start, const float* hard_goal, float* out, int B, int H,
                  int D, int T, void* stream) {
    if (!x_start || !noise || !t_dev || !sqrt_alphas_cumprod_dev || !sqrt_one_minus_alphas_cumprod_dev || !out || B <= 0 || T <= 0)
        return fail(MPDX_E_INVALID, "bad argument");
    const size_t n = (size_t)B * H * D;
    hipLaunchKernelGGL(q_sample_kernel, dim3((unsigned)std::min<size_t>((n + 255) / 256, 2048)), dim3(256), 0, (hipStream_t)stream, x_start, noise,
                       t_dev, sqrt_alphas_cumprod_dev, sqrt_one_minus_alphas_cumprod_dev, hard_start, hard_goal, out, B, H, D, T);
    HIP_TRY(hipGetLastError());
    return 0;
}

int mpdx_weighted_loss(const float* pred, const float* targ, const float* weights_hd, const float* hard_start, const float* hard_goal,
                       int l1, float* out1, int B, int H, int D, void* stream) {
    if (!pred || !targ || !out1 || B <= 0) return fail(MPDX_E_INVALID, "bad argument");
    hipLaunchKernelGGL(weighted_loss_kernel, dim3(1), dim3(1024), 0, (hipStream_t)stream, pred, targ, weights_hd, hard_start, hard_goal, l1, out1,
                       B, H, D);
    HIP_TRY(hipGetLastError());
    return 0;
}

int mpdx_plan(mpdx_unet* u, const float* packed, const float* timetab, int T, const mpdx_step_coefs* coefs, int n_without_noise,
              float* x, const float* noise, const float* hard_start, const float* hard_goal, float* chain, int B, float* ws,
              const mpdx_guide_params* guide, int n_guide_steps, int t_start_guide, uint32_t* guide_flags, int n_per_ctx,
              uint64_t rng_seed, uint64_t rng_offset, void* stream) {
    if (!u || !packed || !timetab || !coefs || !x || !ws || T <= 0 || n_without_noise < 0 || B <= 0)
        return fail(MPDX_E_INVALID, "bad argument");
    if (int rc = handle_status_error(u, "mpdx_plan")) return rc;
    if (guide)
        if (const char* why = motion_params_problem(*guide, u->cfg.n_support_points)) return fail(MPDX_E_INVALID, "%s", why);
    if (guide)
        if (const char* why = scene_params_problem(*guide)) return fail(MPDX_E_INVALID, "%s", why);
    if (guide)
        if (const char* why = chain_params_problem(*guide)) return fail(MPDX_E_INVALID, "%s", why);
    if (guide)
        if (const char* why = tool_params_problem(*guide)) return fail(MPDX_E_INVALID, "%s", why);
    if (int rc = check_ready(u)) return rc;
    PlanSchedule ps;
    if (int rc = ps.build(u, B)) return rc;
    u->inner_runs = u->inner_run_layers = u->plan_joined = u->plan_split = 0;
    hipStream_t st = (hipStream_t)stream;
    const int H = u->cfg.n_support_points, D = u->cfg.state_dim;
    const size_t n = (size_t)B * H * D;
    const int npc = n_per_ctx > 0 ? n_per_ctx : B;
    const int n_ctx = (B + npc - 1) / npc;
    const int steps = T + n_without_noise;
    if (n_guide_steps < 0) return fail(MPDX_E_INVALID, "n_guide_steps %d", n_guide_steps);
    if (n_guide_steps == 0) guide = nullptr;
    const int dbg = sw::debug();
    if (guide) {
        if (!guide_flags) return fail(MPDX_E_INVALID, "guide needs guide_flags");
        if (B % npc) return fail(MPDX_E_INVALID, "B=%d is not a multiple of n_per_ctx=%d", B, npc);
        HIP_TRY(hipMemsetAsync(guide_flags, 0, (size_t)steps * (n_guide_steps + 1) * n_ctx * sizeof(uint32_t), st));
    }
    hipLaunchKernelGGL(add_noise_kernel, dim3((unsigned)std::min<size_t>((n + 255) / 256, 2048)), dim3(256), 0, st, x, (const float*)nullptr,
                       hard_start, hard_goal, 0.f, 0.f, chain, B, H, D);
    bool down_done = false;
    int k = 0;
    for (int i = T - 1; i >= -n_without_noise; --i, ++k) {
        const int t = i < 0 ? 0 : i;
        const bool guided = guide && i < t_start_guide;
        const bool join = ps.join && !guided && i > -n_without_noise;
        const float* tt_next = join ? timetab + (size_t)(i - 1 < 0 ? 0 : i - 1) * u->tt_row : nullptr;
        const float* nz = (t == 0 || !noise) ? nullptr : noise + (size_t)k * n;
        NoiseRng rng;
        memset(&rng, 0, sizeof(rng));
        if (!noise && t != 0) { rng.on = 1; rng.seed = rng_seed; rng.offset = rng_offset; rng.elem0 = (unsigned long long)(k + 1) * n; }
        float* ch = chain ? chain + (size_t)(k + 1) * n : nullptr;
        uint32_t* fl = guided ? guide_flags + (size_t)k * (n_guide_steps + 1) * n_ctx : nullptr;
        FinalArgs fa;
        memset(&fa, 0, sizeof(fa));
        fa.x_in = x; fa.out = x;
        fa.k = coefs[t];
        fa.n_per_ctx = npc;
        if (!guided) {
            fa.rng = rng; fa.noise = nz; fa.hs = hard_start; fa.hg = hard_goal;
            fa.chain = ch; fa.mode = 1;
        } else {
            fa.mode = 2; fa.absmax = fl;
        }
        if (int rc = walk_pass(u, ps.units, packed, timetab + (size_t)t * u->tt_row, padded_input(u, x, ws, B, st), ws, B, fa, st, no_hook, down_done, tt_next, nullptr, ps.split))
            return rc;
        down_done = join;
        u->plan_joined += join ? 1 : 0;
        u->plan_split += join && ps.split ? 1 : 0;
        if (guided) {
            for (int j = 0; j < n_guide_steps; ++j) {
                const bool last = j == n_guide_steps - 1;
                if (int rc = launch_guide(guide, x, nullptr, hard_start, hard_goal, fl + (size_t)j * n_ctx, fl + (size_t)(j + 1) * n_ctx, npc, B, H,
                                          D, st, last ? nz : nullptr, coefs[t].noise_scale, coefs[t].noise_std_extra, last ? ch : nullptr,
                                          coefs[t].guide_scale, last ? &rng : nullptr))
                    return rc;
            }
        }
        if (dbg) {
            if (dbg >= 2) {
                const hipError_t e = hipStreamSynchronize(st);
                if (e != hipSuccess) return fail((int)e, "mpdx_plan: loop iteration %d (t=%d%s) faulted: %s", k, t, guided ? ", guided" : "", hipGetErrorString(e));
            }
            hipError_t e = hipGetLastError();
            if (e != hipSuccess) return fail((int)e, "mpdx_plan: launch in loop iteration %d (t=%d%s) failed: %s", k, t, guided ? ", guided" : "", hipGetErrorString(e));
        }
    }
    HIP_TRY(hipGetLastError());
    return ps.run || ps.split ? handle_status_error(u, "mpdx_plan") : 0;
}

int mpdx_randn(float* out, size_t n, uint64_t seed, uint64_t offset, void* stream) {
    if (!out) return fail(MPDX_E_INVALID, "null argument");
    if (n == 0) return 0;
    const size_t nquad = (n + 3) / 4;
    hipLaunchKernelGGL(randn_kernel, dim3((unsigned)std::min<size_t>((nquad + 255) / 256, 4096)), dim3(256), 0, (hipStream_t)stream, out, n,
                       seed, offset);
    HIP_TRY(hipGetLastError());
    return 0;
}

int mpdx_attention_block(float* x, const float* to_qkv_w, const float* to_out_w, const float* to_out_b, const float* norm_g, const float* norm_b,
                         int B, int L, int Lv, int C, void* stream) {
    if (!x || !to_qkv_w || !to_out_w || !to_out_b || !norm_g || !norm_b) return fail(MPDX_E_INVALID, "null argument");
    if (B <= 0) return fail(MPDX_E_INVALID, "batch must be positive");
    if (const char* why = attn_unsupported(C, L)) return fail(MPDX_E_INVALID, "self-attention block (%d channels on %d positions): %s", C, L, why);
    if (Lv < 1 || Lv > L) return fail(MPDX_E_INVALID, "valid positions must be in [1, %d]", L);
    hipStream_t st = (hipStream_t)stream;
    Layer l;
    l.name = "mpdx_attention_block"; l.attn = true; l.mode = CONV_S1; l.ks = 0; l.epi = EPI_BIAS;
    l.c1 = C; l.cout = C; l.L_in = L; l.L_out = L;
    l.Lv_out = Lv != L ? Lv : 0;
    l.cin_pad = pad_cin(C);
    l.rs = pick_row_stride(l.cin_pad, CONV_S1, L, L, L);
    const int hid_pad = pad_cin(kAttnHid);
    const size_t n_qkv = (size_t)(3 * kAttnHid / 16) * (l.cin_pad / 16) * 256, n_out = (size_t)(C / 16) * (hid_pad / 16) * 256;
    float* packed = nullptr;
    HIP_TRY(hipMalloc(&packed, (n_qkv + n_out) * sizeof(float)));
    hipLaunchKernelGGL(pack_conv_weights_kernel, dim3((unsigned)std::min<size_t>((n_qkv + 255) / 256, 2048)), dim3(256), 0, st, to_qkv_w, packed,
                       3 * kAttnHid, C, 1, l.cin_pad, 1, 0);
    hipLaunchKernelGGL(pack_conv_weights_kernel, dim3((unsigned)std::min<size_t>((n_out + 255) / 256, 2048)), dim3(256), 0, st, to_out_w, packed + n_qkv,
                       C, kAttnHid, 1, hid_pad, 1, 0);
    AttnArgs aa;
    memset(&aa, 0, sizeof(aa));
    aa.x = x; aa.wqkv = packed; aa.wout = packed + n_qkv; aa.bout = to_out_b; aa.g = norm_g; aa.b = norm_b;
    int rc = launch_attention(l, aa, B, st);
    hipError_t e = hipGetLastError();
    const hipError_t es = hipStreamSynchronize(st);
    if (e == hipSuccess) e = es;
    (void)hipFree(packed);
    if (rc) return rc;
    if (e != hipSuccess) return fail((int)e, "mpdx_attention_block: %s", hipGetErrorString(e));
    return 0;
}

}
```

### mpd_public_amd/temporal_unet.py

```python
from __future__ import annotations

import ctypes as C
import math

import torch
import torch.nn as nn

from . import _lib

UNET_DIM_MULTS = {0: (1, 2, 4), 1: (1, 2, 4, 8)}


def group_norm_n_groups(n_channels, target_n_groups=8):
    if n_channels < target_n_groups:
        return 1
    for n_groups in range(target_n_groups, target_n_groups + 10):
        if n_channels % n_groups == 0:
            return n_groups
    return 1


class _Holder(nn.Module):

    def forward(self, *a, **k):
        raise RuntimeError("parameter holder - TemporalUnet.forward runs libmpdx kernels, not torch modules")


def _seq_with(**at):
    n = max(int(k) for k in at) + 1
    return nn.Sequential(*[at.get(str(i), nn.Identity()) for i in range(n)])


def _conv_block(cin, cout, k=5):
    m = _Holder()
    m.block = _seq_with(**{"0": nn.Conv1d(cin, cout, k, padding=k // 2), "2": nn.GroupNorm(group_norm_n_groups(cout), cout), "4": nn.Identity()})
    return m


def _res_block(cin, cout, cond_dim):
    m = _Holder()
    m.blocks = nn.ModuleList([_conv_block(cin, cout), _conv_block(cout, cout)])
    m.cond_mlp = _seq_with(**{"1": nn.Linear(cond_dim, cout), "2": nn.Identity()})
    m.residual_conv = nn.Conv1d(cin, cout, 1) if cin != cout else nn.Identity()
    return m


SELF_ATTENTION_TRAINING_REFUSAL = ("self-attention network: the training pass has no backward for the self-attention blocks "
                                   "(self_attention=True runs inference and evaluation only)")


class _LayerNormHolder(_Holder):
    def __init__(self, dim):
        super().__init__()
        self.g = nn.Parameter(torch.ones(1, dim, 1))
        self.b = nn.Parameter(torch.zeros(1, dim, 1))


def _self_attention(dim, heads=4, dim_head=32):
    hidden = heads * dim_head
    res, pre, att = _Holder(), _Holder(), _Holder()
    att.to_qkv = nn.Conv1d(dim, hidden * 3, 1, bias=False)
    att.to_out = nn.Conv1d(hidden, dim, 1)
    pre.fn = att
    pre.norm = _LayerNormHolder(dim)
    res.fn = pre
    return res


def _resample(dim, up):
    m = _Holder()
    m.conv = nn.ConvTranspose1d(dim, dim, 4, 2, 1) if up else nn.Conv1d(dim, dim, 3, 2, 1)
    return m


class TemporalUnet(nn.Module):
    def __init__(self, n_support_points=None, state_dim=None, unet_input_dim=32, dim_mults=(1, 2, 4, 8), time_emb_dim=32,
                 self_attention=False, conditioning_embed_dim=4, conditioning_type=None, attention_num_heads=2,
                 attention_dim_head=32, **kwargs):
        super().__init__()
        if conditioning_type not in (None, "None"):
            raise NotImplementedError("mpd_public_amd.TemporalUnet: only conditioning_type=None is supported "
                                      "(the only configuration the reference scripts build)")
        self.self_attention = bool(self_attention)
        attn = (lambda dim: _self_attention(dim)) if self.self_attention else (lambda dim: nn.Identity())
        self.state_dim = state_dim
        self.conditioning_type = None
        self.n_support_points = n_support_points
        self.unet_input_dim = unet_input_dim
        self.dim_mults = tuple(int(m) for m in dim_mults)
        self.time_emb_dim = time_emb_dim

        dims = [state_dim] + [unet_input_dim * m for m in self.dim_mults]
        in_out = list(zip(dims[:-1], dims[1:]))
        n_res = len(in_out)

        self.time_mlp = _Holder()
        self.time_mlp.encoder = _seq_with(**{"1": nn.Linear(32, 32 * 4), "3": nn.Linear(32 * 4, time_emb_dim)})
        self.downs = nn.ModuleList()
        for i, (ci, co) in enumerate(in_out):
            last = i >= n_res - 1
            self.downs.append(nn.ModuleList([_res_block(ci, co, time_emb_dim), _res_block(co, co, time_emb_dim), attn(co),
                                             nn.Identity(), _resample(co, up=False) if not last else nn.Identity()]))
        self.ups = nn.ModuleList()
        for ci, co in reversed(in_out[1:]):
            self.ups.append(nn.ModuleList([_res_block(co * 2, ci, time_emb_dim), _res_block(ci, ci, time_emb_dim), attn(ci),
                                           nn.Identity(), _resample(ci, up=True)]))
        mid = dims[-1]
        self.mid_block1 = _res_block(mid, mid, time_emb_dim)
        self.mid_attn = attn(mid)
        self.mid_attention = nn.Identity()
        self.mid_block2 = _res_block(mid, mid, time_emb_dim)
        self.final_conv = nn.Sequential(_conv_block(unet_input_dim, unet_input_dim), nn.Conv1d(unet_input_dim, state_dim, 1))

        self._h = None
        self._packed = None
        self._timetab = None
        self._timetab_T = 0
        self._ws = None
        self._ws_B = 0
        self._stamp = None
        try:
            self._handle()
        except _lib.LibraryUnavailable:
            pass

    _DEVICE_STATE = {"_h": None, "_packed": None, "_timetab": None, "_timetab_T": 0, "_ws": None, "_ws_B": 0, "_stamp": None}

    def __getstate__(self):
        state = dict(self.__dict__)
        state.update(self._DEVICE_STATE)
        return state

    def __setstate__(self, state):
        self.__dict__.update(state)
        self.__dict__.update(self._DEVICE_STATE)

    def __del__(self):
        try:
            if getattr(self, "_h", None):
                _lib.load().mpdx_unet_destroy(self._h)
        except Exception:
            pass

    def _handle(self):
        if self._h is None:
            lib = _lib.load()
            mults = (C.c_int32 * _lib.MAX_LEVELS)(*self.dim_mults)
            cfg = _lib.UnetCfg(int(self.state_dim), int(self.n_support_points), int(self.unet_input_dim), len(self.dim_mults),
                               mults, int(self.time_emb_dim), int(self.self_attention))
            h = C.c_void_p()
            _lib.check(lib.mpdx_unet_create(C.byref(cfg), C.byref(h)), "mpdx_unet_create")
            self._h = h
        return self._h

    def set_plan_join(self, on: bool):
        _lib.check(_lib.load().mpdx_unet_set_plan_join(self._handle(), int(bool(on))), "mpdx_unet_set_plan_join")

    def plan_joined(self) -> int:
        return int(_lib.load().mpdx_unet_plan_joined(self._handle()))

    def set_level_split(self, on):
        _lib.check(_lib.load().mpdx_unet_set_level_split(self._handle(), -1 if on is None else int(bool(on))), "mpdx_unet_set_level_split")

    def plan_split(self) -> int:
        return int(_lib.load().mpdx_unet_plan_split(self._handle()))

    def set_inner_run(self, on: bool):
        _lib.check(_lib.load().mpdx_unet_set_inner_run(self._handle(), int(bool(on))), "mpdx_unet_set_inner_run")

    RUN_SEVEN, RUN_TAIL = 1, 2

    def set_inner_run_parts(self, parts: int):
        _lib.check(_lib.load().mpdx_unet_set_inner_run_parts(self._handle(), int(parts)), "mpdx_unet_set_inner_run_parts")

    def set_inner_run_width(self, width: int):
        _lib.check(_lib.load().mpdx_unet_set_inner_run_width(self._handle(), int(width)), "mpdx_unet_set_inner_run_width")

    def inner_runs(self) -> int:
        return int(_lib.load().mpdx_unet_inner_runs(self._handle()))

    def inner_run_layers(self) -> int:
        return int(_lib.load().mpdx_unet_inner_run_layers(self._handle()))

    def status(self) -> int:
        return int(_lib.load().mpdx_unet_status(self._handle()))

    def _param_stamp(self):
        d = self.__dict__
        n = d.get("_stamp_calls", 0) + 1
        d["_stamp_calls"] = n
        pl = d.get("_plist")
        if pl is None or n % 16 == 0:
            pl = d["_plist"] = list(self.parameters())
        return tuple((p.data_ptr(), p._version) for p in pl)

    def _apply(self, fn, *a, **k):
        self.__dict__["_plist"] = None
        return super()._apply(fn, *a, **k)

    def load_state_dict(self, *a, **k):
        r = super().load_state_dict(*a, **k)
        self.__dict__["_plist"] = None
        return r

    def engine(self, T: int, B: int):
        lib, h = _lib.load(), self._handle()
        dev = next(self.parameters()).device
        if dev.type != "cuda":
            raise RuntimeError("mpd_public_amd.TemporalUnet runs on an AMD GPU only (move the model to 'cuda'); there is no CPU fallback")
        st = _lib.current_stream()
        frozen = self.__dict__.get("_weights_frozen", False) and self._packed is not None and self._stamp is not None
        stamp = self._stamp if frozen else self._param_stamp()
        if self._packed is None or self._stamp != stamp or self._packed.device != dev:
            packed = torch.zeros(lib.mpdx_unet_packed_floats(h), dtype=torch.float32, device=dev)
            sd = self.state_dict()
            n = lib.mpdx_unet_num_params(h)
            if n != len(sd):
                raise RuntimeError(f"state dict has {len(sd)} tensors, libmpdx expects {n}")
            for name, t in sd.items():
                t = t.detach().to(device=dev, dtype=torch.float32).contiguous()
                _lib.check(lib.mpdx_unet_pack_param(h, name.encode(), t.data_ptr(), t.numel(), packed.data_ptr(), st), f"pack {name}")
            self._packed, self._stamp, self._timetab, self._timetab_T = packed, stamp, None, 0
        if self._timetab is None or self._timetab_T < T:
            T_tab = max(int(T), 128)
            tab = torch.empty(lib.mpdx_unet_timetab_floats(h, T_tab), dtype=torch.float32, device=dev)
            half = 16
            freqs = torch.exp(torch.arange(half) * -(math.log(10000) / (half - 1))).to(device=dev, dtype=torch.float32)
            _lib.check(lib.mpdx_unet_build_timetab(h, self._packed.data_ptr(), freqs.data_ptr(), T_tab, tab.data_ptr(), st), "timetab")
            torch.cuda.current_stream().synchronize()
            self._timetab, self._timetab_T = tab, T_tab
        if self._ws is None or self._ws_B < B or self._ws.device != dev:
            self._ws = torch.empty(lib.mpdx_unet_workspace_floats(h, B), dtype=torch.float32, device=dev)
            self._ws_B = B
        return h, self._packed, self._timetab, self._ws

    def forward(self, x, time, context=None):
        if context is not None:
            raise NotImplementedError("context conditioning is not supported (context is always None on this path, inference.py:182)")
        b, h, d = x.shape
        if h != self.n_support_points or d != self.state_dim:
            raise ValueError(f"expected [B,{self.n_support_points},{self.state_dim}], got {tuple(x.shape)}")
        x = x.to(torch.float32).contiguous()
        from .diffusion_model import timestep_hint
        hint = timestep_hint(time)
        tl = [hint] * int(time.numel()) if hint is not None and time.numel() in (1, b) else time.reshape(-1).tolist()
        if len(tl) not in (1, b):
            raise ValueError(f"time must have 1 or {b} entries, got {len(tl)}")
        out = torch.empty_like(x)
        lib = _lib.load()

        def run(xg, t0, og):
            hdl, packed, tab, ws = self.engine(t0 + 1, xg.shape[0])
            _lib.check(lib.mpdx_unet_forward(hdl, packed.data_ptr(), tab.data_ptr(), self._timetab_T, xg.data_ptr(), t0,
                                             og.data_ptr(), xg.shape[0], ws.data_ptr(), _lib.current_stream()), "mpdx_unet_forward")

        distinct = sorted(set(int(v) for v in tl))
        if len(distinct) == 1:
            run(x, distinct[0], out)
            return out
        self.engine(distinct[-1] + 1, b)
        tt = torch.as_tensor(tl, device=x.device)
        for t0 in distinct:
            idx = (tt == t0).nonzero(as_tuple=True)[0]
            xg = x.index_select(0, idx).contiguous()
            og = torch.empty_like(xg)
            run(xg, t0, og)
            out.index_copy_(0, idx, og)
        return out
```

Before: 6659 denoising-steps/s.

## Fold the up-level-0 residual pair into the persistent tail run as its head

Adds a 'head' stage to the persistent tail-run kernel. It computes the level's first k5 GroupNorm-Mish conv together with the 1x1 residual conv in one block, reusing the staged input tile in LDS, and then continues into the existing four tail layers. This removes a separate pair launch and its global round trip before the tail run. The cost is a larger LDS footprint, which needs a raised LDS limit and may lower occupancy, plus extra registers for the 1x1 weights and accumulators. The schedule applies it only when a strict shape and slot check passes, and the narrow width is the default.

```diff
diff --git a/include/mpdx.h b/include/mpdx.h
--- a/include/mpdx.h
+++ b/include/mpdx.h
@@ -43,6 +43,7 @@
 int    mpdx_inner_run_block(int B, int width, int cus, int block, int32_t* cluster, int32_t* tile, int32_t* counter_lines);
 int    mpdx_unet_inner_runs(const mpdx_unet* u);
 int    mpdx_unet_inner_run_layers(const mpdx_unet* u);
+int    mpdx_unet_inner_run_heads(const mpdx_unet* u);
 int    mpdx_unet_status(const mpdx_unet* u);
 int    mpdx_unet_set_status(mpdx_unet* u, unsigned word);
 int    mpdx_unet_num_params(const mpdx_unet* u);
diff --git a/mpd_public_amd/_lib.py b/mpd_public_amd/_lib.py
--- a/mpd_public_amd/_lib.py
+++ b/mpd_public_amd/_lib.py
@@ -109,6 +109,7 @@
     "mpdx_inner_run_block": (_i, [_i, _i, _i, _i, _vp, _vp, _vp]),
     "mpdx_unet_inner_runs": (_i, [_vp]),
     "mpdx_unet_inner_run_layers": (_i, [_vp]),
+    "mpdx_unet_inner_run_heads": (_i, [_vp]),
     "mpdx_unet_status": (_i, [_vp]),
     "mpdx_unet_set_status": (_i, [_vp, C.c_uint]),
     "mpdx_unet_num_params": (_i, [_vp]),
diff --git a/mpd_public_amd/csrc/conv_block.hpp b/mpd_public_amd/csrc/conv_block.hpp
--- a/mpd_public_amd/csrc/conv_block.hpp
+++ b/mpd_public_amd/csrc/conv_block.hpp
@@ -178,8 +178,10 @@
 
 typedef unsigned u32x4 __attribute__((ext_vector_type(4)));
 
-template <int MODE, int KS, int EPI, int MT, int NT, int WN, int WK, class GEO = GeoAny, int TBRES = -1, bool RUN = false>
-__device__ __forceinline__ bool conv_block_body(const ConvArgs& a, const int block_id, const RunCtx rc = RunCtx()) {
+template <int MODE, int KS, int EPI, int MT, int NT, int WN, int WK, class GEO = GeoAny, int TBRES = -1, bool RUN = false, bool HEAD = false>
+__device__ __forceinline__ bool conv_block_body(const ConvArgs& a, const int block_id, const RunCtx rc = RunCtx(), const ConvArgs* const a2 = nullptr) {
+    static_assert(!HEAD || (RUN && MODE == CONV_S1 && KS == 5 && EPI == EPI_GN_MISH && MT == 16 && GEO::NC16 % WK == 0 && NT * (MT / 4) <= 64 * WN * WK),
+                  "a run's head: k5 GroupNorm block + the 1x1 residual conv on 16-channel tiles, the 1x1's k-groups split evenly, one bias element per thread");
     using G = ConvGeom<MODE, KS>;
     constexpr bool GK = GEO::L > 0;
     static_assert(!GK || MODE == CONV_S1 || MODE == CONV_UPT, "compile-time geometry: stride-1 and transposed convolutions on 8 input positions");
@@ -243,6 +245,10 @@
 #ifdef MPDX_RING_FIRST
     ring_init();
 #endif
+    constexpr int NIT1 = HEAD ? GEO::NC16 / WK : 1;
+    f32x4 hf[NIT1][MS];
+    f32x4 head_bi = {0.f, 0.f, 0.f, 0.f};
+    (void)hf; (void)head_bi;
     f32x4 run_bi = {0.f, 0.f, 0.f, 0.f}, run_ga = run_bi, run_be = run_bi, run_tb = run_bi;
     f32x2 run_bi2 = {0.f, 0.f}, run_ga2 = run_bi2, run_be2 = run_bi2, run_tb2 = run_bi2;
     constexpr bool RUN_UP = RUN && MODE == CONV_UPT;
@@ -325,7 +331,11 @@
             }
 #pragma unroll
             for (int u = 0; u < SB; ++u) {
-                if constexpr (RUN) {
+                if constexpr (HEAD) {
+                    constexpr int CH = GEO::NC16 * 8;
+                    const float* src = (cc[u] < CH) ? a.src1 + pos[u] * CH + cc[u] : a.src2 + pos[u] * CH + (cc[u] - CH);
+                    v[u] = *(const f32x4*)src;
+                } else if constexpr (RUN) {
                     const __amdgpu_buffer_rsrc_t srs = __builtin_amdgcn_make_buffer_rsrc((void*)a.src1, 0, 0x7fffffff, 0x00020000);
                     if constexpr (GEO::NC16 == 8) {
                         const int fo = (rc.tiled & 1) ? run_tiled_off((int)pos[u], cc[u]) : (int)(pos[u] * (GEO::NC16 * 16) + cc[u]);
@@ -377,6 +387,15 @@
 #ifndef MPDX_RING_FIRST
     if (!RUN && MPDX_DBG(a, 1)) ring_init();
 #endif
+    if constexpr (HEAD) {
+        const __amdgpu_buffer_rsrc_t wrs2 = __builtin_amdgcn_make_buffer_rsrc((void*)a2->wp, 0, 0x7fffffff, 0x00020000);
+#pragma unroll
+        for (int it = 0; it < NIT1; ++it)
+#pragma unroll
+            for (int m = 0; m < MS; ++m)
+                hf[it][m] = __builtin_bit_cast(f32x4, __builtin_amdgcn_raw_buffer_load_b128(wrs2, wlane, ((mt * MS + m) * GEO::NC16 + wk + it * WK) * 1024, 0));
+        head_bi = *(const f32x4*)(a2->bias + mt * MT + (tid & (MT / 4 - 1)) * 4);
+    }
     CB_STAMP();
     __syncthreads();
     CB_STAMP();
@@ -402,6 +421,8 @@
     }
 
     f32x4 acc[MS][NSW];
+    f32x4 acc2[HEAD ? MS : 1][HEAD ? NSW : 1];
+    (void)acc2;
 #pragma unroll
     for (int m = 0; m < MS; ++m)
 #pragma unroll
@@ -434,6 +455,27 @@
             for (int it = 0; it < NIT; ++it) {
                 kgroup(wk + it * WK, af[it % PF]);
                 if (it + PF < NIT) load_a(wk + (it + PF) * WK, af[it % PF]);
+            }
+        }
+        if constexpr (HEAD) {
+#pragma unroll
+            for (int m = 0; m < MS; ++m)
+#pragma unroll
+                for (int i = 0; i < NSW; ++i) acc2[m][i] = (f32x4){0.f, 0.f, 0.f, 0.f};
+            if (!MPDX_DBG(a, 2)) {
+#pragma unroll
+                for (int it = 0; it < NIT1; ++it) {
+                    const int c16 = wk + it * WK;
+#pragma unroll
+                    for (int i = 0; i < NSW; ++i) {
+                        const f32x4 bf = smem4[boff[i] + PAD * RS4 + c16 * 4];
+#pragma unroll
+                        for (int e = 0; e < 4; ++e)
+#pragma unroll
+                            for (int m = 0; m < MS; ++m)
+                                acc2[m][i] = __builtin_amdgcn_mfma_f32_16x16x4f32(hf[it][m][e], bf[e], acc2[m][i], 0, 0, 0);
+                    }
+                }
             }
         }
     } else
@@ -777,6 +819,31 @@
         }
     }
     CB_STAMP();
+    if constexpr (HEAD) {
+        __syncthreads();
+#pragma unroll
+        for (int m = 0; m < MS; ++m)
+#pragma unroll
+            for (int i = 0; i < NSW; ++i)
+                smem4[(wk * NT + npos[i]) * MTP4 + m * 4 + q] = acc2[m][i];
+        __syncthreads();
+        constexpr int M4 = MT / 4;
+        if (tid < NT * M4) {
+            const int n = tid / M4, c = (tid - n * M4) * 4;
+            const int s = n >> lg_Lout, l = n & (L_out - 1), b = s0 + s;
+            const int co = mt * MT + c;
+            const int ri = n * MTP4 + (c >> 2);
+            f32x4 v = smem4[ri];
+#pragma unroll
+            for (int k = 1; k < WK; ++k) v += smem4[ri + k * NT * MTP4];
+            v += head_bi;
+            if (b < a.B) {
+                const int o = (rc.tiled & 8) ? run_tiled_off(b * 8 + l, co) : (b * L_out + l) * a.C_out + co;
+                const __amdgpu_buffer_rsrc_t drs = __builtin_amdgcn_make_buffer_rsrc((void*)a2->dst, 0, 0x7fffffff, 0x00020000);
+                __builtin_amdgcn_raw_buffer_store_b128(__builtin_bit_cast(u32x4, v), drs, o * 4, 0, 16);
+            }
+        }
+    }
     if constexpr (RUN) {
         asm volatile("s_waitcnt vmcnt(0)" ::: "memory");
         __syncthreads();
diff --git a/mpd_public_amd/csrc/host.hpp b/mpd_public_amd/csrc/host.hpp
--- a/mpd_public_amd/csrc/host.hpp
+++ b/mpd_public_amd/csrc/host.hpp
@@ -99,14 +99,15 @@
     int Hc = 0, xpad_slot = -1;
     bool masked() const { return Hc != cfg.n_support_points; }
     int plan_join = 1;
-    enum RunPart { kRunSeven = 1, kRunTail = 2 };
-    int inner_run = kRunSeven | kRunTail;
+    enum RunPart { kRunSeven = 1, kRunTail = 2, kRunTailHead = 8, kRunAllParts = kRunSeven | kRunTail | kRunTailHead };
+    int inner_run = kRunAllParts;
     int inner_run_width = 0;
     int plan_joined = 0, inner_runs = 0;
     int inner_run_layers = 0;
+    int inner_run_heads = 0;
     struct InnerRunState {
         int capacity = -1;
-        int seven_wgs[2] = {0, 0}, tail_wgs[2] = {0, 0};
+        int seven_wgs[2] = {0, 0}, tail_wgs[2] = {0, 0}, tail_head_wgs[2] = {0, 0};
         long long budget = 0;
         unsigned* counters = nullptr;
         struct Counters {
@@ -150,7 +151,7 @@
     const float* streams_for = nullptr;
     int pack_version = 0, streams_version = -1;
     enum UnitKind { kProgram, kLayer, kPair, kInnerRun, kTailRun };
-    struct Unit { UnitKind kind; int fused; int layer; int count; int width = 0; };
+    struct Unit { UnitKind kind; int fused; int layer; int count; int width = 0; int head = 0; };
     std::vector<int> owner;
     struct TrainLayer {
         int src1_l = -2, src2_l = -2, res_l = -2;
@@ -188,8 +189,10 @@
 void inner_run_slot(int block, int* cluster, int* tile);
 int inner_run_workgroups_per_cu(int width);
 int tail_run_workgroups_per_cu(int width);
+int tail_head_run_workgroups_per_cu(int width);
 int launch_inner_run(const RunArgs<7>& ra, int B, int width, hipStream_t st);
 int launch_tail_run(const RunArgs<4>& ra, int B, int width, hipStream_t st);
+int launch_tail_head_run(const RunArgs<6>& ra, int B, int width, hipStream_t st);
 struct AttnArgs;
 const char* attn_unsupported(int C, int L);
 int launch_attention(const Layer& l, AttnArgs& a, int B, hipStream_t st);
diff --git a/mpd_public_amd/csrc/inner_run.hpp b/mpd_public_amd/csrc/inner_run.hpp
--- a/mpd_public_amd/csrc/inner_run.hpp
+++ b/mpd_public_amd/csrc/inner_run.hpp
@@ -5,6 +5,7 @@
 
 constexpr int kInnerRunLayers = 7;
 constexpr int kTailRunLayers = 4;
+constexpr int kTailHeadRunLayers = kTailRunLayers + 1;
 constexpr int kInnerRunCounterStride = 32;
 constexpr int kRunWide = 32, kRunNarrow = 16;
 
@@ -44,6 +45,7 @@
 };
 typedef RunArgs<kInnerRunLayers> InnerRunArgs;
 typedef RunArgs<kTailRunLayers> TailRunArgs;
+typedef RunArgs<kTailHeadRunLayers + 1> TailHeadRunArgs;
 
 constexpr size_t run_max(size_t a, size_t b) { return a > b ? a : b; }
 
@@ -52,7 +54,7 @@
     typedef InnerRunArgs Args;
     static constexpr int kWidth = NT, kSpt = NT / 8;
     static constexpr int kLayers = kInnerRunLayers;
-    static constexpr bool kUp = false;
+    static constexpr bool kUp = false, kHead = false;
     static constexpr int kLastL = 8, kLastMT = 32, kLastC = 256;
     static __device__ __forceinline__ bool gn(const ConvArgs& a, int id, const RunCtx& rc) { return conv_block_body<CONV_S1, 5, EPI_GN_MISH, 32, NT, 1, 8, GeoL8<16>, -1, true>(a, id, rc); }
     static __device__ __forceinline__ bool up(const ConvArgs&, int, const RunCtx&) { return true; }
@@ -64,13 +66,27 @@
     typedef TailRunArgs Args;
     static constexpr int kWidth = NT, kSpt = NT / 8;
     static constexpr int kLayers = kTailRunLayers;
-    static constexpr bool kUp = true;
+    static constexpr bool kUp = true, kHead = false;
     static constexpr int kLastL = 16, kLastMT = 16, kLastC = 128;
     static __device__ __forceinline__ bool gn(const ConvArgs& a, int id, const RunCtx& rc) { return conv_block_body<CONV_S1, 5, EPI_GN_MISH, 16, NT, 1, 8, GeoL8<8>, -1, true>(a, id, rc); }
     static __device__ __forceinline__ bool up(const ConvArgs& a, int id, const RunCtx& rc) { return conv_block_body<CONV_UPT, 4, EPI_BIAS, 16, 2 * NT, 1, 8, GeoUp8<8>, -1, true>(a, id, rc); }
     static __device__ __forceinline__ int tiled(int i) { return i >= 3 ? 1 : ((i > 0 ? 1 : 0) | (i == 2 ? 2 : 0) | 4); }
     static size_t lds() { return run_max(conv_block_lds_bytes<CONV_S1, 5, 16, NT, 8>(8, 8, 128 + 8), conv_block_lds_bytes<CONV_UPT, 4, 16, 2 * NT, 8>(8, 16, 128 + 4)) + 16; }
 };
+template <int NT>
+struct RunSeqTailHead : RunSeqTail<NT> {
+    typedef TailHeadRunArgs Args;
+    static constexpr int kLayers = kTailHeadRunLayers;
+    static constexpr bool kHead = true;
+    static __device__ __forceinline__ bool head(const ConvArgs& a, const ConvArgs& a2, int id, const RunCtx& rc) {
+        return conv_block_body<CONV_S1, 5, EPI_GN_MISH, 16, NT, 1, 8, GeoL8<32>, -1, true, true>(a, id, rc, &a2);
+    }
+    static __device__ __forceinline__ int tiled(int i) { return i == 0 ? (4 | 8) : i >= 4 ? 1 : (1 | 4 | (i != 2 ? 2 : 0)); }
+    static size_t lds() { return run_max(conv_block_lds_bytes<CONV_S1, 5, 16, NT, 8>(8, 8, 512 + 8) + 16, RunSeqTail<NT>::lds()); }
+};
+static_assert((32 * 5) % 8 == 0 && 32 % 8 == 0, "head of the tail: the k-groups of the k5 (160) and of the 1x1 (32) split evenly over the 8 waves");
+static_assert((kRunWide / 8) * 12 * 520 * sizeof(float) + 16 <= 160 * 1024 && 2 * ((kRunNarrow / 8) * 12 * 520 * sizeof(float) + 16) <= 160 * 1024,
+              "head of the tail: one window per compute unit at width 32, two at width 16");
 
 template <class SEQ>
 __device__ __forceinline__ void run_give_up(const typename SEQ::Args& ra, const RunCtx& rc, const int c, const int m, const int i) {
@@ -79,7 +95,7 @@
         __hip_atomic_fetch_or(ra.status, 1u | ((unsigned)i << 8), __ATOMIC_RELAXED, __HIP_MEMORY_SCOPE_SYSTEM);
         __hip_atomic_store(rc.counter, rc.target + kRunPoison, __ATOMIC_RELAXED, __HIP_MEMORY_SCOPE_AGENT);
     }
-    const ConvArgs& last = ra.layer[ra.n_layers - 1];
+    const ConvArgs& last = ra.layer[ra.n_layers - 1 + (SEQ::kHead ? 1 : 0)];
     constexpr int L = SEQ::kLastL, MT = SEQ::kLastMT;
     for (int e = tid; e < SEQ::kSpt * L * MT; e += 512) {
         const int b = c * SEQ::kSpt + (e >> geo_ilog2(L * MT)), l = (e >> geo_ilog2(MT)) & (L - 1), ch = m * MT + (e & (MT - 1));
@@ -99,12 +115,19 @@
     rc.counter = ra.counters + (size_t)c * kInnerRunCounterStride;
     rc.budget = ra.budget;
     const int n_gn = SEQ::kUp ? ra.n_layers - 1 : ra.n_layers;
+    constexpr int H = SEQ::kHead ? 1 : 0;
+    if constexpr (SEQ::kHead) {
+        rc.wait = 0;
+        rc.target = ra.base;
+        rc.tiled = SEQ::tiled(0);
+        (void)SEQ::head(ra.layer[0], ra.layer[1], c * 8 + m, rc);
+    }
 #pragma nounroll
-    for (int i = 0; i < n_gn; ++i) {
+    for (int i = H; i < n_gn; ++i) {
         rc.wait = i > 0;
         rc.target = ra.base + 8u * (unsigned)i;
         rc.tiled = SEQ::tiled(i);
-        if (SEQ::gn(ra.layer[i], c * 8 + m, rc)) continue;
+        if (SEQ::gn(ra.layer[i + H], c * 8 + m, rc)) continue;
         run_give_up<SEQ>(ra, rc, c, m, i);
         return;
     }
@@ -112,7 +135,7 @@
         rc.wait = n_gn > 0;
         rc.target = ra.base + 8u * (unsigned)n_gn;
         rc.tiled = SEQ::tiled(n_gn);
-        if (!SEQ::up(ra.layer[n_gn], c * 8 + m, rc)) run_give_up<SEQ>(ra, rc, c, m, n_gn);
+        if (!SEQ::up(ra.layer[n_gn + H], c * 8 + m, rc)) run_give_up<SEQ>(ra, rc, c, m, n_gn);
     }
 }
 
diff --git a/mpd_public_amd/csrc/k_inner_run.hip b/mpd_public_amd/csrc/k_inner_run.hip
--- a/mpd_public_amd/csrc/k_inner_run.hip
+++ b/mpd_public_amd/csrc/k_inner_run.hip
@@ -16,6 +16,7 @@
 template <class SEQ>
 static int workgroups_per_cu() {
     int n = 0;
+    if (SEQ::lds() > 64 * 1024 && raise_lds_limit((const void*)inner_run_kernel<SEQ, kSameXcd>)) return 0;
     if (hipOccupancyMaxActiveBlocksPerMultiprocessor(&n, (const void*)inner_run_kernel<SEQ, kSameXcd>, 512, SEQ::lds()) != hipSuccess) {
         (void)hipGetLastError();
         return 0;
@@ -28,11 +29,16 @@
 int tail_run_workgroups_per_cu(int width) {
     return width == kRunWide ? workgroups_per_cu<RunSeqTail<kRunWide>>() : width == kRunNarrow ? workgroups_per_cu<RunSeqTail<kRunNarrow>>() : 0;
 }
+int tail_head_run_workgroups_per_cu(int width) {
+    return width == kRunWide ? workgroups_per_cu<RunSeqTailHead<kRunWide>>() : width == kRunNarrow ? workgroups_per_cu<RunSeqTailHead<kRunNarrow>>() : 0;
+}
 
 template <class SEQ>
 static int launch_run(const typename SEQ::Args& ra, int B, hipStream_t st, const char* what) {
     if (ra.n_layers != SEQ::kLayers || ra.nc != run_clusters(B, SEQ::kWidth))
         return fail(MPDX_E_INVALID, "%s: %d layers, %d clusters for B=%d at width %d", what, ra.n_layers, ra.nc, B, SEQ::kWidth);
+    if (SEQ::lds() > 64 * 1024)
+        if (int rc = raise_lds_limit((const void*)inner_run_kernel<SEQ, kSameXcd>)) return rc;
     hipLaunchKernelGGL((inner_run_kernel<SEQ, kSameXcd>), dim3(run_grid(ra.nc, kSameXcd)), dim3(512), SEQ::lds(), st, ra);
     return 0;
 }
@@ -46,5 +52,10 @@
     if (width == kRunWide) return launch_run<RunSeqTail<kRunWide>>(ra, B, st, "tail run");
     return fail(MPDX_E_INVALID, "tail run: width %d", width);
 }
+int launch_tail_head_run(const TailHeadRunArgs& ra, int B, int width, hipStream_t st) {
+    if (width == kRunNarrow) return launch_run<RunSeqTailHead<kRunNarrow>>(ra, B, st, "tail run with its head");
+    if (width == kRunWide) return launch_run<RunSeqTailHead<kRunWide>>(ra, B, st, "tail run with its head");
+    return fail(MPDX_E_INVALID, "tail run with its head: width %d", width);
+}
 
 }
diff --git a/mpd_public_amd/csrc/mpdx.hip b/mpd_public_amd/csrc/mpdx.hip
--- a/mpd_public_amd/csrc/mpdx.hip
+++ b/mpd_public_amd/csrc/mpdx.hip
@@ -722,7 +722,8 @@
     for (int width : {kRunWide, kRunNarrow}) {
         r.seven_wgs[run_index(width)] = inner_run_workgroups_per_cu(width);
         r.tail_wgs[run_index(width)] = tail_run_workgroups_per_cu(width);
-        any = any || r.seven_wgs[run_index(width)] > 0 || r.tail_wgs[run_index(width)] > 0;
+        r.tail_head_wgs[run_index(width)] = tail_head_run_workgroups_per_cu(width);
+        any =any || r.seven_wgs[run_index(width)] > 0 || r.tail_wgs[run_index(width)] > 0;
     }
     if (!any) return 0;
     const size_t bytes = inner_run_counter_bytes(cus, kRunWide) + inner_run_counter_bytes(cus, kRunNarrow);
@@ -813,7 +814,8 @@
 static int g_run_trace_kind = -1;
 constexpr int kRunTraceSlots = 32;
 template <int N>
-static int fill_run_args(mpdx_unet* u, int kind, int first, int width, const float* packed, const float* row, const float* x, float* ws, int B, hipStream_t st, RunArgs<N>& ra) {
+static int fill_run_args(mpdx_unet* u, int kind, int first, int width, const float* packed, const float* row, const float* x, float* ws, int B, hipStream_t st, RunArgs<N>& ra,
+                         int n_counted = N, int n_own = N) {
     memset(&ra, 0, sizeof(ra));
     if (!inner_run_width_ok(width)) return fail(MPDX_E_STATE, "run unit of width %d", width);
     const int nc = inner_run_clusters(B, width);
@@ -822,10 +824,10 @@
         ra.layer[k].n_tiles_n = nc;
         ra.layer[k].trace = g_run_trace && g_run_trace_kind == kind ? g_run_trace + k * kRunTraceSlots : nullptr;
     }
-    ra.n_layers = N; ra.nc = nc;
-    if (int rc = inner_run_begin(u->run, width, nc, N, st, &ra.counters, &ra.base)) return rc;
+    ra.n_layers = n_counted; ra.nc = nc;
+    if (int rc = inner_run_begin(u->run, width, nc, n_counted, st, &ra.counters, &ra.base)) return rc;
     ra.status = u->run.status_dev; ra.budget = u->run.budget;
-    u->inner_run_layers += N;
+    u->inner_run_layers += n_own;
     return 0;
 }
 static int run_inner_run(mpdx_unet* u, int first, int width, const float* packed, const float* row, const float* x, float* ws, int B, hipStream_t st) {
@@ -842,12 +844,24 @@
     ra.layer[0].dst = sp; ra.layer[1].src1 = sp; ra.layer[2].res = sp;
     return launch_tail_run(ra, B, width, st);
 }
+static int run_tail_head_run(mpdx_unet* u, int first, int width, const float* packed, const float* row, const float* x, float* ws, int B, hipStream_t st) {
+    TailHeadRunArgs ra;
+    if (int rc = fill_run_args(u, mpdx_unet::kTailRun, first, width, packed, row, x, ws, B, st, ra, kTailHeadRunLayers, kTailRunLayers)) return rc;
+    const size_t half = (size_t)B * 8 * 128;
+    float* const p1 = ra.layer[0].dst + half;
+    float* const p2 = ra.layer[1].dst + half;
+    ra.layer[2].dst = p1; ra.layer[3].src1 = p1; ra.layer[4].res = p1;
+    ra.layer[4].dst = p2; ra.layer[5].src1 = p2;
+    u->inner_run_heads++;
+    return launch_tail_head_run(ra, B, width, st);
+}
 
 static int run_unit(mpdx_unet* u, const mpdx_unet::Unit& un, const float* packed, const float* row, const float* x, float* ws, int B,
                     const FinalArgs* fa, hipStream_t st) {
     if (un.kind == mpdx_unet::kProgram) return run_fused(u, u->fused[un.fused], packed, row, x, ws, B, fa, st);
     if (un.kind == mpdx_unet::kPair) return run_pair(u, u->layers[un.layer], u->layers[un.layer + 1], packed, row, x, ws, B, st);
     if (un.kind == mpdx_unet::kInnerRun) return run_inner_run(u, un.layer, un.width, packed, row, x, ws, B, st);
+    if (un.kind == mpdx_unet::kTailRun && un.head) return run_tail_head_run(u, un.layer, un.width, packed, row, x, ws, B, st);
     if (un.kind == mpdx_unet::kTailRun) return run_tail_run(u, un.layer, un.fused, un.width, packed, row, x, ws, B, st);
     return run_layer(u, u->layers[un.layer], packed, row, x, ws, B, st);
 }
@@ -1001,6 +1015,34 @@
     }
     return -1;
 }
+static bool tail_head_ok(const mpdx_unet* u, const std::vector<mpdx_unet::Unit>& units, int tf) {
+    if (tf < 1 || units[tf - 1].kind != mpdx_unet::kPair || units[tf - 1].count != 2 || units[tf - 1].layer + 2 != units[tf].layer) return false;
+    const int f = units[tf - 1].layer;
+    const Layer &p1 = u->layers[f], &p2 = u->layers[f + 1];
+    const Layer &l0 = u->layers[f + 2], &l1 = u->layers[f + 3], &l2 = u->layers[f + 4], &l3 = u->layers[f + 5];
+    if (p1.attn || p2.attn || p1.Lv_out || p2.Lv_out) return false;
+    if (!(p1.mode == CONV_S1 && p1.ks == 5 && p1.epi == EPI_GN_MISH && p1.c1 == 256 && p1.c2 == 256 && p1.cin_pad == 512 && p1.rs == 520 && p1.cout == 128 &&
+          p1.L_in == 8 && p1.L_out == 8 && p1.gs == 16 && p1.tb_off >= 0 && p1.res == SRC_NONE && layer_ksplit(p1))) return false;
+    if (!(p2.mode == CONV_S1 && p2.ks == 1 && p2.epi == EPI_BIAS && p2.c1 == 256 && p2.c2 == 256 && p2.cin_pad == 512 && p2.cout == 128 && p2.L_in == 8 &&
+          p2.L_out == 8 && p2.res == SRC_NONE && p2.tb_off < 0 && p2.src1 == p1.src1 && p2.src2 == p1.src2)) return false;
+    if (p1.src1 < 0 || p1.src2 < 0 || p1.src1 == p1.src2 || p1.dst == p2.dst) return false;
+    if (!(l0.src1 == p1.dst && l0.res == p2.dst && l1.dst == p1.dst)) return false;
+    if (u->slot_floats < 2 * 8 * 128) return false;
+    for (int s : {p1.dst, p2.dst, l3.dst})
+        if (s == p1.src1 || s == p1.src2) return false;
+    if (l3.dst == p1.dst || l3.dst == p2.dst) return false;
+    std::vector<int> kept = {p1.dst, p2.dst};
+    for (int j = f + 2 + kTailRunLayers; j < (int)u->layers.size(); ++j) {
+        const Layer& l = u->layers[j];
+        for (int s : kept)
+            if (l.src1 == s || l.src2 == s || l.res == s) return false;
+        kept.erase(std::remove(kept.begin(), kept.end(), l.dst), kept.end());
+    }
+    for (int s : kept)
+        if (s == u->final_slot) return false;
+    (void)l2;
+    return true;
+}
 static int device_cus() {
     int dev = 0, cus = 0;
     if (hipGetDevice(&dev) != hipSuccess || hipDeviceGetAttribute(&cus, hipDeviceAttributeMultiprocessorCount, dev) != hipSuccess) (void)hipGetLastError();
@@ -1008,6 +1050,7 @@
 }
 static int inner_run_auto_width(int B) { return (void)B, kRunNarrow; }
 static int tail_run_auto_width(int B) { return B <= 64 ? kRunNarrow : kRunWide; }
+static int tail_head_auto_width(int B) { return (void)B, kRunNarrow; }
 static bool level_split_auto(int B) { return B <= kSplitMaxB; }
 struct PlanSchedule {
     std::vector<mpdx_unet::Unit> units;
@@ -1038,6 +1081,11 @@
                 units[tf] = {mpdx_unet::kTailRun, spare, units[tf].layer, kTailRunLayers, swt};
                 units.erase(units.begin() + tf + 1, units.begin() + tf + kTailRunLayers);
                 run = true;
+                const int wh = (u->inner_run & mpdx_unet::kRunTailHead) && tail_head_ok(u, units, tf) ? width_of(u->run.tail_head_wgs, tail_head_auto_width(B)) : 0;
+                if (wh) {
+                    units[tf - 1] = {mpdx_unet::kTailRun, -1, units[tf - 1].layer, kTailRunLayers + 2, wh, 1};
+                    units.erase(units.begin() + tf);
+                }
             }
         }
         if (!u->plan_join || u->masked() || units.size() < 2) return 0;
@@ -1142,12 +1190,13 @@
 
 int mpdx_unet_set_inner_run(mpdx_unet* u, int on) {
     if (!u) return fail(MPDX_E_INVALID, "null argument");
-    u->inner_run = on ? (mpdx_unet::kRunSeven | mpdx_unet::kRunTail) : 0;
+    u->inner_run = on ? mpdx_unet::kRunAllParts : 0;
     return 0;
 }
 int mpdx_unet_set_inner_run_parts(mpdx_unet* u, int parts) {
     if (!u) return fail(MPDX_E_INVALID, "null argument");
-    if (parts & ~(mpdx_unet::kRunSeven | mpdx_unet::kRunTail)) return fail(MPDX_E_INVALID, "inner-run parts 0x%x: bit 0 the seven 256 -> 256 layers, bit 1 the tail of up level 0", parts);
+    if (parts & ~mpdx_unet::kRunAllParts)
+        return fail(MPDX_E_INVALID, "inner-run parts 0x%x: bit 0 the seven 256 -> 256 layers, bit 1 the tail of up level 0, bit 3 the tail's head (the level's first residual pair)", parts);
     u->inner_run = parts;
     return 0;
 }
@@ -1170,6 +1219,7 @@
 }
 int mpdx_unet_inner_runs(const mpdx_unet* u) { return u ? u->inner_runs : 0; }
 int mpdx_unet_inner_run_layers(const mpdx_unet* u) { return u ? u->inner_run_layers : 0; }
+int mpdx_unet_inner_run_heads(const mpdx_unet* u) { return u ? u->inner_run_heads : 0; }
 int mpdx_unet_status(const mpdx_unet* u) {
     if (!u) return fail(MPDX_E_INVALID, "null argument");
     return handle_status_error(u, "mpdx_unet_status");
@@ -1346,7 +1396,7 @@
     if (int rc = check_ready(u)) return rc;
     PlanSchedule ps;
     if (int rc = ps.build(u, B)) return rc;
-    u->inner_runs = u->inner_run_layers = u->plan_joined = u->plan_split = 0;
+    u->inner_runs = u->inner_run_layers = u->inner_run_heads = u->plan_joined = u->plan_split = 0;
     hipStream_t st = (hipStream_t)stream;
     const int H = u->cfg.n_support_points, D = u->cfg.state_dim;
     const size_t n = (size_t)B * H * D;
diff --git a/mpd_public_amd/temporal_unet.py b/mpd_public_amd/temporal_unet.py
--- a/mpd_public_amd/temporal_unet.py
+++ b/mpd_public_amd/temporal_unet.py
@@ -168,7 +168,7 @@
     def set_inner_run(self, on: bool):
         _lib.check(_lib.load().mpdx_unet_set_inner_run(self._handle(), int(bool(on))), "mpdx_unet_set_inner_run")
 
-    RUN_SEVEN, RUN_TAIL = 1, 2
+    RUN_SEVEN, RUN_TAIL, RUN_TAIL_HEAD = 1, 2, 8
 
     def set_inner_run_parts(self, parts: int):
         _lib.check(_lib.load().mpdx_unet_set_inner_run_parts(self._handle(), int(parts)), "mpdx_unet_set_inner_run_parts")
@@ -181,6 +181,9 @@
 
     def inner_run_layers(self) -> int:
         return int(_lib.load().mpdx_unet_inner_run_layers(self._handle()))
+
+    def inner_run_heads(self) -> int:
+        return int(_lib.load().mpdx_unet_inner_run_heads(self._handle()))
 
     def status(self) -> int:
         return int(_lib.load().mpdx_unet_status(self._handle()))
```

Measured after the change: 6752 denoising-steps/s (median of 6 runs). 1.4% higher.
